# xipengwang/AprilSAM

Hardware: AMD Instinct MI355X
Metric: Gauss-Newton iterations/sec + factorise ms on M3500 (chi2 match <=1e-6) (higher is better)
Workload: dtype f64; 1 GPU; M3500 batch april_graph_cholesky, 1 replica per GPU (3500 poses, 5454 factors, n=10500); parallelism=single GPU, fronts=680, levels=9, nnz_L=422121

## Files before the change

aprilsam_amd/abi.py:

```python
import ctypes as C


class ZArray(C.Structure):
    _fields_ = [("el_sz", C.c_size_t), ("size", C.c_int), ("alloc", C.c_int), ("data", C.c_void_p)]


class Matd3x3(C.Structure):
    _fields_ = [("nrows", C.c_uint), ("ncols", C.c_uint), ("data", C.c_double * 9)]


class Graph(C.Structure):
    _fields_ = [("factors", C.POINTER(ZArray)), ("nodes", C.POINTER(ZArray)),
                ("attr", C.c_void_p), ("stype", C.c_void_p)]


class FactorCommon(C.Structure):
    _fields_ = [("z", C.POINTER(C.c_double)), ("ztruth", C.POINTER(C.c_double)),
                ("W", C.POINTER(Matd3x3)), ("impl", C.c_void_p)]


class Factor(C.Structure):
    _fields_ = [("type", C.c_int), ("nnodes", C.c_int), ("nodes", C.POINTER(C.c_int)),
                ("length", C.c_int), ("attr", C.c_void_p),
                ("copy", C.c_void_p), ("eval", C.c_void_p), ("state_eval", C.c_void_p),
                ("destroy", C.c_void_p), ("u", FactorCommon), ("stype", C.c_void_p)]


class FactorMax(C.Structure):
    _fields_ = [("factors", C.POINTER(C.POINTER(Factor))), ("logw", C.POINTER(C.c_double)), ("nfactors", C.c_int)]


def max_view(factor):
    f = factor.contents if hasattr(factor, "contents") else factor
    return FactorMax.from_address(C.addressof(f) + Factor.u.offset)


FACTOR_MAX_TYPE = 3
_DESTROY = C.CFUNCTYPE(None, C.c_void_p)


def destroy_factor(fptr):
    _DESTROY(fptr.contents.destroy)(C.cast(fptr, C.c_void_p))


class Node(C.Structure):
    _fields_ = [("UID", C.c_int), ("type", C.c_int), ("length", C.c_int),
                ("state", C.POINTER(C.c_double)), ("init", C.POINTER(C.c_double)),
                ("truth", C.POINTER(C.c_double)), ("l_point", C.POINTER(C.c_double)),
                ("delta_X", C.POINTER(C.c_double)), ("attr", C.c_void_p),
                ("copy", C.c_void_p), ("update", C.c_void_p), ("relinearize", C.c_void_p),
                ("destroy", C.c_void_p), ("impl", C.c_void_p), ("stype", C.c_void_p)]


class CholeskyParam(C.Structure):
    _fields_ = [("tikhanov", C.c_double), ("chol", C.c_void_p), ("factor_num", C.c_int),
                ("ordering", C.POINTER(C.c_int)), ("nreordering", C.c_int), ("show_timing", C.c_int),
                ("delta_x", C.POINTER(C.c_double)), ("B", C.POINTER(C.c_double)),
                ("y", C.POINTER(C.c_double)), ("A", C.c_void_p), ("tr", C.c_void_p),
                ("l_thresh", C.c_double), ("delta_thresh", C.c_double), ("nthreshold", C.c_int),
                ("batch_time", C.c_double), ("delta_xy", C.c_double), ("delta_theta", C.c_double)]


class Stats(C.Structure):
    _fields_ = [("n_nodes", C.c_int), ("n_factors", C.c_int), ("n_fronts", C.c_int), ("n_levels", C.c_int),
                ("max_front_rows", C.c_int), ("symbolic_reused", C.c_int), ("not_spd", C.c_int),
                ("reserved0", C.c_int), ("nnz_L", C.c_longlong), ("flops_factor", C.c_double),
                ("bytes_fronts", C.c_double),
                ("ms_pack", C.c_double), ("ms_symbolic", C.c_double), ("ms_h2d", C.c_double),
                ("ms_device", C.c_double), ("ms_d2h", C.c_double), ("ms_unpack", C.c_double),
                ("ms_total", C.c_double), ("ms_dev_linearize", C.c_double), ("ms_dev_factor", C.c_double),
                ("ms_dev_solve", C.c_double), ("chi2_before", C.c_double), ("error_code", C.c_int), ("reserved1", C.c_int),
                ("inc_replanned", C.c_int), ("inc_old_old_cross", C.c_int), ("inc_fronts_updated", C.c_int), ("dn_launch_fronts", C.c_int)]

    def asdict(self):
        return {k: getattr(self, k) for k, _ in self._fields_}



class LmOpts(C.Structure):
    _fields_ = [("max_iters", C.c_int), ("check_every", C.c_int), ("lambda0", C.c_double), ("lambda_max", C.c_double),
                ("eta", C.c_double), ("ftol", C.c_double), ("xtol", C.c_double)]


class LmReport(C.Structure):
    _fields_ = [("status", C.c_int), ("iterations", C.c_int), ("accepted", C.c_int), ("rejected_not_spd", C.c_int),
                ("F_initial", C.c_double), ("F_final", C.c_double), ("chi2_final", C.c_double), ("lambda_final", C.c_double)]

    def asdict(self):
        return {k: getattr(self, k) for k, _ in self._fields_}


LM_CONVERGED_F, LM_CONVERGED_X, LM_STALLED, LM_MAX_ITERS = 1, 2, 3, 4


class GncOpts(C.Structure):
    _fields_ = [("loss", C.c_int), ("c", C.c_double), ("mu_step", C.c_double), ("max_stages", C.c_int), ("lm", LmOpts)]


class GncReport(C.Structure):
    _fields_ = [("status", C.c_int), ("stages", C.c_int), ("iterations", C.c_int), ("accepted", C.c_int), ("stages_stalled", C.c_int),
                ("n_inliers", C.c_int), ("mu_initial", C.c_double), ("mu_final", C.c_double), ("s_max", C.c_double),
                ("F_final", C.c_double), ("chi2_final", C.c_double)]

    def asdict(self):
        return {k: getattr(self, k) for k, _ in self._fields_}


GNC_GM, GNC_TLS = 1, 2
GNC_FINISHED, GNC_MAX_STAGES = 1, 2


class ChordalOpts(C.Structure):
    _fields_ = [("stages", C.c_int)]


class ChordalReport(C.Structure):
    _fields_ = [("status", C.c_int), ("n_degenerate", C.c_int), ("not_spd_stage", C.c_int), ("min_norm", C.c_double),
                ("F_initial", C.c_double), ("F_final", C.c_double)]

    def asdict(self):
        return {k: getattr(self, k) for k, _ in self._fields_}


ROBUST_NONE, ROBUST_HUBER, ROBUST_CAUCHY, ROBUST_DCS = 0, 1, 2, 3

EXPECTED_SIZES = {"ZArray": 24, "Graph": 32, "Factor": 104, "Node": 112, "CholeskyParam": 128}
EXPECTED_OFFSETS = {
    "Node": dict(UID=0, type=4, length=8, state=16, init=24, truth=32, l_point=40, delta_X=48, attr=56,
                 copy=64, update=72, relinearize=80, destroy=88, impl=96, stype=104),
    "Factor": dict(type=0, nnodes=4, nodes=8, length=16, attr=24, copy=32, eval=40, state_eval=48,
                   destroy=56, u=64, stype=96),
    "CholeskyParam": dict(tikhanov=0, chol=8, factor_num=16, ordering=24, nreordering=32, show_timing=36,
                          delta_x=40, B=48, y=56, A=64, tr=72, l_thresh=80, delta_thresh=88,
                          nthreshold=96, batch_time=104, delta_xy=112, delta_theta=120),
}
```

aprilsam_amd/csrc/capi.cpp:

```cpp
#include <algorithm>
#include <cstdio>
#include <cstdlib>
#include <cstring>
#include <string>
#include <vector>

#include "../../include/aprilsam_amd.h"
#include "plan.h"
#include "errors.h"
#include "refmodel.h"
#include "solver.h"

extern "C" {

void APRILSAM_VERSION(void) {
    printf("================\n");
    printf("| APRILSAM 0.0 |   solver: aprilsam_amd (MI355X / gfx950)\n");
    printf("================\n");
    printf("\n");
}

void april_graph_cholesky_param_init(april_graph_cholesky_param_t *param) {
    asam::drop_context(param);
    asam::unbind_param(param);
// ... 77 lines not shown
    for (int i = 0; i < M->N; i++) visited[i] = 0;
    M->solve_visit(x, dxy, dth, [&](int n, bool upd) { visited[n] = upd ? 2 : 1; });
    return M->start_over;
}
void aprilsam_amd_refmodel_get(void *m, int *parent, int *changed, int *relin) {
    asam::RefModel *M = (asam::RefModel *)m;
    for (int i = 0; i < M->N; i++) { if (parent) parent[i] = M->parent[i]; if (changed) changed[i] = M->changed[i]; if (relin) relin[i] = M->relin[i]; }
}
int aprilsam_amd_refmodel_check(void *m) { return ((asam::RefModel *)m)->check_tree(); }
int aprilsam_amd_last_error(char *msg, int cap) { return asam::get_last_error(msg, cap); }
void aprilsam_amd_clear_error(void) { asam::clear_last_error(); }
int aprilsam_amd_selftest(void) { return asam::selftest(); }
const char *aprilsam_amd_version(void) { return "aprilsam_amd 0.1 (gfx950, multifrontal FP64)"; }
void aprilsam_amd_free(void *p) { free(p); }

struct aprilsam_amd_plan { asam::Plan P; };

aprilsam_amd_plan_t *aprilsam_amd_plan_create(int n_nodes, int n_factors, const int *factor_nodes, const double *xy, int leaf_nodes) {
    aprilsam_amd_plan *pl = new aprilsam_amd_plan();
    try {
        asam::build_plan(pl->P, n_nodes, n_factors, factor_nodes, xy, leaf_nodes > 0 ? leaf_nodes : asam::g_opt.leaf_nodes);
    } catch (const asam::SolverError &e) {
        asam::set_last_error(e.code, e.msg);
        fprintf(stderr, "aprilsam_amd: ERROR %d: %s\n", e.code, e.msg.c_str());
        delete pl;
        return nullptr;
    } catch (const std::exception &e) {
        asam::set_last_error(asam::ERR_INTERNAL, e.what());
        fprintf(stderr, "aprilsam_amd: ERROR %d: %s\n", (int)asam::ERR_INTERNAL, e.what());
        delete pl;
        return nullptr;
    }
    return pl;
}
void aprilsam_amd_plan_destroy(aprilsam_amd_plan_t *plan) { delete plan; }

long long aprilsam_amd_shard_plan(const aprilsam_amd_plan_t *plan, int world, int what, long long *out, long long cap) {
    if (!plan || world < 1) return -1;
    std::vector<int> owner; std::vector<char> top; std::vector<long long> xfer, bcast, v;
    asam::shard_map(plan->P, world, owner, top, xfer, bcast);
    if (what == 1) v = xfer; else if (what == 2) v = bcast; else if (what == 3) v.assign(owner.begin(), owner.end());
    else if (what == 4) v = asam::shard_critical_path(plan->P, world, owner, top); else return -1;
    if (out) for (long long i = 0; i < (long long)v.size() && i < cap; i++) out[i] = v[i];
    return (long long)v.size();
}

int aprilsam_amd_xcd_place(int nF, const int *parent, const int *level, const int *nsb, int l0, int cap, int cap_leaf, int which, int *out, int out_cap) {
    if (nF < 0 || !parent || !level || !nsb || which < 0 || which > 3) return -100;
    std::vector<int> up, leaves;
    int top = 0;
    for (int t = 0; t < nF; t++) top = std::max(top, level[t]);
    for (int l = l0; l <= top; l++) for (int t = 0; t < nF; t++) if (level[t] == l) up.push_back(t);
    if (l0 == 1) for (int t = 0; t < nF; t++) if (level[t] == 0) leaves.push_back(t);
    const asam::XcdLists x = asam::xcd_place(up, leaves, parent, nsb, nF, cap, cap_leaf);
    if (which == 3) return asam::xcd_check(x, up, leaves, parent, nF, cap, cap_leaf);
    const std::vector<int> &v = which == 0 ? x.up : which == 1 ? x.dn : x.leaf;
    if (out) for (int i = 0; i < (int)v.size() && i < out_cap; i++) out[i] = v[i];
    return (int)v.size();
}

long long aprilsam_amd_plan_query(const aprilsam_amd_plan_t *plan, const char *what, long long **out) {
    std::string k(what);
    if (k.compare(0, 3, "bd_") == 0 || k.compare(0, 3, "rd_") == 0) asam::build_gather_lists(const_cast<asam::Plan &>(plan->P));
    const asam::Plan &P = plan->P;
    std::vector<long long> v;
    auto from = [&](const auto &a) { v.assign(a.begin(), a.end()); };
    if (k == "perm") from(P.perm);
    else if (k == "pos") from(P.pos);
    else if (k == "front_first") from(P.f_first);
    else if (k == "front_nsb") from(P.f_nsb);
    else if (k == "front_nub") from(P.f_nub);
    else if (k == "front_parent") from(P.f_parent);
    else if (k == "front_level") from(P.f_level);
    else if (k == "front_rows_ptr") from(P.f_rows_ptr);
    else if (k == "front_rows") from(P.f_rows);
    else if (k == "front_rel") from(P.f_rel);
    else if (k == "front_off") from(P.f_off);
    else if (k == "ch_ptr") from(P.ch_ptr);
    else if (k == "ch_idx") from(P.ch_idx);
    else if (k == "factor_front") from(P.fac_front);
    else if (k == "factor_la") from(P.fac_la);
    else if (k == "factor_lb") from(P.fac_lb);
    else if (k == "factor_swap") from(P.fac_swap);
    else if (k == "bd_front_ptr") from(P.bd_front_ptr);
    else if (k == "bd_row") from(P.bd_row);
    else if (k == "bd_col") from(P.bd_col);
    else if (k == "bd_src_ptr") from(P.bd_src_ptr);
    else if (k == "bd_src") from(P.bd_src);
    else if (k == "rd_front_ptr") from(P.rd_front_ptr);
    else if (k == "rd_col") from(P.rd_col);
    else if (k == "rd_src_ptr") from(P.rd_src_ptr);
    else if (k == "rd_src") from(P.rd_src);
    else if (k == "lev_ptr") from(P.lev_ptr);
    else if (k == "lev_fronts") from(P.lev_fronts);
    else if (k == "stats") v = { P.nF, P.nLevels, P.max_rows, (long long)P.nnzL, (long long)P.flops, (long long)P.pool_doubles };
    else { *out = nullptr; return -1; }
    *out = (long long *)malloc(sizeof(long long) * (v.size() + 1));
    if (!v.empty()) memcpy(*out, v.data(), sizeof(long long) * v.size());
    return (long long)v.size();
}

}
```

aprilsam_amd/csrc/kernels.hip.h:

```cpp
#pragma once
#include <hip/hip_runtime.h>
#include <stdint.h>

#include <type_traits>
namespace asam {

constexpr int PROF_SLOTS = 16;
constexpr int PROF_XCD_UP = 12, PROF_XCD_DN = 13;
constexpr int PROF_X_STORED = 14, PROF_X_DRAINED = 11, PROF_X_FLAG = 15;
__device__ __forceinline__ int xcc_id() { return __builtin_amdgcn_s_getreg(20 | (0 << 6) | ((4 - 1) << 11)) & 7; }
constexpr int TPB = 256;
constexpr int NB = 32;
constexpr int TILE = 64;
constexpr int ASM_CB = 4;
constexpr int OBP = 4;

struct FrontDesc {
    long long off;
    int nsb, nub, first;
    int dest_begin, dest_end;
    int ch_begin, ch_end;
    int rows_begin;
    int parent;
    int dinv0;
    int prim1, prim2;
    int pad[2];
};
static_assert(sizeof(FrontDesc) == 64, "FrontDesc must stay one cache line");
struct DestRec { int brow, bcol, src_begin, src_end; };
struct ChildRec {
    long long uoff;
    int cR;
    int cnu;
    int rel_begin;
    int pad;
};
static_assert(sizeof(ChildRec) == 24, "ChildRec layout");

struct DevPlan {
    int nF;
    const FrontDesc *fd;
    const DestRec *dest;
    const ChildRec *child;
    const int *f_rows, *f_rel;
    const int *slot_blk, *slot_rhs;
    const int *src_idx;
    const double *lambda;
    long long *prof;
    int prof_mode;
    int schur_first_nub;
    int *epoch; const int *flevel; int l0; const int *marks;
    int xmode; uint4 *xg; unsigned xg_bytes;
};
enum { X_FLUSH = 0, X_WT = 1, X_TAGGED = 2 };
constexpr int XG_CONST = -1;

__host__ __device__ inline int asm_chunks(int nbc) { return (nbc + ASM_CB - 1) / ASM_CB; }
struct SyrkRange { int k_lo, k_hi, col_lo, col_hi, ntr, ntc; };
__host__ __device__ inline SyrkRange syrk_range(int R, int C, int ns, int s_lo, int s_hi, int tile = TILE, bool ahead = false) {
    SyrkRange g;
    g.k_lo = s_lo * NB;
    g.k_hi = s_hi * NB < ns ? s_hi * NB : ns;
    g.col_lo = g.k_hi;
    g.col_hi = ahead ? (g.k_hi + OBP * NB < ns ? g.k_hi + OBP * NB : ns) : C;
    if (g.k_hi <= g.k_lo || g.col_hi <= g.col_lo) { g.ntr = g.ntc = 0; return g; }
    g.ntr = ((R - 2) - g.col_lo + tile - 1) / tile;
    g.ntc = (g.col_hi - g.col_lo + tile - 1) / tile;
    return g;
}
__host__ __device__ inline int syrk_tiles(int R, int C, int ns, int s_lo, int s_hi, int tile = TILE, bool ahead = false) {
    SyrkRange g = syrk_range(R, C, ns, s_lo, s_hi, tile, ahead);
    return g.ntc * g.ntr - g.ntc * (g.ntc - 1) / 2;
}
__device__ __forceinline__ int find_seg(const int *__restrict__ pre, int n, int bid) {
    int lo = 0, hi = n;
    while (hi - lo > 1) { int m = (lo + hi) >> 1; if (pre[m] <= bid) lo = m; else hi = m; }
    return lo;
}

__device__ __forceinline__ void trapezoid_tile(int l, int ntr, int ntc, int *ti, int *tj_);
constexpr int SYRK_SB = 8;
constexpr int SYRK_MODE_XCD_SHIFT = 8;
__host__ __device__ inline void trapezoid_tile_xcd(int l, int nt, int ntr, int ntc, int *ti, int *tj) {
    const int q = nt >> 3, rem = nt & 7, x = l & 7;
    int lp = x * q + (x < rem ? x : rem) + (l >> 3);
    for (int c0 = 0;; ) {
        const int w = ntc - c0 < SYRK_SB ? ntc - c0 : SYRK_SB;
        const int cnt = w * (ntr - c0) - w * (w - 1) / 2;
        if (lp < cnt || c0 + w >= ntc) {
            const int tri = w * (w + 1) / 2;
            if (lp < tri) { int r = 0; while ((r + 1) * (r + 2) / 2 <= lp) r++; *ti = c0 + r; *tj = c0 + lp - r * (r + 1) / 2; }
            else { const int e = lp - tri; *ti = c0 + w + e / w; *tj = c0 + e % w; }
            return;
        }
        lp -= cnt; c0 += w;
    }
}

__device__ __forceinline__ double mod2pi_dev(double v) {
    const double TWOPI = 6.2831853071795862319959;
    const double PI_ = 3.141592653589793238462643383279502884196;
    double vin = v + PI_;
    return (vin - TWOPI * floor(vin / TWOPI)) - PI_;
}

__device__ __forceinline__ double fast_rsqrt(double d) {
    double y = __builtin_amdgcn_rsq(d);
    const double h = 0.5 * d;
    double e = fma(-h * y, y, 0.5);
// ... 28 lines not shown
            double acc = 0;
#pragma unroll
            for (int k = 0; k < 3; k++) acc += a[i * 3 + k] * b[k * 3 + j];
            c[i * 3 + j] = acc;
        }
}
__device__ __forceinline__ void a_v(const double *a, const double *v, double *c) {
#pragma unroll
    for (int i = 0; i < 3; i++) {
        double acc = 0;
#pragma unroll
        for (int k = 0; k < 3; k++) acc += a[i * 3 + k] * v[k];
        c[i] = acc;
    }
}

__device__ __forceinline__ void factor_residual(bool binary, const double *pa, const double *pb, const double *z,
                                                double *J0, double *J1, double *r) {
    if (binary) {
        double xa = pa[0], ya = pa[1], ta = pa[2];
        double xb = pb[0], yb = pb[1], tb = pb[2];
        double sa, ca;
        sincos(ta, &sa, &ca);
        double dx = xb - xa, dy = yb - ya;
        double zh0 = ca * dx + sa * dy, zh1 = -sa * dx + ca * dy, zh2 = tb - ta;
        J0[0] = -ca; J0[1] = -sa; J0[2] = -sa * dx + ca * dy;
        J0[3] = sa;  J0[4] = -ca; J0[5] = -ca * dx - sa * dy;
        J0[6] = 0;   J0[7] = 0;   J0[8] = -1;
        J1[0] = ca;  J1[1] = sa;  J1[2] = 0;
        J1[3] = -sa; J1[4] = ca;  J1[5] = 0;
        J1[6] = 0;   J1[7] = 0;   J1[8] = 1;
        r[0] = z[0] - zh0; r[1] = z[1] - zh1; r[2] = mod2pi_dev(z[2] - zh2);
    } else {
        J0[0] = 1; J0[1] = 0; J0[2] = 0; J0[3] = 0; J0[4] = 1; J0[5] = 0; J0[6] = 0; J0[7] = 0; J0[8] = 1;
        r[0] = z[0] - pa[0]; r[1] = z[1] - pa[1]; r[2] = mod2pi_dev(z[2] - pa[2]);
    }
}
__device__ __forceinline__ double rtWr(const double *w, const double *r) {
    double X0 = w[0] * r[0] + w[1] * r[1] + w[2] * r[2];
    double X1 = w[3] * r[0] + w[4] * r[1] + w[5] * r[2];
    double X2 = w[6] * r[0] + w[7] * r[1] + w[8] * r[2];
    return r[0] * X0 + r[1] * X1 + r[2] * X2;
}

__global__ void __launch_bounds__(TPB) k_scatter_host(int nh, const int *__restrict__ idx, const double *__restrict__ hostH, const int *__restrict__ fb,
                                                      const unsigned char *__restrict__ swp, const int *__restrict__ slot_blk,
                                                      const int *__restrict__ slot_rhs, double *__restrict__ Hc) {
    const int k = blockIdx.x * blockDim.x + threadIdx.x;
    if (k >= nh) return;
    const int f = idx[k];
    const double *H = hostH + (size_t)33 * k;
    double *o = Hc + (size_t)slot_blk[3 * f] * 9;
#pragma unroll
    for (int i = 0; i < 3; i++)
#pragma unroll
        for (int j = 0; j < 3; j++) o[i * 3 + j] = (i <= j) ? H[i * 3 + j] : H[j * 3 + i];
    double *go = Hc + (size_t)slot_rhs[2 * f] * 9;
    go[0] = H[27]; go[1] = H[28]; go[2] = H[29];
    if (fb[f] >= 0) {
        const bool s = swp[f] & 1;
        double *o1 = Hc + (size_t)slot_blk[3 * f + 1] * 9, *o2 = Hc + (size_t)slot_blk[3 * f + 2] * 9;
        double *g1 = Hc + (size_t)slot_rhs[2 * f + 1] * 9;
#pragma unroll
        for (int i = 0; i < 3; i++)
#pragma unroll
            for (int j = 0; j < 3; j++) {
                o1[i * 3 + j] = s ? H[9 + j * 3 + i] : H[9 + i * 3 + j];
                o2[i * 3 + j] = (i <= j) ? H[18 + i * 3 + j] : H[18 + j * 3 + i];
            }
        g1[0] = H[30]; g1[1] = H[31]; g1[2] = H[32];
    }
}

#ifndef LIN_WAVES
#define LIN_WAVES 4
#endif
constexpr int LIN_STRIDE = 13;
template <bool STAGED>
__device__ __forceinline__ void linearise_factor(int gtid, int f_begin, int f_end, const int *__restrict__ flist, const int *__restrict__ fa, const int *__restrict__ fb,
                                                 const double *__restrict__ Z, const double *__restrict__ Wm,
                                                 const double *__restrict__ lp, const double *__restrict__ st,
                                                 const unsigned char *__restrict__ swp, const int *__restrict__ slot_blk,
                                                 const int *__restrict__ slot_rhs, double *__restrict__ Hc, const double *__restrict__ upt,
                                                 double (*stg)[STAGED ? 64 * LIN_STRIDE : 1], int (*sid)[STAGED ? 128 : 1], double *mirror = nullptr) {
    int f = f_begin + gtid;
    bool active = f < f_end;
    if (!STAGED && !active) return;
    if (!active) f = f_begin;
    if (flist) f = flist[f];
    int a = fa[f], b = fb[f];
    if (a < 0) { if (!STAGED) return; active = false; a = 0; b = -1; }
    double w[9], z[3], J0[9], J1[9], r[3], pa[3], pb[3] = { 0, 0, 0 };
#pragma unroll
    for (int k = 0; k < 9; k++) w[k] = Wm[(size_t)9 * f + k];
#pragma unroll
    for (int k = 0; k < 3; k++) z[k] = Z[(size_t)3 * f + k];
    const bool binary = b >= 0;
    const double *src = binary ? lp + (size_t)3 * a : (upt ? upt + (size_t)3 * f : st + (size_t)3 * a);
#pragma unroll
    for (int k = 0; k < 3; k++) pa[k] = src[k];
    if (binary) {
#pragma unroll
        for (int k = 0; k < 3; k++) pb[k] = lp[(size_t)3 * b + k];
    }
    factor_residual(binary, pa, pb, z, J0, J1, r);
    const int wave = threadIdx.x >> 6, lane = threadIdx.x & 63;
    auto flush = [&](const double *v, auto nv_, int s0, int s1) {
        constexpr int NV = decltype(nv_)::value;
        double *mine = stg[wave] + lane * LIN_STRIDE;
#pragma unroll
        for (int k = 0; k < NV; k++) mine[k] = v[k];
        sid[wave][2 * lane] = s0; sid[wave][2 * lane + 1] = s1;
        asm volatile("s_waitcnt lgkmcnt(0)" ::: "memory");
#pragma unroll
        for (int it = 0; it < NV; it++) {
            const int idx = it * 64 + lane, t = idx / NV, e = idx - t * NV;
            const int sl = sid[wave][2 * t + (e < 9 ? 0 : 1)];
            if (sl >= 0) Hc[(size_t)sl * 9 + (e < 9 ? e : e - 9)] = stg[wave][t * LIN_STRIDE + e];
        }
        asm volatile("" ::: "memory");
    };
    double JtW0[9], H[9], g[3], out[12];
    at_b(J0, w, JtW0);
    a_b(JtW0, J0, H);
    a_v(JtW0, r, g);
    if constexpr (STAGED) {
#pragma unroll
        for (int i = 0; i < 3; i++)
#pragma unroll
            for (int j = 0; j < 3; j++) out[i * 3 + j] = (i <= j) ? H[i * 3 + j] : H[j * 3 + i];
        out[9] = g[0]; out[10] = g[1]; out[11] = g[2];
        flush(out, std::integral_constant<int, 12>{}, active ? slot_blk[3 * f] : -1, active ? slot_rhs[2 * f] : -1);
    } else {
        double *o = Hc + (size_t)slot_blk[3 * f] * 9;
#pragma unroll
        for (int i = 0; i < 3; i++)
#pragma unroll
            for (int j = 0; j < 3; j++) o[i * 3 + j] = (i <= j) ? H[i * 3 + j] : H[j * 3 + i];
        double *go = Hc + (size_t)slot_rhs[2 * f] * 9;
        go[0] = g[0]; go[1] = g[1]; go[2] = g[2];
        if (mirror) {
#pragma unroll
            for (int k = 0; k < 9; k++) mirror[33 * gtid + k] = o[k];
#pragma unroll
            for (int k = 0; k < 3; k++) mirror[33 * gtid + 9 + k] = g[k];
        }
    }
    if (STAGED ? __ballot(binary && active) != 0ull : binary) {
        const bool on = binary && active;
        a_b(JtW0, J1, H);
        const unsigned sw = swp[f];
        const bool s = sw & 1;
        double JtW1[9], H2[9];
        at_b(J1, w, JtW1);
        a_b(JtW1, J1, H2);
        a_v(JtW1, r, g);
        if (sw & 2) {
            double Hba[9];
            a_b(JtW1, J0, Hba);
#pragma unroll
            for (int i = 0; i < 3; i++)
#pragma unroll
                for (int j = 0; j < 3; j++) H[i * 3 + j] = Hba[j * 3 + i];
        }
        if constexpr (STAGED) {
#pragma unroll
            for (int i = 0; i < 3; i++)
#pragma unroll
                for (int j = 0; j < 3; j++) out[i * 3 + j] = s ? H[j * 3 + i] : H[i * 3 + j];
            flush(out, std::integral_constant<int, 9>{}, on ? slot_blk[3 * f + 1] : -1, -1);
#pragma unroll
            for (int i = 0; i < 3; i++)
#pragma unroll
                for (int j = 0; j < 3; j++) out[i * 3 + j] = (i <= j) ? H2[i * 3 + j] : H2[j * 3 + i];
            out[9] = g[0]; out[10] = g[1]; out[11] = g[2];
            flush(out, std::integral_constant<int, 12>{}, on ? slot_blk[3 * f + 2] : -1, on ? slot_rhs[2 * f + 1] : -1);
        } else {
            double *o1 = Hc + (size_t)slot_blk[3 * f + 1] * 9, *o2 = Hc + (size_t)slot_blk[3 * f + 2] * 9;
            double *g1 = Hc + (size_t)slot_rhs[2 * f + 1] * 9;
#pragma unroll
            for (int i = 0; i < 3; i++)
#pragma unroll
                for (int j = 0; j < 3; j++) o1[i * 3 + j] = s ? H[j * 3 + i] : H[i * 3 + j];
#pragma unroll
            for (int i = 0; i < 3; i++)
#pragma unroll
// ... 1423 lines not shown
    syrk_big_body<4, false, 1>(P, list, pre, n, s_lo, s_hi, mode, pool);
}

__device__ __forceinline__ void trapezoid_tile(int l, int ntr, int ntc, int *ti, int *tj_) {
    const float b = 2.0f * ntr + 1.0f;
    int tj = (int)((b - sqrtf(fmaxf(b * b - 8.0f * l, 0.0f))) * 0.5f);
    if (tj < 0) tj = 0;
    if (tj > ntc - 1) tj = ntc - 1;
    while (tj > 0 && tj * ntr - tj * (tj - 1) / 2 > l) tj--;
    while (tj + 1 < ntc && (tj + 1) * ntr - (tj + 1) * tj / 2 <= l) tj++;
    *tj_ = tj;
    *ti = tj + (l - (tj * ntr - tj * (tj - 1) / 2));
}

template <int CTRL, int ROW_MASK>
__device__ __forceinline__ double dpp_take(double v) {
    const int lo = __builtin_amdgcn_update_dpp(0, __double2loint(v), CTRL, ROW_MASK, 0xf, true);
    const int hi = __builtin_amdgcn_update_dpp(0, __double2hiint(v), CTRL, ROW_MASK, 0xf, true);
    return __hiloint2double(hi, lo);
}
__device__ __forceinline__ double wave_sum63(double v) {
    v += dpp_take<0x111, 0xf>(v);
    v += dpp_take<0x112, 0xf>(v);
    v += dpp_take<0x114, 0xf>(v);
    v += dpp_take<0x118, 0xf>(v);
    v += dpp_take<0x142, 0xa>(v);
    v += dpp_take<0x143, 0xc>(v);
    return v;
}

constexpr long long BS_SPLIT_MIN = 1 << 17;
constexpr int BS_CHUNK = 4096;
__host__ __device__ inline bool bs_split_front(int nsb, int nub) { return nub > 0 && (9ll * nsb * nub >= BS_SPLIT_MIN || 3 * nsb > NB * 4); }
__global__ void __launch_bounds__(TPB) k_backsolve_gemv(DevPlan P, const int *__restrict__ list, const int *__restrict__ pre, int n,
                                                        const double *__restrict__ pool, double *__restrict__ x) {
    __shared__ double xu[BS_CHUNK];
    const int seg = find_seg(pre, n, blockIdx.x);
    const int t = list[seg], cb = blockIdx.x - pre[seg];
    const FrontDesc D_ = P.fd[t];
    const int nsb = D_.nsb, nub = D_.nub, nbc = nsb + nub;
    const int R = 3 * (nbc + 1), ns = 3 * nsb, nu = 3 * nub;
    const int k0 = cb * NB, wdt = min(NB, ns - k0);
    const double *Fg = pool + D_.off;
    const int tid = threadIdx.x, wave = tid >> 6, lane = tid & 63;
    const int *rows = P.f_rows + D_.rows_begin;
    const int c0 = wave * 8;
    double acc[8];
    const double *colp[8];
#pragma unroll
    for (int q = 0; q < 8; q++) { acc[q] = 0; colp[q] = Fg + (size_t)(k0 + min(c0 + q, wdt - 1)) * R + ns; }
    for (int r0 = 0; r0 < nu; r0 += BS_CHUNK) {
        const int nr = min(BS_CHUNK, nu - r0);
        __syncthreads();
        for (int e = tid; e < nr; e += TPB) xu[e] = x[(size_t)3 * rows[(r0 + e) / 3] + (r0 + e) % 3];
        __syncthreads();
        int i = lane;
        for (; i + 192 < nr; i += 256) {
            double v[4][8];
#pragma unroll
            for (int u = 0; u < 4; u++)
#pragma unroll
                for (int q = 0; q < 8; q++) v[u][q] = colp[q][r0 + i + 64 * u];
#pragma unroll
            for (int u = 0; u < 4; u++) {
                const double xv = xu[i + 64 * u];
#pragma unroll
                for (int q = 0; q < 8; q++) acc[q] = fma(v[u][q], xv, acc[q]);
            }
        }
        for (; i < nr; i += 64) {
            const double xv = xu[i];
#pragma unroll
            for (int q = 0; q < 8; q++) acc[q] = fma(colp[q][r0 + i], xv, acc[q]);
        }
    }
#pragma unroll
    for (int q = 0; q < 8; q++) {
        const double sum = wave_sum63(acc[q]);
        if (lane == 63 && c0 + q < wdt) x[(size_t)3 * D_.first + k0 + c0 + q] = sum;
    }
}

__host__ __device__ inline size_t backsolve_lds(int m, int ns, bool pre) { return (size_t)(m + NB + 8 + NB * (NB + 1) + (pre ? (size_t)ns * ((m + 3) | 1) : 0)) * 8; }
struct UpdArgs { const int *perm; const double *lp; double *st, *dX, *st_out, *dx_out; int *bad_out; double *lp_next; };
__device__ __forceinline__ void backsolve_finish(const FrontDesc &D_, int t, const double *xw, double *__restrict__ x, int *xflags, int *bad, const UpdArgs &upd, int ev = 0,
                                                 int xmode = X_FLUSH, const DevPlan *P = nullptr, long long *pf = nullptr) {
    const int tid = threadIdx.x, nsb = D_.nsb, ns = 3 * nsb;
    if (xmode == X_TAGGED) {
        const __amdgpu_buffer_rsrc_t r = xg_rsrc(*P);
        for (int e = tid; e < ns; e += TPB) st_granule(r, (size_t)3 * D_.first + e, xw[e], ev);
        if (pf && tid == 0) pf[PROF_X_STORED] = pf[PROF_X_FLAG] = wall_clock64();
        for (int e = tid; e < ns; e += TPB) x[(size_t)3 * D_.first + e] = xw[e];
    } else if (xmode == X_WT) {
        for (int e = tid; e < ns; e += TPB) st_agent(x + (size_t)3 * D_.first + e, xw[e]);
        if (pf && tid == 0) pf[PROF_X_STORED] = wall_clock64();
        publish_flag_wt(xflags + t, ev, pf);
    } else {
        for (int e = tid; e < ns; e += TPB) x[(size_t)3 * D_.first + e] = xw[e];
        if (pf && tid == 0) pf[PROF_X_STORED] = wall_clock64();
        if (xflags) publish_flag(xflags + t, ev, pf);
    }
    if (upd.perm) {
        for (int k = tid; k < nsb; k += TPB) {
            const int i = upd.perm[D_.first + k];
            const double d0 = xw[3 * k], d1 = xw[3 * k + 1], d2 = xw[3 * k + 2];
            if (isnan(d0) || isnan(d1) || isnan(d2)) {
                const double qnan = __longlong_as_double(0x7ff8000000000000ll);
                upd.dX[3 * i + 0] = qnan; upd.dX[3 * i + 1] = qnan; upd.dX[3 * i + 2] = qnan;
                if (upd.dx_out) { upd.dx_out[3 * i + 0] = qnan; upd.dx_out[3 * i + 1] = qnan; upd.dx_out[3 * i + 2] = qnan; }
                continue;
            }
            const double s0 = upd.lp[3 * i + 0] + d0, s1 = upd.lp[3 * i + 1] + d1, s2 = mod2pi_dev(upd.lp[3 * i + 2] + d2);
            if (upd.st) { upd.st[3 * i + 0] = s0; upd.st[3 * i + 1] = s1; upd.st[3 * i + 2] = s2; }
            if (upd.lp_next) { upd.lp_next[3 * i + 0] = s0; upd.lp_next[3 * i + 1] = s1; upd.lp_next[3 * i + 2] = s2; }
            upd.dX[3 * i + 0] = d0; upd.dX[3 * i + 1] = d1; upd.dX[3 * i + 2] = d2;
            if (upd.st_out) {
                upd.st_out[3 * i + 0] = s0; upd.st_out[3 * i + 1] = s1; upd.st_out[3 * i + 2] = s2;
                upd.dx_out[3 * i + 0] = d0; upd.dx_out[3 * i + 1] = d1; upd.dx_out[3 * i + 2] = d2;
            }
        }
    }
    if (upd.bad_out && tid == 0 && __hip_atomic_load(bad, __ATOMIC_RELAXED, __HIP_MEMORY_SCOPE_AGENT) != 0) {
#pragma unroll
        for (int k = 0; k < 4; k++) upd.bad_out[k] = __hip_atomic_load(bad + k, __ATOMIC_RELAXED, __HIP_MEMORY_SCOPE_AGENT);
    }
}
constexpr int BS_TALL_ROWS = 768;
template <bool PRE, bool TALL = false>
__global__ void __launch_bounds__(TPB) k_backsolve_t(DevPlan P, const int *__restrict__ fronts, const double *__restrict__ pool,
                                                     double *__restrict__ x, int split, int *xflags, int wait, int *bad, UpdArgs upd) {
    extern __shared__ __attribute__((aligned(16))) double smem[];
    const int t = fronts[blockIdx.x];
    if (t < 0) return;
    const int ev = xflags ? flag_value(P) : 0;
    const FrontDesc D_ = P.fd[t];
    const int nsb = D_.nsb, nub = D_.nub, nbc = nsb + nub;
    const int R = 3 * (nbc + 1), ns = 3 * nsb, m = 3 * nbc;
    double *xw = smem;
    double *part = smem + m;
    double *Ldg = smem + m + NB + 8;
    const double *Fg = pool + D_.off;
    const int tid = threadIdx.x, wave = tid >> 6, lane = tid & 63;
    const int *rows = P.f_rows + D_.rows_begin;
    long long *pf = (P.prof && P.prof_mode == 2) ? P.prof + (size_t)t * PROF_SLOTS : nullptr;
    double *Lp = smem + m + NB + 8 + NB * (NB + 1);
    const int ldp = R | 1;
    auto Lat = [&](int c, int r) -> double { if constexpr (PRE) return Lp[c * ldp + r]; else return Fg[(size_t)c * R + r]; };
    if constexpr (PRE) {
        const int ne = ns * R;
        for (int e0 = tid; e0 < ne; e0 += 8 * TPB) {
            double v[8];
#pragma unroll
            for (int u = 0; u < 8; u++) v[u] = Fg[min(e0 + u * TPB, ne - 1)];
#pragma unroll
            for (int u = 0; u < 8; u++) { const int e = e0 + u * TPB; if (e < ne) { const int c = e / R; Lp[c * ldp + (e - c * R)] = v[u]; } }
        }
    }
    const int xmode = x_handover_mode(P, xflags, ev, PRE && wait);
    const bool xtag = xmode == X_TAGGED && D_.parent >= 0;
    if (wait && D_.parent >= 0 && !xtag) {
        if (tid == 0) wait_flag(xflags + D_.parent, bad, ev);
        if constexpr (PRE) { __syncthreads(); asm volatile("" ::: "memory"); }
        else acquire_all();
    }
    if (pf && tid == 0 && !xtag) pf[4] = wall_clock64();
    const bool pre_t = split && bs_split_front(nsb, nub);
    const int mprod = pre_t ? ns : m;
    if (pre_t) { for (int e = tid; e < ns; e += TPB) xw[e] = Fg[(size_t)e * R + m] - x[(size_t)3 * D_.first + e]; }
    else {
        for (int e = tid; e < ns; e += TPB) xw[e] = Fg[(size_t)e * R + m];
        if (xtag) gather_x(P, D_, rows, xw + ns, 3 * nub, ev, bad, pf);
        else for (int e = tid; e < 3 * nub; e += TPB) { const double *xp = x + (size_t)3 * rows[e / 3] + e % 3; if constexpr (PRE) xw[ns + e] = ld_agent(xp); else xw[ns + e] = *xp; }
    }
    __syncthreads();
    if (pf && tid == 0) pf[5] = wall_clock64();
    long long t_prod = 0, t_sum = 0, t_solve = 0, ts = 0;
    constexpr int PFU = 8;
    double pv[TALL ? PFU : 1][8], pdg[4];
    auto prefetch = [&](int k1p) {
        if constexpr (TALL && !PRE) {
            const int k0p = max(0, k1p - NB), wdtp = k1p - k0p;
#pragma unroll
            for (int q = 0; q < 4; q++) {
                const int e = tid + q * TPB, r = e & 31, cc = e >> 5;
                pdg[q] = Fg[(size_t)(k0p + min(cc, wdtp - 1)) * R + k0p + min(r, wdtp - 1)];
            }
#pragma unroll
            for (int u = 0; u < PFU; u++) {
                const int row = min(k1p + lane + 64 * u, mprod - 1);
                if (k1p + 64 * u < mprod) {
#pragma unroll
                    for (int q = 0; q < 8; q++) pv[u][q] = Fg[(size_t)(k0p + min(wave * 8 + q, wdtp - 1)) * R + row];
                } else {
#pragma unroll
                    for (int q = 0; q < 8; q++) pv[u][q] = 0.0;
                }
            }
        }
    };
    prefetch(ns);
    for (int k1 = ns; k1 > 0; k1 -= NB) {
        const int k0 = max(0, k1 - NB), wdt = k1 - k0;
        if (pf) ts = wall_clock64();
        double dg[4];
#pragma unroll
        for (int q = 0; q < 4; q++) {
            const int e = tid + q * TPB, r = e & 31, cc = e >> 5;
            if constexpr (TALL && !PRE) dg[q] = pdg[q]; else dg[q] = Lat(k0 + min(cc, wdt - 1), k0 + min(r, wdt - 1));
// ... 153 lines not shown
    double *Iv = Ls + 6 * NB * (NB + 1);
    const bool pre_t = split && bs_split_front(nsb, nub);
    for (int e = tid; e < ns; e += TPB) xw[e] = pre_t ? x[(size_t)3 * D_.first + e] : 0.0;
    __syncthreads();
    for (int B = nB - 1; B >= 0; B--) {
        const int k0 = B * OBW, Wb = min(OBW, ns - k0), nsub = (Wb + NB - 1) / NB;
        double lv[24], iv[16];
#pragma unroll
        for (int k = 0; k < 24; k++) {
            const int e = tid + TPB * k, bq = e >> 10, i = e & 31, j = (e >> 5) & 31;
            const int sr = bq == 0 ? 1 : (bq < 3 ? 2 : 3), sc = bq == 0 ? 0 : (bq < 3 ? bq - 1 : bq - 3);
            lv[k] = Fg[(size_t)(k0 + min(NB * sc + j, Wb - 1)) * R + k0 + min(NB * sr + i, Wb - 1)];
        }
        const double *dv = dinv_keep + ((size_t)D_.dinv0 + B * OBP) * (NB * NB);
#pragma unroll
        for (int k = 0; k < 16; k++) iv[k] = dv[tid + TPB * k];
        Gemv128 g;
        const int wnext = B < nB - 1 ? min(OBW, ns - (k0 + OBW)) : 1;
        if (B < nB - 1) gemv128_load(g, Fg, R, k0 + OBW, wnext, k0);
        if (B < nB - 2 && tid == 0) wait_flag(tflag + B, bad);
#pragma unroll
        for (int k = 0; k < 24; k++) {
            const int e = tid + TPB * k, bq = e >> 10, i = e & 31, j = (e >> 5) & 31;
            const int sr = bq == 0 ? 1 : (bq < 3 ? 2 : 3);
            Ls[bq * (NB * (NB + 1)) + i * (NB + 1) + j] = (NB * sr + i < Wb) ? lv[k] : 0.0;
        }
#pragma unroll
        for (int k = 0; k < 16; k++) { const int e = tid + TPB * k; Iv[(e >> 10) * (NB * (NB + 1)) + ((e >> 5) & 31) * (NB + 1) + (e & 31)] = iv[k]; }
        if (B < nB - 1) gemv128_sums(g, w, [&](int q, double sum) { xs[32 * wave + q] = sum; });
        __syncthreads();
        {
            double v = 0.0;
            const int e = tid;
            if (e < Wb) {
                v = Fg[(size_t)(k0 + e) * R + m] - xw[k0 + e];
                if (B < nB - 1) v -= xs[e];
                if (B < nB - 2) v -= ld_agent(farf + (size_t)B * OBW + e);
            }
            __syncthreads();
            if (e < OBW) w[e] = v;
        }
        __syncthreads();
        for (int sb = nsub - 1; sb >= 0; sb--) {
            {
                const int i = tid & 31, part = tid >> 5;
                double acc = 0;
#pragma unroll
                for (int jj = 0; jj < 4; jj++) { const int j = 4 * part + jj; acc = fma(Iv[sb * (NB * (NB + 1)) + j * (NB + 1) + i], w[NB * sb + j], acc); }
                xs[part * NB + i] = acc;
            }
            __syncthreads();
            if (tid < NB) {
                double v = 0;
#pragma unroll
                for (int part = 0; part < 8; part++) v += xs[part * NB + tid];
                w[NB * sb + tid] = v;
                if (NB * sb + tid < Wb) xw[k0 + NB * sb + tid] = v;
            }
            __syncthreads();
            if (sb > 0) {
                const int q = tid >> 6, l = tid & 63, j = l & 31, half = l >> 5;
                if (q < sb) {
                    const int bq = (sb == 1 ? 0 : (sb == 2 ? 1 : 3)) + q;
                    double acc = 0;
#pragma unroll
                    for (int ii = 0; ii < 16; ii++) { const int i = 16 * half + ii; acc = fma(Ls[bq * (NB * (NB + 1)) + i * (NB + 1) + j], w[NB * sb + i], acc); }
                    xs[256 + (q * 2 + half) * NB + j] = acc;
                }
                __syncthreads();
                if (tid < NB * sb) { const int q = tid >> 5, j = tid & 31; w[NB * q + j] -= xs[256 + (q * 2) * NB + j] + xs[256 + (q * 2 + 1) * NB + j]; }
                __syncthreads();
            }
        }
        for (int e = tid; e < Wb; e += TPB) x[(size_t)3 * D_.first + k0 + e] = xw[k0 + e];
        if (B >= 2 && H > 0) publish_flag(xflag + B);
    }
    __syncthreads();
    for (int e = tid; e < 2 * BSB_MAXB; e += TPB) reset_flag(xflag + e, 0);
    backsolve_finish(D_, t, xw, x, nullptr, bad, upd);
}

constexpr int BSW = 64;
constexpr int BSW_MAX_NS = NB + 8 + NB * (NB + 1) - 256;
template <int BSWT = BSW>
__device__ __forceinline__ void backsolve_w_body(const DevPlan &P, const int t, const double *__restrict__ pool, double *__restrict__ x, int *xflags, int *bad,
                                                 const UpdArgs &upd, double *smem) {
    const int ev = xflags ? flag_value(P) : 0;
    const FrontDesc D_ = P.fd[t];
    const int nsb = D_.nsb, nub = D_.nub, nbc = nsb + nub;
    const int R = 3 * (nbc + 1), ns = 3 * nsb, m = 3 * nbc;
    double *xw = smem;
    double *partial = smem + m;
    double *dgs = smem + m + 256;
    double *Lp = smem + m + NB + 8 + NB * (NB + 1);
    const int ldp = R | 1;
    const double *Fg = pool + D_.off;
    const int tid = threadIdx.x, wave = tid >> 6, lane = tid & 63;
    const int *rows = P.f_rows + D_.rows_begin;
    long long *pf = (P.prof && P.prof_mode == 2) ? P.prof + (size_t)t * PROF_SLOTS : nullptr;
    if (pf && tid == 0) pf[PROF_XCD_DN] = 1 + xcc_id();
    {
        const int ne = ns * R;
        for (int e0 = tid; e0 < ne; e0 += 8 * TPB) {
            double v[8];
#pragma unroll
            for (int u = 0; u < 8; u++) v[u] = Fg[min(e0 + u * TPB, ne - 1)];
#pragma unroll
            for (int u = 0; u < 8; u++) {
                const int e = e0 + u * TPB;
                if (e < ne) {
                    const int c = e / R, r = e - c * R;
                    Lp[c * ldp + r] = r > c ? v[u] : 0.0;
                    if (r == c) dgs[c] = v[u];
                }
            }
        }
    }
    const int xmode = x_handover_mode(P, xflags, ev, true);
    const bool xtag = xmode == X_TAGGED && D_.parent >= 0;
    if (xflags && D_.parent >= 0 && !xtag) {
        if (tid == 0) wait_flag(xflags + D_.parent, bad, ev);
        __syncthreads();
        asm volatile("" ::: "memory");
    }
    if (pf && tid == 0 && !xtag) pf[4] = wall_clock64();
    for (int e = tid; e < ns; e += TPB) xw[e] = Fg[(size_t)e * R + m];
    if (xtag) gather_x(P, D_, rows, xw + ns, 3 * nub, ev, bad, pf);
    else for (int e = tid; e < 3 * nub; e += TPB) xw[ns + e] = ld_agent(x + (size_t)3 * rows[e / 3] + e % 3);
    __syncthreads();
    if (pf && tid == 0) pf[5] = wall_clock64();
    for (int k1 = ns; k1 > 0; k1 -= BSWT) {
        const int k0 = max(0, k1 - BSWT), wdt = k1 - k0;
        const bool on = lane < wdt;
        const int c = k0 + (on ? lane : 0);
        const double *Lc = Lp + (size_t)c * ldp;
        auto chain = [&](auto w_) {
            constexpr int W = decltype(w_)::value;
            double l[W];
#pragma unroll
            for (int i = 1; i < W; i++) l[i] = Lc[k0 + min(i, wdt - 1)];
            const double rinv = on ? 1.0 / dgs[c] : 1.0;
#pragma unroll
            for (int i = 1; i < W; i++) l[i] *= rinv;
            __syncthreads();
            if (pf && tid == 0 && k1 == ns) pf[6] = wall_clock64();
            double w = on ? (xw[c] - ((partial[64 + lane] + partial[128 + lane]) + partial[192 + lane])) * rinv : 0.0;
#pragma unroll
            for (int i = W - 1; i > 0; i--) {
                const double xi = readlane_d(w, i);
                w = fma(-l[i], xi, w);
            }
            if (on) xw[c] = w;
        };
        if (wave == 0) {
            if (wdt <= 16) chain(std::integral_constant<int, 16>{});
            else if (BSWT <= 32 || wdt <= 32) chain(std::integral_constant<int, 32>{});
            else if constexpr (BSWT > 32) chain(std::integral_constant<int, 64>{});
        } else {
            double acc0 = 0, acc1 = 0;
            int i = k1 + wave - 1;
            for (; i + 3 < m; i += 6) { acc0 = fma(Lc[i], xw[i], acc0); acc1 = fma(Lc[i + 3], xw[i + 3], acc1); }
            if (i < m) acc0 = fma(Lc[i], xw[i], acc0);
            partial[wave * 64 + lane] = acc0 + acc1;
            __syncthreads();
        }
        __syncthreads();
    }
    if (pf && tid == 0) pf[7] = wall_clock64();
    backsolve_finish(D_, t, xw, x, xflags, bad, upd, ev, xmode, &P, pf);
}
__global__ void __launch_bounds__(TPB) k_backsolve_w(DevPlan P, const int *__restrict__ fronts, const double *__restrict__ pool,
                                                     double *__restrict__ x, int *xflags, int *bad, UpdArgs upd) {
    extern __shared__ __attribute__((aligned(16))) double smem[];
    const int t = fronts[blockIdx.x];
    if (t < 0) return;
    backsolve_w_body(P, t, pool, x, xflags, bad, upd, smem);
}

__host__ __device__ inline long long upd_packed_offset(int R, int ns, int j) {
    const long long Rv = R - 2, nb0 = ns / 3, b = j / 3, e = j - 3 * b;
    return 3 * ((b - nb0) * Rv - 3 * (nb0 + b - 1) * (b - nb0) / 2) + e * (Rv - 3 * b);
}
__global__ void __launch_bounds__(TPB) k_guard(int mode, const long long *__restrict__ offs, int n, int len, double *__restrict__ pool, int *count) {
    const int b = blockIdx.x;
    if (b >= n) return;
    unsigned long long *g = (unsigned long long *)(pool + offs[b]);
    int bad = 0;
    for (int i = threadIdx.x; i < len; i += TPB) {
        if (mode == 0) g[i] = ~0ull;
        else if (g[i] != ~0ull) bad++;
    }
    if (bad) { atomicAdd(count, bad); count[1] = b; }
}
__global__ void __launch_bounds__(TPB) k_poison(DevPlan P, const int *__restrict__ list, int n, const int *__restrict__ skip_mode, int skip_stride, int what,
                                                double *__restrict__ pool, double *__restrict__ x) {
    if ((int)blockIdx.x >= n) return;
    if (skip_mode && skip_mode[(size_t)blockIdx.x * skip_stride]) return;
    const int t = list ? list[blockIdx.x] : (int)blockIdx.x;
    const FrontDesc D = P.fd[t];
    const int nbc = D.nsb + D.nub, R = 3 * (nbc + 1), ns = 3 * D.nsb, C = 3 * nbc;
    const double qnan = __longlong_as_double(0x7ff8000000000000ll);
    double *Fg = pool + D.off;
    if (what & 1)
        for (int c = ns + (threadIdx.x >> 6); c < C; c += TPB / 64)
            for (int r = 3 * (c / 3) + (threadIdx.x & 63); r < R - 2; r += 64) Fg[(size_t)c * R + r] = qnan;
    if (what & 2) for (int e = threadIdx.x; e < ns; e += TPB) x[(size_t)3 * D.first + e] = qnan;
}
__global__ void __launch_bounds__(TPB) k_pack_update(double *__restrict__ front, int R, int ns, double *__restrict__ buf, int dir) {
    const int j = ns + blockIdx.x, Rv = R - 2, r0 = j / 3 * 3;
    double *__restrict__ col = front + (size_t)j * R;
    double *__restrict__ pk = buf + upd_packed_offset(R, ns, j) - r0;
    if (dir == 0) { for (int r = r0 + threadIdx.x; r < Rv; r += TPB) pk[r] = col[r]; }
    else { for (int r = r0 + threadIdx.x; r < Rv; r += TPB) col[r] = pk[r]; }
}

struct Patch { void *dst; long long src_off; long long bytes; };
__global__ void __launch_bounds__(TPB) k_apply_patches(const Patch *__restrict__ patches, const char *__restrict__ payload) {
    const Patch p = patches[blockIdx.x];
    const char *src = payload + p.src_off;
    char *dst = (char *)p.dst;
    if (((((size_t)dst) | ((size_t)src) | (size_t)p.bytes) & 3) == 0) {
        for (long long i = threadIdx.x; i < p.bytes / 4; i += TPB) ((int *)dst)[i] = ((const int *)src)[i];
    } else {
        for (long long i = threadIdx.x; i < p.bytes; i += TPB) dst[i] = src[i];
    }
}
struct IncFlags { int *epoch; int *marks; const int *up_list; int n_up; };
constexpr int INL_PATCHES = 24, INL_BYTES = 2048;
struct alignas(16) InlinePatches { Patch hdr[INL_PATCHES]; char pay[INL_BYTES]; };
struct IncPrologue {
    const Patch *patches; const char *payload; int n_patch, f_begin, f_end;
    int inl;

    const int *fa, *fb; const double *Z, *Wm, *lp, *st; const unsigned char *swp; const int *slot_blk, *slot_rhs; double *Hc; int *bad;
    long long *stamps;
    int *done; int seq;
};
struct IncArgsHead { IncPrologue a; IncFlags fl; InlinePatches inl; };
constexpr int TAIL_MAXF = 8;
__device__ __forceinline__ void inc_prologue_body(const IncPrologue &a, const IncFlags &fl, double *mirror = nullptr) {
    const Patch *patches = a.patches; const char *payload = a.payload; const int n_patch = a.n_patch, f_begin = a.f_begin, f_end = a.f_end;
    const int *__restrict__ fa = a.fa, *__restrict__ fb = a.fb; const double *__restrict__ Z = a.Z, *__restrict__ Wm = a.Wm, *__restrict__ lp = a.lp, *__restrict__ st = a.st;
    const unsigned char *__restrict__ swp = a.swp; const int *__restrict__ slot_blk = a.slot_blk, *__restrict__ slot_rhs = a.slot_rhs; double *__restrict__ Hc = a.Hc; int *__restrict__ bad = a.bad;
    const int wave = threadIdx.x >> 6, lane = threadIdx.x & 63, nthr = (int)blockDim.x;
    if (threadIdx.x < 4) bad[threadIdx.x] = 0;
    const char *kargs = (const char *)__builtin_amdgcn_kernarg_segment_ptr() + offsetof(IncArgsHead, inl);
    if (a.inl) { patches = (const Patch *)(kargs + offsetof(InlinePatches, hdr)); payload = kargs + offsetof(InlinePatches, pay); }
    for (int q = wave; q < n_patch; q += nthr >> 6) {
        const Patch p = patches[q];
        const char *src = payload + p.src_off;
        char *dst = (char *)p.dst;
        if (((((size_t)dst) | ((size_t)src) | (size_t)p.bytes) & 3) == 0) {
            const int nw = (int)(p.bytes / 4);
            for (int i0 = lane; i0 < nw; i0 += 512) {
                int v[8];
#pragma unroll
                for (int u = 0; u < 8; u++) v[u] = ((const int *)src)[min(i0 + 64 * u, nw - 1)];
#pragma unroll
                for (int u = 0; u < 8; u++) if (i0 + 64 * u < nw) ((int *)dst)[i0 + 64 * u] = v[u];
// ... 243 lines not shown
```

aprilsam_amd/csrc/plan.h:

```cpp
#pragma once
#include <cstdint>
#include <functional>
#include <vector>

namespace asam {

struct Plan {
    int N = 0;
    int F = 0;
    int leaf_nodes = 16;

    std::vector<int> perm;
    std::vector<int> pos;

    int nF = 0;
    std::vector<int> f_first;
    std::vector<int> f_nsb;
    std::vector<int> f_nub;
    std::vector<int> f_parent;
    std::vector<int> f_level;
    std::vector<int64_t> f_rows_ptr;
    std::vector<int> f_rows;
    std::vector<int> f_rel;
    std::vector<int> ch_ptr, ch_idx;
    std::vector<int64_t> f_off;
    int64_t pool_doubles = 0;

    inline int rows(int t) const { return 3 * (f_nsb[t] + f_nub[t] + 1); }
    inline int cols(int t) const { return 3 * (f_nsb[t] + f_nub[t]); }

    std::vector<int> fac_front;
    std::vector<int> fac_la, fac_lb;
    std::vector<int> bd_front_ptr;
    std::vector<int> bd_row, bd_col;
    std::vector<int> bd_src_ptr;
    std::vector<int> bd_src;
    std::vector<int> rd_front_ptr;
    std::vector<int> rd_col;
    std::vector<int> rd_src_ptr;
    std::vector<int> rd_src;
    std::vector<uint8_t> fac_swap;
    struct DestRec { int brow, bcol, src_begin, src_end; };
    std::vector<int> dest_front_ptr;
    std::vector<DestRec> dest;
    std::vector<int> slot_blk;
    std::vector<int> slot_rhs;
    int n_slots = 0;

    int nLevels = 0;
    std::vector<int> lev_ptr, lev_fronts;

    int max_rows = 0;
    int64_t nnzL = 0;
    double flops = 0;
};

void build_plan(Plan &P, int N, int F, const int *factor_nodes, const double *xy, int leaf_nodes);
void build_gather_lists(Plan &P);

struct XcdLists { std::vector<int> up, dn, leaf; };
XcdLists xcd_place(const std::vector<int> &up, const std::vector<int> &leaves, const int *parent, const int *nsb, int nF, int cap, int cap_leaf);
int xcd_check(const XcdLists &x, const std::vector<int> &up, const std::vector<int> &leaves, const int *parent, int nF, int cap, int cap_leaf);

struct NDTree {
    struct Node { std::vector<int> verts; std::vector<int> children; };
    std::vector<Node> nodes;
    std::vector<int> roots;
};
void nested_dissection(int N, const std::vector<int> &adj_ptr, const std::vector<int> &adj,
                       const double *xy, int leaf_nodes, NDTree &tree);

struct PlanSession { explicit PlanSession(int n_nodes, int min_nodes = 1024); ~PlanSession(); PlanSession(const PlanSession &) = delete; bool on = false; };
void plan_parallel_for(int n, int grain, const std::function<void(int, int)> &body);

}
```

aprilsam_amd/csrc/solver.h:

```cpp
#pragma once
#include <vector>
#include "../../include/aprilsam_amd.h"

namespace asam {

struct Options {
    int leaf_nodes = 16;
    int deterministic = 0;
    int use_graph = 1;
    int device_timing = 0;
    int trust_factor_cache = 0;
    int small_lds_kb = 156;
    int inc_fast = 1;
    int inc_multi = 1;
    int inc_one = 1;
    int inc_one_up = 3, inc_one_dn = 4, inc_one_threads = 512, inc_one_spin = 1;
    int inc_tail = 1;
    int inc_inline = 1;
    int inc_tail_solve = 1;
    int inc_lazy_states = 1;
    int inc_replan_tall = 1;
    int inc_update = 1;
    int speculate_factors = 1;
    int warm_up = 1;
    int syrk_xcd_order = 512;
    int syrk_small_tiles = 320;
    int syrk_pair_tiles = 2048;
    int syrk_group = 3;
    int schur_first = 40;
    int small_threads = 1024;
    int tp_threads = 512;
    int tp_fronts = 1000;
    int tp_lds_kb = 80;
    int amalg = 0;
    int amalg_max = 64;
    int pin_last = 0;
    int batch_extend = 1;
    int extend_tail_fronts = 3;
    int persist = 1;
    int persist_max_fronts = 240;
    int xcd_place = 1;
    int tail_poses = 28;
    int blk_backsolve = 1;
    int wave_backsolve = 1;
    int tagged_x = 1;
    int linearize_staged_min = 32768;
    int mem_cap_mb = 0;
    int pool_guard = 0;
    int pool_poison = 0;
    int skip_flag_waits = 0;
    int panel_mode = 1;
};
extern Options g_opt;

void batch_step(april_graph_t *g, april_graph_cholesky_param_t *param);
void inc_step(april_graph_t *g, april_graph_cholesky_param_t *param);
void inc_solve_only(april_graph_t *g, april_graph_cholesky_param_t *param);
double graph_chi2(april_graph_t *g);
int batch_resident(april_graph_t *g, april_graph_cholesky_param_t *param, int iters, double *chi2_out, double *ms_out);
int resident_begin(april_graph_t *g, april_graph_cholesky_param_t *param);
int resident_steps(april_graph_t *g, april_graph_cholesky_param_t *param, int n, int mode);
int resident_sync(april_graph_t *g, april_graph_cholesky_param_t *param);
double resident_chi2(april_graph_t *g);
int resident_end(april_graph_t *g, april_graph_cholesky_param_t *param);
int level_profile(const april_graph_cholesky_param_t *param, double *out, int cap_levels);
int kernel_profile(const april_graph_cholesky_param_t *param, double *ms, long long *calls, double *flops, double *bytes, const char **names);
void drop_context(const april_graph_cholesky_param_t *p);
void drop_graph_pack(const april_graph_t *g);
bool get_stats(const april_graph_cholesky_param_t *p, aprilsam_amd_stats_t *out);
int shard_begin(april_graph_t *g, april_graph_cholesky_param_t *param, int rank, int world);
long long shard_info(const april_graph_cholesky_param_t *param, int what, long long *out, long long cap);
int shard_comm_unique_id(char *out128);
int shard_comm_init_rccl(const april_graph_cholesky_param_t *param, const char *id128);
int shard_comm_init_host(const april_graph_cholesky_param_t *param, const aprilsam_amd_host_comm_t *cb);
int shard_comm_info(const april_graph_cholesky_param_t *param, long long *out, char *path, int cap);
int shard_iterate(april_graph_t *g, april_graph_cholesky_param_t *param, int n);
int shard_gather_states(april_graph_t *g, april_graph_cholesky_param_t *param);
double shard_chi2(april_graph_t *g, april_graph_cholesky_param_t *param);
void shard_end(const april_graph_cholesky_param_t *param);
int debug_guard_selftest(const april_graph_cholesky_param_t *param);
int debug_stage(april_graph_t *g, april_graph_cholesky_param_t *param, int what, double *out);
int debug_front_times(const april_graph_cholesky_param_t *param, long long *out, int n_fronts);
int api_device_count();
int selftest();
struct Plan;
void shard_map(const Plan &P, int world, std::vector<int> &owner, std::vector<char> &top, std::vector<long long> &xfer, std::vector<long long> &bcast);
std::vector<long long> shard_critical_path(const Plan &P, int world, const std::vector<int> &owner, const std::vector<char> &top);
int api_set_device(int d);
int api_param_set_device(const april_graph_cholesky_param_t *param, int slot);
int api_param_get_device(const april_graph_cholesky_param_t *param);
void unbind_param(const april_graph_cholesky_param_t *param);
void warm_up() noexcept;
int api_set_option(const char *name, double v);
int api_get_option(const char *name, double *v);
int marginals(april_graph_t *g, april_graph_cholesky_param_t *param, int n, const int *qa, const int *qb, double *cov, bool joint);
long long selinv_runs(const april_graph_cholesky_param_t *param);
int marginals_joint_any(april_graph_t *g, april_graph_cholesky_param_t *param, int n, const int *a, const int *b, double *cov);
int gate_xyt(april_graph_t *g, april_graph_cholesky_param_t *param, int n, const int *a, const int *b, const double *z, const double *W, double *d2, double *S);
long long path_solve_bytes(const april_graph_cholesky_param_t *param);
int max_selected(april_graph_t *g, april_graph_cholesky_param_t *param, int n, const int *factors, int *out);
void lm_opts_init(aprilsam_amd_lm_opts_t *opts);
int optimize_lm(april_graph_t *g, april_graph_cholesky_param_t *param, const aprilsam_amd_lm_opts_t *opts, aprilsam_amd_lm_report_t *report, double *trace);
void gnc_opts_init(aprilsam_amd_gnc_opts_t *opts);
int optimize_gnc(april_graph_t *g, april_graph_cholesky_param_t *param, const aprilsam_amd_gnc_opts_t *opts, int n, const int *candidates,
                 aprilsam_amd_gnc_report_t *report, double *weights, double *stage_trace);
long long graph_captures(const april_graph_cholesky_param_t *param);
void chordal_opts_init(aprilsam_amd_chordal_opts_t *opts);
int initialize_chordal(april_graph_t *g, april_graph_cholesky_param_t *param, const aprilsam_amd_chordal_opts_t *opts, aprilsam_amd_chordal_report_t *report,
                       double *rot_out, double *raw_out);
constexpr int MAX_MIX_K = 8;
bool is_native_max(const april_graph_factor_t *f);
bool max_check(const april_graph_factor_t *f, char *why, int cap);
double max_const(const april_graph_factor_t *f, int i);
int max_select(const april_graph_factor_t *f, const double *pa, const double *pb);
bool robust_of(const april_graph_factor_t *f, int *kind, double *c);
bool plain_common_factor(const april_graph_factor_t *f);
double robust_host_s(const double *z, const double *w, const double *pa, const double *pb);
int robust_weights(april_graph_t *g, april_graph_cholesky_param_t *param, int n, const int *factors, double *w);

}
```

aprilsam_amd/csrc/solver.hip.cpp:

```cpp
#include <hip/hip_runtime.h>
#include <rccl/rccl.h>
#include <dlfcn.h>

#include <algorithm>
#include <array>
#include <chrono>
#include <thread>
#include <cmath>
#include <cstdio>
#include <cstdlib>
#include <cstring>
#include <functional>
#include <map>
#include <memory>
#include <atomic>
#include <mutex>
#include <string>
#include <unordered_map>
#include <vector>

#include "../../include/aprilsam_amd.h"
#include "errors.h"
#include "kernels.hip.h"
#include "maxmix.hip.h"
#include "robust.hip.h"
#include "gnc.hip.h"
#include "lm.hip.h"
#include "chordal.hip.h"
#include "selinv.hip.h"
#include "pathsolve.hip.h"
#include "plan.h"
#include "refmodel.h"
#include "solver.h"

namespace asam {

#define HIPCHECK(expr)                                                                                 \
    do {                                                                                               \
        hipError_t e_ = (expr);                                                                        \
        if (e_ != hipSuccess) {                                                                        \
            (void)hipGetLastError();                                                                   \
            fail(e_ == hipErrorOutOfMemory ? ERR_OOM : ERR_HIP, "%s failed: %s (%s:%d)", #expr, hipGetErrorString(e_), __FILE__, __LINE__); \
        }                                                                                              \
    } while (0)

static double now_ms() {
    return std::chrono::duration<double, std::milli>(std::chrono::steady_clock::now().time_since_epoch()).count();
}

Options g_opt;
struct OptionDef { const char *name; int Options::*member; int min_value; bool policy; int max_value = 0x7fffffff; };
static const OptionDef OPTION_TABLE[] = {
    { "leaf_nodes", &Options::leaf_nodes, 1, false }, { "deterministic", &Options::deterministic, 0, true }, { "use_graph", &Options::use_graph, 0, true },
    { "device_timing", &Options::device_timing, 0, true }, { "trust_factor_cache", &Options::trust_factor_cache, 0, true },
    { "small_lds_kb", &Options::small_lds_kb, 0, false }, { "syrk_xcd_order", &Options::syrk_xcd_order, 0, false },
    { "schur_first", &Options::schur_first, 0, false }, { "syrk_small_tiles", &Options::syrk_small_tiles, 0, false }, { "syrk_pair_tiles", &Options::syrk_pair_tiles, 0, false }, { "syrk_group", &Options::syrk_group, 2, false, 8 }, { "panel_mode", &Options::panel_mode, 0, false },
    { "small_threads", &Options::small_threads, 64, false }, { "tp_fronts", &Options::tp_fronts, 0, false }, { "tp_lds_kb", &Options::tp_lds_kb, 0, false },
    { "tp_threads", &Options::tp_threads, 64, false }, { "inc_fast", &Options::inc_fast, 0, true }, { "inc_multi", &Options::inc_multi, 0, true },
    { "inc_one", &Options::inc_one, 0, true }, { "inc_one_up", &Options::inc_one_up, 1, true }, { "inc_one_dn", &Options::inc_one_dn, 1, true },
    { "inc_one_threads", &Options::inc_one_threads, 64, true }, { "inc_one_spin", &Options::inc_one_spin, 0, true }, { "inc_tail", &Options::inc_tail, 0, false },
    { "inc_inline", &Options::inc_inline, 0, true }, { "inc_update", &Options::inc_update, 0, true }, { "inc_tail_solve", &Options::inc_tail_solve, 0, true },
    { "inc_lazy_states", &Options::inc_lazy_states, 0, true }, { "inc_replan_tall", &Options::inc_replan_tall, 0, true },
    { "speculate_factors", &Options::speculate_factors, 0, true }, { "warm_up", &Options::warm_up, 0, true }, { "pin_last", &Options::pin_last, 0, false }, { "persist", &Options::persist, 0, false },
    { "persist_max_fronts", &Options::persist_max_fronts, 0, false }, { "xcd_place", &Options::xcd_place, 0, false }, { "linearize_staged_min", &Options::linearize_staged_min, 0, false },
    { "wave_backsolve", &Options::wave_backsolve, 0, false }, { "tagged_x", &Options::tagged_x, 0, false, 2 }, { "blk_backsolve", &Options::blk_backsolve, 0, false }, { "tail_poses", &Options::tail_poses, 8, false },
    { "batch_extend", &Options::batch_extend, 0, true }, { "extend_tail_fronts", &Options::extend_tail_fronts, 0, true }, { "mem_cap_mb", &Options::mem_cap_mb, 0, true },
    { "pool_guard", &Options::pool_guard, 0, false }, { "amalg", &Options::amalg, 0, false }, { "amalg_max", &Options::amalg_max, 1, false }, { "pool_poison", &Options::pool_poison, 0, false }, { "skip_flag_waits", &Options::skip_flag_waits, 0, false },
};
static const OptionDef *find_option(const char *name) {
    for (const OptionDef &d : OPTION_TABLE) if (!strcmp(d.name, name)) return &d;
    return nullptr;
}
static std::once_flag g_opt_once;
static void load_env_options() {
    std::call_once(g_opt_once, [] {
        for (const OptionDef &d : OPTION_TABLE) {
            std::string env = "APRILSAM_AMD_";
            for (const char *q = d.name; *q; q++) env += (char)toupper((unsigned char)*q);
            const char *sv = getenv(env.c_str());
            if (sv && *sv) g_opt.*(d.member) = std::min(d.max_value, std::max(d.min_value, (int)atof(sv)));
        }
    });
}

constexpr int MAX_SLOTS = 64;
static std::atomic<int> g_device{ -1 };
static std::mutex g_slot_mu[MAX_SLOTS];
static thread_local int t_slot = 0;
static int device_count() {
    static std::atomic<int> cached{ 0 };
    int n = cached.load(std::memory_order_relaxed);
    if (n > 0) return n;
    if (hipGetDeviceCount(&n) != hipSuccess) { (void)hipGetLastError(); return 0; }
    if (n > 0) cached.store(n, std::memory_order_relaxed);
    return n;
}
static int physical_device(int slot) { const int n = device_count(); return n > 0 ? slot % n : 0; }
static thread_local int t_device = -1;
template <class V> struct Registry {
    using Map = std::map<const void *, std::unique_ptr<V>>;
    Map m; mutable std::mutex mu;
    typename Map::iterator find(const void *k) { std::lock_guard<std::mutex> lk(mu); return m.find(k); }
    typename Map::iterator end() { return m.end(); }
    std::pair<typename Map::iterator, bool> emplace(const void *k, std::unique_ptr<V> v) { std::lock_guard<std::mutex> lk(mu); return m.emplace(k, std::move(v)); }
    void erase(typename Map::iterator it) { std::lock_guard<std::mutex> lk(mu); m.erase(it); }
    void put(const void *k, std::unique_ptr<V> v) { std::lock_guard<std::mutex> lk(mu); m[k] = std::move(v); }
    template <class F> void for_each(F &&f) { std::lock_guard<std::mutex> lk(mu); for (auto &kv : m) f(*kv.second); }
    template <class F> bool with(const void *k, F &&f) { std::lock_guard<std::mutex> lk(mu); auto it = m.find(k); if (it == m.end()) return false; f(*it->second); return true; }
};
static std::map<const void *, int> g_param_slot; static std::mutex g_param_slot_mu;
static std::atomic<int> g_param_slot_n{ 0 };
static int default_slot() { const int d = g_device.load(std::memory_order_relaxed); return d < 0 ? 0 : d % MAX_SLOTS; }
static int slot_of_graph(const void *g);
static int slot_for(const void *param, const void *g) {
    if (param && g_param_slot_n.load(std::memory_order_acquire) > 0) { std::lock_guard<std::mutex> lk(g_param_slot_mu); auto it = g_param_slot.find(param); if (it != g_param_slot.end()) return it->second; }
    if (!param && g) { const int s = slot_of_graph(g); if (s >= 0) return s; }
    return default_slot();
}
struct SlotLock {
    int slot; std::unique_lock<std::mutex> lk;
    SlotLock(const void *param, const void *g) : slot(slot_for(param, g)), lk(g_slot_mu[slot]) {
        for (int now; (now = slot_for(param, g)) != slot; ) { lk.unlock(); slot = now; lk = std::unique_lock<std::mutex>(g_slot_mu[slot]); }
        t_slot = slot;
        if (device_count() > 0) {
            const int dev = physical_device(slot);
            int cur = -1;
            if (t_device != dev || hipGetDevice(&cur) != hipSuccess || cur != dev) { (void)hipSetDevice(dev); t_device = dev; }
        }
    }
};
static std::once_flag g_dev_once;
static void ensure_device() {
    std::call_once(g_dev_once, [] {
        load_env_options();
        int n = device_count();
        if (n <= 0) fail(ERR_NO_DEVICE, "no HIP device visible: the april_graph_cholesky* / april_graph_chi2 entry points of "
                         "libaprilsam_amd.so run on an AMD GPU only (there is NO CPU fallback: nothing was computed)");
        if (g_device < 0) {
            const char *lr = getenv("LOCAL_RANK");
            g_device = lr ? atoi(lr) % n : 0;
        }
    });
}

template <class T> struct DBuf {
    T *p = nullptr; size_t cap = 0;
    bool need(size_t n) {
// ... 312 lines not shown
```

aprilsam_amd/csrc/solver_context.inc.h:

```cpp
enum { K_LINEARIZE = 0, K_FRONT_SMALL, K_ASSEMBLE_BIG, K_PANEL_BIG, K_SYRK_BIG, K_BACKSOLVE, K_UPDATE, NKERN };
static const char *const KNAMES[NKERN] = { "k_linearize", "k_front_small", "k_assemble_big", "k_panel_big", "k_syrk_big", "k_backsolve", "k_update_states" };
struct Launch { int list_off, pre_off, n, grid; bool single = false; int tile = TILE; };

struct LevelPlan {
    int small_off = 0, n_small = 0; size_t small_lds = 0;
    long long full_limit = 0;
    int small_nt = 512;
    int n_big = 0; size_t asm_lds = 0;
    Launch asm_big{};
    std::vector<Launch> syrka, syrk1;
    bool paired = false;
    std::vector<Launch> bchain, btile, syrkw;
    int all_off = 0, n_all = 0; size_t solve_lds = 0;
    size_t solve_w_lds = 0; int maxns = 0;
    Launch bs_gemv{};
    Launch bs_blk{}; size_t bs_blk_lds = 0;
    int rest_off = 0, n_rest = 0; size_t rest_lds = 0;
};

struct IncState {
    bool ready = false;
    bool pristine = false;
    int Nb = 0, Fb = 0, nF0 = 0, nLev0 = 0;
    int cap_nodes = 0, cap_fact = 0;
// ... 16 lines not shown
    std::vector<int> t_first, t_cnt;
    std::vector<int> tf_of;
    std::vector<std::vector<int>> kids;
    std::vector<LevelPlan> base_levels;
    std::vector<int> st_i32, st_tab, st_sb, st_sr, st_ids; std::vector<DestRec> st_dest; std::vector<ChildRec> st_child;
    std::vector<unsigned char> st_sw; std::vector<double> st_zeros; std::vector<char> need;
    std::vector<char> stale;
    bool upd_ok = true;
    bool base_has_big = false;
    std::vector<char> st_mid, st_mode; std::vector<int> st_owner, st_mask, st_wout, st_slot; std::vector<UpdRec> st_upd, st_rec;
};

struct SelLevel { int gat_off = 0, n_gat = 0, diag_off = 0, n_diag = 0, tri_off = 0, n_tri = 0, x_off = 0, n_x = 0, sus_off = 0, n_sus = 0, sss_off = 0, n_sss = 0; };

struct PathState {
    long long serial = -1;
    int N = 0;
    std::vector<SelFront> fr; std::vector<int> depth, i32, rec, node_j;
    DBuf<PsFront> d_fr; DBuf<int4> d_ent; DBuf<int> d_cmap; DBuf<long long> d_at; DBuf<PsPath> d_path; DBuf<PsPair> d_pair;
    DBuf<double> d_buf, d_cov, d_in; HBuf<double> h_out;
    long long peak_doubles = 0;
    void release() {
        d_fr.release(); d_ent.release(); d_cmap.release(); d_at.release(); d_path.release(); d_pair.release(); d_buf.release(); d_cov.release(); d_in.release(); h_out.release();
        fr.clear(); depth.clear(); i32.clear(); rec.clear(); node_j.clear(); serial = -1;
    }
};

struct Context {
    Plan plan;
    bool have_plan = false;
    std::vector<int> pat;
    int patN = 0;
    DBuf<int> d_i32; DBuf<FrontDesc> d_fd; DBuf<DestRec> d_dest; DBuf<ChildRec> d_child; DBuf<double> d_lambda;
    DevPlan dp{};
    DBuf<int> d_tab;
    std::vector<LevelPlan> levels;
    DBuf<unsigned char> d_swap;
    DBuf<int> d_pos;
    DBuf<long long> d_prof;
    DBuf<double> d_pool, d_H, d_x, d_diag;
    DBuf<int> d_bad;
    HBuf<int> h_bad;
    IncPrologue pro{}; InlinePatches inl{};
    bool no_speculation = false;
    HBuf<long long> h_kstamp; HBuf<int> h_done; int done_seq = 0, one_wait = 0;
    std::vector<double> h_lambda;
    aprilsam_amd_stats_t st{};
    hipEvent_t ev[8] = {};
    bool have_events = false;
    double k_ms[NKERN] = {}; long long k_calls[NKERN] = {};
    std::vector<hipEvent_t> k_ev; std::vector<int> k_ids, k_lev;
    std::vector<double> lev_up_ms, lev_dn_ms;
    bool have_fact = false;
    int plan_pin = 0;
    long long plan_persist = 0;
    int same_topo_batches = 0;
    bool used_inc = false;
    bool want_inc = false;
    int batch_nodes = 0;
    IncState inc;
    int inc_F = 0, inc_N = 0;
    std::vector<RefModel::Visit> visits; std::vector<int> involved;
    std::vector<int> base_tab;
    std::vector<int> inc_slot_blk, inc_slot_rhs;
    long long pat_serial = -1, pat_topo = -1;
    RefModel model;
    PatchList patches;
    int batch_factors = 0;
    std::vector<unsigned char> wt; bool wt_any = false, wt_dirty = false;
    long long wt_serial = -1, wt_topo = -1, wt_content = -1;
    DBuf<long long> d_guard; DBuf<int> d_guard_cnt; int n_guard = 0, guard_len = 0;
    std::vector<unsigned char> swap_host;
    int persist_l0 = -1;
    int p_up_off = 0, p_up_n = 0, p_dn_off = 0, p_dn_n = 0, p_nt = 1024; size_t p_up_lds = 0, p_dn_lds = 0; long long p_up_full = 0; int p_dn_maxns = 0, p_dn_maxnu = 0;
    int x_up_off = 0, x_up_n = 0, x_dn_off = 0, x_dn_n = 0;
    int x_leaf_off = 0, x_leaf_n = 0;
    DBuf<int> d_flags, d_flevel, d_perm, d_epoch, d_marks;
    DBuf<uint4> d_xg;
    int flag_stride = 0;
    long long epoch_steps = 0;
    DBuf<double> d_dinv, d_bsb_far; DBuf<int> d_bsb_flags;
    DBuf<int> d_solve_tab; std::vector<int> solve_tab;
    DBuf<UpdRec> d_upd; DBuf<double> d_wbuf;
    hipGraphExec_t gexec = nullptr;
    const void *gexec_key = nullptr;
    long long gexec_serial = 0;
    long long gexec_mx = -1;
    long long gexec_rb = -1;
    hipGraphExec_t gexec_api = nullptr;
    const void *api_key[9] = {};
    hipGraphExec_t gexec_lm = nullptr;
    const void *lm_key[10] = {};
    DBuf<double> d_lm_trial, d_lm_hacc, d_lm_terms, d_lm_trace; DBuf<LmScalars> d_lm; HBuf<LmScalars> h_lm;
    DBuf<double> d_ch; HBuf<double> h_ch; DBuf<int> d_ch_sel;
    long long n_captures = 0;
    int api_key_runs = 0;
    struct Retired { hipGraphExec_t g; hipEvent_t done; };
    std::vector<Retired> retired;
    hipStream_t graph_stream = nullptr;
    void reap_retired(bool wait = false) {
        size_t keep = 0;
        for (Retired &r : retired) {
            if (r.done) {
                if (wait) (void)hipEventSynchronize(r.done);
                else if (hipEventQuery(r.done) != hipSuccess) { retired[keep++] = r; continue; }
                (void)hipEventDestroy(r.done);
            }
            (void)hipGraphExecDestroy(r.g);
        }
        retired.resize(keep);
    }
    void retire(hipGraphExec_t &g) {
        if (!g) return;
        if (retired.size() >= 8) reap_retired();
        if (retired.size() >= 32) reap_retired(true);
        Retired r{ g, nullptr };
        if (graph_stream && hipEventCreateWithFlags(&r.done, hipEventDisableTiming) == hipSuccess) {
            if (hipEventRecord(r.done, graph_stream) != hipSuccess) { (void)hipEventDestroy(r.done); r.done = nullptr; }
        } else r.done = nullptr;
        retired.push_back(r); g = nullptr;
    }
    double lambda_val = -1; int lambda_N = -1;
    int fact_kind = 0; long long fact_epoch = -1; bool fact_asym = false;
    DBuf<double> d_sigma, d_sel_scr; DBuf<SelFront> d_sel_fd; DBuf<int> d_sel_i32, d_sel_q; DBuf<int4> d_sel_ent; HBuf<double> h_cov;
    long long fact_serial = 0;
    std::vector<SelLevel> sel_levels; int sel_tab_kind = 0, sel_N = 0;
    long long sel_serial = -1, sel_tab_serial = -1, sel_runs = 0, sel_pool = 1; double sel_flops = 0;
    PathState ps;
    void release_sel() {
        d_sigma.release(); d_sel_scr.release(); d_sel_fd.release(); d_sel_i32.release(); d_sel_q.release(); d_sel_ent.release(); h_cov.release();
        sel_levels.clear(); sel_serial = -1; sel_tab_serial = -1;
        ps.release();
    }
    void release() {
        release_sel();
        d_i32.release(); d_fd.release(); d_dest.release(); d_child.release(); d_lambda.release(); d_tab.release(); d_swap.release(); d_pos.release();
        d_pool.release(); d_H.release(); d_x.release(); d_diag.release(); d_bad.release(); h_bad.release(); patches.release();
        h_done.release(); h_kstamp.release(); d_prof.release(); d_upd.release(); d_wbuf.release(); d_flags.release(); d_flevel.release(); d_epoch.release(); d_marks.release(); d_perm.release(); d_solve_tab.release(); d_dinv.release(); d_bsb_far.release(); d_bsb_flags.release(); d_guard.release(); d_guard_cnt.release(); n_guard = 0;
        d_lm_trial.release(); d_lm_hacc.release(); d_lm_terms.release(); d_lm_trace.release(); d_lm.release(); h_lm.release();
        d_ch.release(); h_ch.release(); d_ch_sel.release();
        retire(gexec); retire(gexec_api); retire(gexec_lm); reap_retired(true);
        if (have_events) for (auto &e : ev) (void)hipEventDestroy(e);
        have_events = false;
        for (auto &e : k_ev) (void)hipEventDestroy(e);
        k_ev.clear();
    }
};
static Registry<Context> g_ctx;

static void forget_stream(hipStream_t s) {
    g_ctx.for_each([&](Context &c) { if (c.graph_stream == s) c.graph_stream = nullptr; });
}

static Context &ctx_for(const april_graph_cholesky_param_t *p) {
    auto it = g_ctx.find(p);
    if (it == g_ctx.end()) it = g_ctx.emplace(p, std::make_unique<Context>()).first;
    return *it->second;
}
void drop_context(const april_graph_cholesky_param_t *p) {
    SlotLock lk(p, nullptr);
    auto it = g_ctx.find(p);
    if (it != g_ctx.end()) { it->second->release(); g_ctx.erase(it); }
}
bool get_stats(const april_graph_cholesky_param_t *p, aprilsam_amd_stats_t *out) {
    SlotLock lk(p, nullptr);
    auto it = g_ctx.find(p);
    if (it == g_ctx.end()) return false;
    *out = it->second->st;
    return true;
}

struct ShardState;
static void drop_shard_state(const void *param);
static void on_failure(const april_graph_cholesky_param_t *param, const april_graph_t *g, int code, const std::string &msg) {
    set_last_error(code, msg);
    fprintf(stderr, "aprilsam_amd: ERROR %d: %s -- node states left untouched\n", code, msg.c_str());
    fflush(stderr);
    SlotLock lk(param, g);
    (void)hipGetLastError();
    if (g) {
        auto it = g_packs.find(g);
        if (it != g_packs.end()) {
            hipStream_t s = it->second->stream;
            if (s) {
                hipStreamCaptureStatus cs = hipStreamCaptureStatusNone;
                if (hipStreamIsCapturing(s, &cs) == hipSuccess && cs != hipStreamCaptureStatusNone) {
                    hipGraph_t gr = nullptr;
                    (void)hipStreamEndCapture(s, &gr);
                    if (gr) (void)hipGraphDestroy(gr);
                }
                (void)hipStreamSynchronize(s);
                (void)hipGetLastError();
            }
            it->second->release(); g_packs.erase(it);
        }
    }
    if (param) {
        drop_shard_state(param);
        auto it = g_ctx.find(param);
        aprilsam_amd_stats_t st{};
        if (it != g_ctx.end()) { st = it->second->st; it->second->release(); }
        auto fresh = std::make_unique<Context>();
        fresh->st = st; fresh->st.error_code = code; fresh->st.not_spd = 0;
        g_ctx.put(param, std::move(fresh));
    }
}
template <class Fn> static void guarded(const april_graph_cholesky_param_t *param, const april_graph_t *g, Fn &&fn) {
    try { fn(); }
    catch (const SolverError &e) { on_failure(param, g, e.code, e.msg); }
    catch (const std::bad_alloc &) { on_failure(param, g, ERR_OOM, "host memory exhausted (std::bad_alloc)"); }
    catch (const std::exception &e) { on_failure(param, g, ERR_INTERNAL, e.what()); }
}
template <class Fn> static int guarded_rc(const april_graph_cholesky_param_t *param, const april_graph_t *g, Fn &&fn) {
    try { return fn(); }
    catch (const SolverError &e) { on_failure(param, g, e.code, e.msg); return e.code; }
    catch (const std::bad_alloc &) { on_failure(param, g, ERR_OOM, "host memory exhausted (std::bad_alloc)"); return ERR_OOM; }
    catch (const std::exception &e) { on_failure(param, g, ERR_INTERNAL, e.what()); return ERR_INTERNAL; }
}

static const int FIRST_EPOCH = 1 << 20;
struct Context;
static void rewind_epoch(Context &c, hipStream_t s, long long phases);
static void set_const_granules(Context &c, hipStream_t s);
enum { FACT_NONE = 0, FACT_PLAN = 1, FACT_EXTENDED = 2 };
// ... 79 lines not shown
        if (!wide.empty() && wgs <= BSB_MAX_WGS && g_opt.blk_backsolve) {
            const int lo = (int)tab.size();
            tab.insert(tab.end(), wide.begin(), wide.end());
            L.bs_blk = Launch{ lo, (int)tab.size(), (int)wide.size(), 0, false };
            int acc = 0; tab.push_back(0);
            for (int t : wide) { acc += 1 + bsb_helpers(3 * nsb_of(t)); tab.push_back(acc); L.bs_blk_lds = std::max(L.bs_blk_lds, bsb_lds(3 * nsb_of(t))); }
            L.bs_blk.grid = acc;
            L.rest_off = (int)tab.size(); L.n_rest = (int)rest.size();
            tab.insert(tab.end(), rest.begin(), rest.end());
            size_t mm = 0; for (int t : rest) mm = std::max<size_t>(mm, cols(t));
            L.rest_lds = (mm + NB + 8 + NB * (NB + 1)) * 8;
        }
    }
    const int steps = (3 * nsb_of(big[0]) + NB - 1) / NB;
    auto active = [&](int sidx) { int nact = 0; while (nact < (int)big.size() && 3 * nsb_of(big[nact]) > sidx * NB) nact++; return nact; };
    const int nobs = (steps + OBP - 1) / OBP;
    auto make_sub = [&](int i0, int i1, auto count) {
        Launch La; La.list_off = list_off + i0; La.n = i1 - i0; La.pre_off = (int)tab.size();
        int acc = 0; tab.push_back(0);
        for (int i = i0; i < i1; i++) { acc += count(big[i]); tab.push_back(acc); }
        La.grid = acc; La.single = acc == La.n;
        return La;
    };
    auto tile_for = [&](int i0, int i1, int s_lo, int s_hi, bool ahead) {
        int tile = TILE;
        if (g_opt.syrk_small_tiles > 0) {
            long long nt64 = 0;
            for (int i = i0; i < i1; i++) nt64 += syrk_tiles(rows(big[i]), cols(big[i]), 3 * nsb_of(big[i]), s_lo, s_hi, TILE, ahead);
            if (nt64 < g_opt.syrk_small_tiles) tile = TILE / 2;
        }
        return tile;
    };
    {
        long long nt0 = 0;
        for (int i = 0; i < active(0); i++) nt0 += syrk_tiles(rows(big[i]), cols(big[i]), 3 * nsb_of(big[i]), 0, OBP, TILE);
        L.paired = g_opt.syrk_pair_tiles > 0 && nobs >= 2 && nt0 >= g_opt.syrk_pair_tiles;
    }
    for (int o = 0; o < nobs; o++) {
        const int s_lo = o * OBP, s_hi = std::min(s_lo + OBP, steps), nact = active(s_lo);
        if (!L.paired) {
            const int tile = tile_for(0, nact, s_lo, s_hi, false);
            L.syrkw.push_back(make(nact, [&](int t) { return syrk_tiles(rows(t), cols(t), 3 * nsb_of(t), s_lo, s_hi, tile); }));
            L.syrkw.back().tile = tile;
            continue;
        }
        const int G = std::max(2, g_opt.syrk_group), p_lo = (o - o % G) * OBP;
        if (o % G != G - 1) {
            const int n2 = o + 1 < nobs ? active((o + 1) * OBP) : 0;
            int tile = tile_for(0, n2, p_lo, s_hi, true);
            L.syrka.push_back(make_sub(0, n2, [&](int t) { return syrk_tiles(rows(t), cols(t), 3 * nsb_of(t), p_lo, s_hi, tile, true); })); L.syrka.back().tile = tile;
            tile = tile_for(n2, nact, p_lo, s_hi, false);
            L.syrk1.push_back(make_sub(n2, nact, [&](int t) { return syrk_tiles(rows(t), cols(t), 3 * nsb_of(t), p_lo, s_hi, tile); })); L.syrk1.back().tile = tile;
            L.syrkw.push_back(Launch{ 0, 0, 0, 0, false });
        } else {
            const int tile = tile_for(0, nact, p_lo, s_hi, false);
            L.syrka.push_back(Launch{ 0, 0, 0, 0, false }); L.syrk1.push_back(Launch{ 0, 0, 0, 0, false });
            L.syrkw.push_back(make(nact, [&](int t) { return syrk_tiles(rows(t), cols(t), 3 * nsb_of(t), p_lo, s_hi, tile); }));
            L.syrkw.back().tile = tile;
        }
    }
    for (int o = 0; o * OBP < steps; o++) {
        const int nact = active(o * OBP);
        Launch bc{ list_off, 0, nact, nact, true };
        L.bchain.push_back(bc);
        long long tiles1 = 0;
        for (int i = 0; i < nact; i++) tiles1 += block_tiles(rows(big[i]), 3 * nsb_of(big[i]), o, 1);
        const int rb = tiles1 > 1024 ? 2 : 1;
        L.btile.push_back(make(nact, [&](int t) { return block_tiles(rows(t), 3 * nsb_of(t), o, rb); }));
        L.btile.back().tile = rb;
    }
}

struct ShardLayout { std::vector<long long> off; std::vector<char> ghost; long long pool_doubles = 0; };

static void fill_swap_host(Context &c) {
    const Plan &P = c.plan;
    c.swap_host.assign(P.fac_swap.begin(), P.fac_swap.end());
    if (c.wt_any) for (size_t f = 0; f < c.swap_host.size() && f < c.wt.size(); f++) c.swap_host[f] |= (unsigned char)(c.wt[f] << 1);
}
static void upload_plan(Context &c, hipStream_t s, const ShardLayout *lay = nullptr) {
    const Plan &P = c.plan;
    const bool uprof = getenv("APRILSAM_AMD_PLAN_PROFILE") != nullptr;
    const double u0 = uprof ? now_ms() : 0;
    c.retire(c.gexec); c.retire(c.gexec_api); c.retire(c.gexec_lm); c.api_key_runs = 0;
    c.lambda_N = -1;
    c.release_sel();
    std::vector<FrontDesc> &fd = c.inc.fd; fd.assign(P.nF, FrontDesc());
    std::vector<ChildRec> ch(std::max<size_t>(1, P.ch_idx.size()));
    for (int t = 0; t < P.nF; t++) {
        FrontDesc &d = fd[t];
        memset(&d, 0, sizeof(d));
        d.off = lay ? std::max<long long>(lay->off[t], 0) : P.f_off[t]; d.nsb = P.f_nsb[t]; d.nub = P.f_nub[t]; d.first = P.f_first[t];
        d.dest_begin = P.dest_front_ptr[t]; d.dest_end = P.dest_front_ptr[t + 1];
        d.ch_begin = P.ch_ptr[t]; d.ch_end = P.ch_ptr[t + 1];
        d.rows_begin = 0; d.parent = P.f_parent[t];
    }
    for (int t = 0; t < P.nF; t++) {
        int best = -1, second = -1;
        for (int k = P.ch_ptr[t]; k < P.ch_ptr[t + 1]; k++) if (P.f_nub[P.ch_idx[k]] > 0 && (best < 0 || P.f_nub[P.ch_idx[k]] > P.f_nub[P.ch_idx[best]])) best = k;
        for (int k = P.ch_ptr[t]; k < P.ch_ptr[t + 1]; k++) if (k != best && P.f_nub[P.ch_idx[k]] > 0 && (second < 0 || P.f_nub[P.ch_idx[k]] > P.f_nub[P.ch_idx[second]])) second = k;
        fd[t].prim1 = best < 0 ? 0 : best - P.ch_ptr[t] + 1; fd[t].prim2 = second < 0 ? 0 : second - P.ch_ptr[t] + 1;
    }
    for (size_t k = 0; k < P.ch_idx.size(); k++) {
        const int cfr = P.ch_idx[k];
        ChildRec &r = ch[k];
        r.cR = P.rows(cfr); r.cnu = P.f_nub[cfr];
        r.uoff = P.f_off[cfr] + (long long)(3 * P.f_nsb[cfr]) * r.cR + 3 * P.f_nsb[cfr];
        if (lay) {
            if (lay->ghost[cfr]) { r.cR = 3 * r.cnu + 3; r.uoff = lay->off[cfr]; }
            else r.uoff = std::max<long long>(lay->off[cfr], 0) + (long long)(3 * P.f_nsb[cfr]) * r.cR + 3 * P.f_nsb[cfr];
        }
        r.rel_begin = 0; r.pad = cfr;
    }
    const double u1 = uprof ? now_ms() : 0;
    const bool inc = c.want_inc;
    const int INC_NODES_ = inc ? INC_NODES : 0, INC_FACT_ = inc ? INC_FACT : 0;
    const size_t INC_I32_ = inc ? INC_I32 : 0, INC_DEST_ = inc ? INC_DEST : 0, INC_CHILD_ = inc ? INC_CHILD : 0, INC_TAB_ = inc ? INC_TAB : 0;
    c.inc.cap_nodes = INC_NODES_; c.inc.cap_fact = INC_FACT_;
    std::vector<int> i32;
    auto put32 = [&](const std::vector<int> &v) { size_t o = i32.size(); i32.insert(i32.end(), v.begin(), v.end()); if (v.empty()) i32.push_back(0); return o; };
    size_t o_rows = put32(P.f_rows), o_rel = put32(P.f_rel);
    size_t o_sb = put32(P.slot_blk); i32.resize(i32.size() + (size_t)3 * INC_FACT_, -1);
    size_t o_sr = put32(P.slot_rhs); i32.resize(i32.size() + (size_t)2 * INC_FACT_, -1);
    c.inc.i32_used = (long long)i32.size(); c.inc.dest_used = (long long)P.dest.size(); c.inc.child_used = (long long)P.ch_idx.size();
    for (int t = 0; t < P.nF; t++) fd[t].rows_begin = (int)(o_rows + P.f_rows_ptr[t]);
    for (size_t k = 0; k < P.ch_idx.size(); k++) ch[k].rel_begin = (int)(o_rel + P.f_rows_ptr[ch[k].pad]);
    c.d_i32.need(i32.size() + INC_I32_); c.d_fd.need(fd.size() + 1 + (inc ? MAX_TAIL_FRONTS : 0)); c.d_child.need(ch.size() + INC_CHILD_);
    c.d_dest.need(std::max<size_t>(1, P.dest.size()) + INC_DEST_);
    HIPCHECK(hipMemcpyAsync(c.d_i32.p, i32.data(), i32.size() * 4, hipMemcpyHostToDevice, s));
    HIPCHECK(hipMemcpyAsync(c.d_fd.p, fd.data(), fd.size() * sizeof(FrontDesc), hipMemcpyHostToDevice, s));
    HIPCHECK(hipMemcpyAsync(c.d_child.p, ch.data(), ch.size() * sizeof(ChildRec), hipMemcpyHostToDevice, s));
    static_assert(sizeof(DestRec) == sizeof(Plan::DestRec), "DestRec layout");
    if (!P.dest.empty()) HIPCHECK(hipMemcpyAsync(c.d_dest.p, P.dest.data(), P.dest.size() * sizeof(DestRec), hipMemcpyHostToDevice, s));
    c.d_lambda.need((size_t)P.N + INC_NODES_);
    DevPlan &d = c.dp;
    d.nF = P.nF;
    d.fd = c.d_fd.p; d.dest = c.d_dest.p; d.child = c.d_child.p;
    d.f_rows = c.d_i32.p; d.f_rel = c.d_i32.p; d.slot_blk = c.d_i32.p + o_sb; d.slot_rhs = c.d_i32.p + o_sr; d.src_idx = c.d_i32.p;
    c.inc.o_rows = (long long)o_rows; c.inc.o_rel = (long long)o_rel;
    d.lambda = c.d_lambda.p;
    d.prof = nullptr; d.prof_mode = 0;
    d.schur_first_nub = std::max(0, g_opt.schur_first);
    d.epoch = nullptr; d.flevel = nullptr; d.l0 = 0; d.marks = nullptr;
    if (getenv("APRILSAM_AMD_KPROF")) { c.d_prof.need((size_t)PROF_SLOTS * P.nF); HIPCHECK(hipMemsetAsync(c.d_prof.p, 0, (size_t)8 * PROF_SLOTS * P.nF, s)); d.prof = c.d_prof.p; d.prof_mode = atoi(getenv("APRILSAM_AMD_KPROF")) >= 2 ? atoi(getenv("APRILSAM_AMD_KPROF")) : 1; }
    c.d_swap.need((size_t)P.F + INC_FACT_); c.d_pos.need((size_t)P.N + INC_NODES_);
    fill_swap_host(c);
    HIPCHECK(hipMemcpyAsync(c.d_swap.p, c.swap_host.data(), P.F, hipMemcpyHostToDevice, s));
    c.wt_dirty = false;
    HIPCHECK(hipMemcpyAsync(c.d_pos.p, P.pos.data(), (size_t)P.N * 4, hipMemcpyHostToDevice, s));
    c.d_perm.need((size_t)P.N + INC_NODES_);
    HIPCHECK(hipMemcpyAsync(c.d_perm.p, P.perm.data(), (size_t)P.N * 4, hipMemcpyHostToDevice, s));

    const double u2 = uprof ? now_ms() : 0;
    std::vector<int> tab;
    c.levels.assign(P.nLevels, LevelPlan());
    for (int l = 0; l < P.nLevels; l++) {
        std::vector<int> fr(P.lev_fronts.begin() + P.lev_ptr[l], P.lev_fronts.begin() + P.lev_ptr[l + 1]);
        build_level(c.levels[l], fr, tab, [&](int t, int *nsb, int *nub) { *nsb = P.f_nsb[t]; *nub = P.f_nub[t]; }, [](int) { return true; });
    }
    {
        long long slots = 0;
        for (int t = 0; t < P.nF; t++) fd[t].dinv0 = -1;
        for (int l = 0; l < P.nLevels; l++) {
            const LevelPlan &L = c.levels[l];
            for (int k = 0; k < L.asm_big.n; k++) { const int t = tab[L.asm_big.list_off + k]; fd[t].dinv0 = (int)slots; slots += (long long)OBP * bsb_blocks(3 * P.f_nsb[t]); }
        }
        c.d_dinv.need((size_t)std::max<long long>(slots, 1) * NB * NB);
        HIPCHECK(hipMemcpyAsync(c.d_fd.p, fd.data(), fd.size() * sizeof(FrontDesc), hipMemcpyHostToDevice, s));
        if (!c.d_bsb_flags.p) { c.d_bsb_flags.need((size_t)BSB_MAX_WGS * 2 * BSB_MAXB); HIPCHECK(hipMemsetAsync(c.d_bsb_flags.p, 0, c.d_bsb_flags.cap * 4, s)); c.d_bsb_far.need((size_t)BSB_MAX_WGS * BSB_FAR); }
    }
    for (int l = 0; l < P.nLevels; l++)
        if (c.levels[l].solve_lds > 160 * 1024)
            fail(ERR_UNSUPPORTED, "a frontal matrix has more rows than the back-substitution kernel can hold in LDS (an unsplittable dense region "
                 "of more than ~6000 poses); this build does not tile the solve of such a front");
    c.persist_l0 = -1;
    if (g_opt.persist && !lay && P.nLevels >= 3) {
        int l0 = P.nLevels, cnt = 0;
        const int nt_top = c.levels[P.nLevels - 1].small_nt;
        for (int l = P.nLevels - 1; l >= 0; l--) {
            const LevelPlan &L = c.levels[l];
            if (L.n_big > 0 || L.bs_gemv.grid > 0 || L.small_nt != nt_top || L.n_small != L.n_all || cnt + L.n_small > g_opt.persist_max_fronts) break;
            cnt += L.n_small; l0 = l;
        }
        if (P.nLevels - l0 >= 2) {
            c.persist_l0 = l0; c.p_nt = nt_top; c.p_up_lds = 0; c.p_dn_lds = 0; c.p_up_full = 0; c.p_dn_maxns = 0; c.p_dn_maxnu = 0;
            c.p_up_off = (int)tab.size(); c.p_up_n = cnt;
            for (int l = l0; l < P.nLevels; l++) {
                const LevelPlan &L = c.levels[l];
                for (int k = 0; k < L.n_small; k++) tab.push_back(tab[L.small_off + k]);
                c.p_up_lds = std::max(c.p_up_lds, L.small_lds); c.p_up_full = std::max(c.p_up_full, L.full_limit);
                for (int k = 0; k < L.n_all; k++) { const int t = tab[L.all_off + k]; c.p_dn_lds = std::max(c.p_dn_lds, backsolve_lds(P.cols(t), 3 * P.f_nsb[t], true)); c.p_dn_maxns = std::max(c.p_dn_maxns, 3 * P.f_nsb[t]); c.p_dn_maxnu = std::max(c.p_dn_maxnu, P.cols(t) - 3 * P.f_nsb[t]); }
            }
            c.p_dn_off = (int)tab.size(); c.p_dn_n = cnt;
            for (int l = P.nLevels - 1; l >= l0; l--) { const LevelPlan &L = c.levels[l]; for (int k = 0; k < L.n_all; k++) tab.push_back(tab[L.all_off + k]); }
        }
    }
    c.x_up_n = c.x_dn_n = c.x_leaf_n = 0;
    if (c.persist_l0 >= 0 && g_opt.xcd_place) {
        int cus = 0;
        HIPCHECK(hipDeviceGetAttribute(&cus, hipDeviceAttributeMultiprocessorCount, physical_device(t_slot)));
        const int per_xcd = std::max(1, cus / 8);
        auto per_cu = [](size_t lds, int nt) { return std::max(1, std::min(2048 / std::max(nt, 64), (int)((160 * 1024) / std::max<size_t>(lds, 1)))); };
        const std::vector<int> up(tab.begin() + c.p_up_off, tab.begin() + c.p_up_off + c.p_up_n);
        const LevelPlan &L0 = c.levels[0];
        const bool leaf = c.persist_l0 == 1 && L0.n_big == 0 && L0.bs_gemv.grid == 0 && L0.bs_blk.grid == 0 && L0.n_small == L0.n_all;
        const std::vector<int> leaves = leaf ? std::vector<int>(tab.begin() + L0.small_off, tab.begin() + L0.small_off + L0.n_small) : std::vector<int>();
        const int cap = per_xcd * per_cu(c.p_up_lds, c.p_nt), cap_leaf = per_xcd * (((int)leaves.size() + 8 * per_xcd - 1) / (8 * per_xcd));
        const XcdLists x = xcd_place(up, leaves, P.f_parent.data(), P.f_nsb.data(), P.nF, cap, cap_leaf);
        c.x_up_off = (int)tab.size(); c.x_up_n = (int)x.up.size(); tab.insert(tab.end(), x.up.begin(), x.up.end());
        c.x_dn_off = (int)tab.size(); c.x_dn_n = (int)x.dn.size(); tab.insert(tab.end(), x.dn.begin(), x.dn.end());
        c.x_leaf_off = (int)tab.size(); c.x_leaf_n = (int)x.leaf.size(); tab.insert(tab.end(), x.leaf.begin(), x.leaf.end());
    }
    {
        const size_t stride = (size_t)P.nF + MAX_TAIL_FRONTS;
        const bool fresh = c.d_flags.need(3 * stride);
        c.d_flevel.need(stride);
        if (fresh || (size_t)c.flag_stride != stride) HIPCHECK(hipMemsetAsync(c.d_flags.p, 0, c.d_flags.cap * 4, s));
        c.flag_stride = (int)stride;
        if (c.d_marks.need(stride)) HIPCHECK(hipMemsetAsync(c.d_marks.p, 0, c.d_marks.cap * 4, s));
        if (c.d_epoch.need(1)) { HIPCHECK(hipMemcpyAsync(c.d_epoch.p, &FIRST_EPOCH, 4, hipMemcpyHostToDevice, s)); c.epoch_steps = 0; }
        d.epoch = c.d_epoch.p;
    }
    if (inc) { c.d_upd.need((size_t)g_opt.persist_max_fronts + 64); c.d_wbuf.need((size_t)1 << 19); }
    HIPCHECK(hipMemcpyAsync(c.d_flevel.p, P.f_level.data(), (size_t)P.nF * 4, hipMemcpyHostToDevice, s));
    if (tab.empty()) tab.push_back(0);
    c.d_tab.need(tab.size() + INC_TAB_);
    c.inc.tab_used = (long long)tab.size();
    c.base_tab = tab;
    const double u3 = uprof ? now_ms() : 0;
    HIPCHECK(hipMemcpyAsync(c.d_tab.p, tab.data(), tab.size() * 4, hipMemcpyHostToDevice, s));
    HIPCHECK(hipStreamSynchronize(s));
    const double u4 = uprof ? now_ms() : 0;

    const long long pool_slack = inc ? std::max<long long>(INC_POOL_MIN, P.pool_doubles / 4) : 0;
// ... 136 lines not shown
```

aprilsam_amd/csrc/solver_launch.inc.h:

```cpp

template <class K> static void allow_full_lds(K kern) { HIPCHECK(hipFuncSetAttribute((const void *)kern, hipFuncAttributeMaxDynamicSharedMemorySize, 160 * 1024)); }
static void set_small_attr() {
    static std::once_flag once[MAX_SLOTS];
    std::call_once(once[physical_device(t_slot) % MAX_SLOTS], [] {
        allow_full_lds(k_front_small<256>); allow_full_lds(k_front_small<512>); allow_full_lds(k_front_small<1024>);
        allow_full_lds(k_backsolve_t<false>); allow_full_lds(k_backsolve_t<true>); allow_full_lds(k_backsolve_w); allow_full_lds(k_backsolve_t<false, true>);
        allow_full_lds(k_block_chain); allow_full_lds(k_backsolve_blk); allow_full_lds(k_block_solve<1>); allow_full_lds(k_block_solve<2>);
        allow_full_lds(k_inc_one<256>); allow_full_lds(k_inc_one<512>); allow_full_lds(k_inc_one<1024>);
    });
}
template <class... Args> static void launch_front_small_nt(int nt, int grid, size_t lds, hipStream_t s, const Args &...a) {
    if (nt >= 1024) hipLaunchKernelGGL(k_front_small<1024>, dim3(grid), dim3(1024), lds, s, a...);
    else if (nt >= 512) hipLaunchKernelGGL(k_front_small<512>, dim3(grid), dim3(512), lds, s, a...);
    else hipLaunchKernelGGL(k_front_small<256>, dim3(grid), dim3(256), lds, s, a...);
}
template <class... Args> static void launch_inc_one_nt(int nt, size_t lds, hipStream_t s, const Args &...a) {
    if (nt >= 1024) hipLaunchKernelGGL(k_inc_one<1024>, dim3(1), dim3(1024), lds, s, a...);
    else if (nt >= 512) hipLaunchKernelGGL(k_inc_one<512>, dim3(1), dim3(512), lds, s, a...);
    else hipLaunchKernelGGL(k_inc_one<256>, dim3(1), dim3(256), lds, s, a...);
}

struct KTimer {
    Context *c = nullptr; hipStream_t s = nullptr; size_t nev = 0;
    int level = -1;
    void tic(int id) {
        if (!c) return;
        if (c->k_ev.size() < nev + 2) { c->k_ev.resize(nev + 2); HIPCHECK(hipEventCreate(&c->k_ev[nev])); HIPCHECK(hipEventCreate(&c->k_ev[nev + 1])); }
        HIPCHECK(hipEventRecord(c->k_ev[nev], s));
        c->k_ids.push_back(id); c->k_lev.push_back(level);
    }
    void toc() { if (c) { HIPCHECK(hipEventRecord(c->k_ev[nev + 1], s)); nev += 2; } }
};
static KTimer no_timer;

enum BsForm { BS_WAVE, BS_THREAD, BS_THREAD_TALL };
static void launch_backsolve_list(Context &c, hipStream_t s, BsForm form, const int *list, int n, size_t lds, int split, int *bad, const UpdArgs &upd) {
    if (form == BS_WAVE) hipLaunchKernelGGL(k_backsolve_w, dim3(n), dim3(TPB), lds, s, c.dp, list, c.d_pool.p, c.d_x.p, (int *)nullptr, bad, upd);
    else if (form == BS_THREAD_TALL) hipLaunchKernelGGL((k_backsolve_t<false, true>), dim3(n), dim3(TPB), lds, s, c.dp, list, c.d_pool.p, c.d_x.p, split, (int *)nullptr, 0, bad, upd);
    else hipLaunchKernelGGL((k_backsolve_t<false>), dim3(n), dim3(TPB), lds, s, c.dp, list, c.d_pool.p, c.d_x.p, split, (int *)nullptr, 0, bad, upd);
}

static void launch_backsolve(Context &c, const LevelPlan &L, hipStream_t s, KTimer &kt, const int *tab = nullptr, UpdArgs upd = UpdArgs{}, int list_off = -1, int list_n = 0) {
    if (!tab) tab = c.d_tab.p;
    if (!L.n_all) return;
    kt.tic(K_BACKSOLVE);
    if (L.bs_gemv.grid > 0)
        hipLaunchKernelGGL(k_backsolve_gemv, dim3(L.bs_gemv.grid), dim3(TPB), 0, s, c.dp, tab + L.bs_gemv.list_off, tab + L.bs_gemv.pre_off,
                           L.bs_gemv.n, c.d_pool.p, c.d_x.p);
    int n_all = list_off >= 0 ? list_n : L.n_all, all_off = list_off >= 0 ? list_off : L.all_off; size_t solve_lds = L.solve_lds;
    if (L.bs_blk.grid > 0) {
        hipLaunchKernelGGL(k_backsolve_blk, dim3(L.bs_blk.grid), dim3(TPB), L.bs_blk_lds, s, c.dp, tab + L.bs_blk.list_off, tab + L.bs_blk.pre_off, L.bs_blk.n,
                           c.d_pool.p, c.d_x.p, c.d_dinv.p, c.d_bsb_flags.p, c.d_bsb_far.p, L.bs_gemv.grid > 0 ? 1 : 0, c.d_bad.p, upd);
        n_all = L.n_rest; all_off = L.rest_off; solve_lds = L.rest_lds;
        if (!n_all) { kt.toc(); return; }
    }
    const bool wave = g_opt.wave_backsolve && L.bs_gemv.grid == 0 && L.n_all < g_opt.tp_fronts && L.maxns <= BSW_MAX_NS && L.solve_w_lds <= 80 * 1024;
    const BsForm form = wave ? BS_WAVE : solve_lds >= (size_t)(BS_TALL_ROWS + NB + 8 + NB * (NB + 1)) * 8 ? BS_THREAD_TALL : BS_THREAD;
    launch_backsolve_list(c, s, form, tab + all_off, n_all, wave ? L.solve_w_lds : solve_lds, L.bs_gemv.grid > 0 ? 1 : 0, c.d_bad.p, upd);
    kt.toc();
}

static int launch_xmode(const Context &c, int max_upd_rows) { return c.dp.xmode == X_TAGGED && max_upd_rows > TPB ? (int)X_FLUSH : c.dp.xmode; }
static int device_cus() {
    int cus = 0;
    HIPCHECK(hipDeviceGetAttribute(&cus, hipDeviceAttributeMultiprocessorCount, physical_device(t_slot)));
    return cus;
}
static size_t handover_lds(int xmode, size_t lds, int grid) {
    if (xmode == X_WT || (xmode == X_TAGGED && grid <= device_cus())) return std::max(lds, HANDOVER_LDS_MIN);
    return lds;
}
static DevPlan launch_plan(const Context &c, DevPlan d, int max_upd_rows) { d.xmode = launch_xmode(c, max_upd_rows); return d; }
static DevPlan persist_plan(const Context &c) { DevPlan d = c.dp; d.flevel = c.d_flevel.p; d.l0 = c.persist_l0; d.xmode = launch_xmode(c, c.p_dn_maxnu); return d; }
static void launch_backsolve_multi(Context &c, hipStream_t s, const DevPlan &dp, const int *list, int n, size_t lds, int maxns, int *xflags, const UpdArgs &upd) {
    lds = handover_lds(dp.xmode, lds, n);
    if (g_opt.wave_backsolve && maxns <= BSW_MAX_NS) hipLaunchKernelGGL(k_backsolve_w, dim3(n), dim3(TPB), lds, s, dp, list, c.d_pool.p, c.d_x.p, xflags, c.d_bad.p, upd);
    else hipLaunchKernelGGL((k_backsolve_t<true>), dim3(n), dim3(TPB), lds, s, dp, list, c.d_pool.p, c.d_x.p, 0, xflags, 1, c.d_bad.p, upd);
}

static void enqueue_poison(Context &c, hipStream_t s, const int *list, int n, int what = 3, const UpdRec *recs = nullptr) {
    if (g_opt.pool_poison <= 0 || n <= 0) return;
    static_assert(offsetof(UpdRec, mode) % 4 == 0 && sizeof(UpdRec) % 4 == 0, "UpdRec::mode as a strided int");
    hipLaunchKernelGGL(k_poison, dim3(n), dim3(TPB), 0, s, c.dp, list, n, recs ? (const int *)((const char *)recs + offsetof(UpdRec, mode)) : (const int *)nullptr,
                       (int)(sizeof(UpdRec) / 4), what, c.d_pool.p, c.d_x.p);
}
static void launch_front_persist(Context &c, hipStream_t s) {
    const bool xp = c.x_up_n > 0;
    const int *list = c.d_tab.p + (xp ? c.x_up_off : c.p_up_off), n = xp ? c.x_up_n : c.p_up_n;
    DevPlan dpe = persist_plan(c);
    if (g_opt.skip_flag_waits > 0) dpe.l0 = 1 << 30;
    launch_front_small_nt(c.p_nt, n, c.p_up_lds, s, dpe, list, c.d_pool.p, c.d_H.p, c.d_bad.p, c.p_up_full, c.d_flags.p, 1);
}

static void launch_front_small(Context &c, const LevelPlan &L, hipStream_t s, const int *tab = nullptr, int list_off = -1, int list_n = 0) {
    if (!tab) tab = c.d_tab.p;
    const int off = list_off >= 0 ? list_off : L.small_off, n = list_off >= 0 ? list_n : L.n_small;
    launch_front_small_nt(L.small_nt, n, L.small_lds, s, c.dp, tab + off, c.d_pool.p, c.d_H.p, c.d_bad.p, L.full_limit, (int *)nullptr, 0);
}

static void enqueue_big_steps(Context &c, const LevelPlan &L, hipStream_t s, KTimer &kt, const int *tab = nullptr) {
    if (!tab) tab = c.d_tab.p;
    const int xcd = std::max(0, g_opt.syrk_xcd_order) << SYRK_MODE_XCD_SHIFT;
    for (size_t o = 0; o < L.bchain.size(); o++) {
        const Launch &bc = L.bchain[o], &bt = L.btile[o], &sw = L.syrkw[o];
        kt.tic(K_PANEL_BIG);
        hipLaunchKernelGGL(k_block_chain, dim3(bc.n), dim3(BCH_THREADS), block_chain_lds(), s, c.dp, tab + bc.list_off, (int)o, c.d_pool.p, c.d_diag.p, c.d_dinv.p, c.d_bad.p);
        if (bt.grid > 0) {
            if (bt.tile == 2) hipLaunchKernelGGL(k_block_solve<2>, dim3(bt.grid), dim3(TPB), block_solve_lds(), s, c.dp, tab + bt.list_off, tab + bt.pre_off, bt.n, (int)o, c.d_pool.p, c.d_diag.p, c.d_dinv.p);
            else hipLaunchKernelGGL(k_block_solve<1>, dim3(bt.grid), dim3(TPB), block_solve_lds(), s, c.dp, tab + bt.list_off, tab + bt.pre_off, bt.n, (int)o, c.d_pool.p, c.d_diag.p, c.d_dinv.p);
        }
        kt.toc();
        auto wide = [&](const Launch &w, int s_lo, int s_hi, int mode) {
            if (w.grid <= 0) return;
            kt.tic(K_SYRK_BIG);
            if (w.tile == TILE / 2) hipLaunchKernelGGL(k_syrk_big32, dim3(w.grid), dim3(TPB), 0, s, c.dp, tab + w.list_off, tab + w.pre_off, w.n, s_lo, s_hi, mode | xcd, c.d_pool.p);
            else hipLaunchKernelGGL(k_syrk_big, dim3(w.grid), dim3(TPB), 0, s, c.dp, tab + w.list_off, tab + w.pre_off, w.n, s_lo, s_hi, mode | xcd, c.d_pool.p);
            kt.toc();
        };
        const int G = std::max(2, g_opt.syrk_group), g0 = (int)(o - o % G) * OBP;
        if (!L.paired) wide(sw, (int)o * OBP, (int)(o + 1) * OBP, 1);
        else if ((int)(o % G) != G - 1) { wide(L.syrka[o], g0, (int)(o + 1) * OBP, 2); wide(L.syrk1[o], g0, (int)(o + 1) * OBP, 1); }
        else wide(sw, g0, (int)(o + 1) * OBP, 1);
    }
}

static void enqueue_factor_level(Context &c, const LevelPlan &L, hipStream_t s, KTimer &kt, const int *tab = nullptr) {
    if (!tab) tab = c.d_tab.p;
    if (L.n_small) {
        kt.tic(K_FRONT_SMALL);
        launch_front_small(c, L, s, tab);
        kt.toc();
    }
    if (L.n_big) {
        kt.tic(K_ASSEMBLE_BIG);
        hipLaunchKernelGGL(k_assemble_big, dim3(L.asm_big.grid), dim3(TPB), L.asm_lds, s, c.dp, tab + L.asm_big.list_off,
                           tab + L.asm_big.pre_off, L.asm_big.n, c.d_pool.p, c.d_H.p);
        kt.toc();
        enqueue_big_steps(c, L, s, kt, tab);
    }
}

template <class K, class... Args> static void launch_gnc(hipStream_t s, GraphPack &gp, K kern, const Args &...a) {
    hipLaunchKernelGGL(kern, dim3((gp.gc_n + TPB - 1) / TPB), dim3(TPB), 0, s, gp.gc_n, (const int *)gp.d_gc_f.p, (const double *)gp.d_gc_W0.p, (const GncPar *)gp.d_gc_par.p, a...);
}
static void enqueue_gnc_weight(GraphPack &gp, hipStream_t s, const double *upt) {
    if (gp.gc_n == 0) return;
    launch_gnc(s, gp, k_gnc_weight, (const int *)gp.d_fa.p, (const int *)gp.d_fb.p, (const double *)gp.d_z.p, (const double *)gp.d_lp.p, (const double *)gp.d_state.p, upt, gp.d_W.p, gp.d_gc_w.p);
}

static void enqueue_linearise(Context &c, GraphPack &gp, hipStream_t s, bool unary_at_lp) {
    const int F = c.plan.F;
    enqueue_select(gp, s);
    enqueue_robust(gp, s, unary_at_lp ? gp.d_upt.p : (const double *)nullptr);
    enqueue_gnc_weight(gp, s, unary_at_lp ? gp.d_upt.p : (const double *)nullptr);
    auto launch = [&](auto kern) {
        hipLaunchKernelGGL(kern, dim3((F + TPB - 1) / TPB), dim3(TPB), 0, s, 0, F, (const int *)nullptr, gp.d_fa.p, gp.d_fb.p, gp.d_z.p, gp.d_W.p,
                           gp.d_lp.p, gp.d_state.p, c.d_swap.p, c.dp.slot_blk, c.dp.slot_rhs, c.d_H.p, c.d_bad.p, unary_at_lp ? gp.d_upt.p : (const double *)nullptr, c.d_epoch.p);
    };
    if (F >= g_opt.linearize_staged_min) launch(k_linearize_t<true>); else launch(k_linearize_t<false>);
    if (!gp.host_idx.empty()) {
        const int nh = (int)gp.host_idx.size();
        HIPCHECK(hipMemcpyAsync(gp.d_hostH.p, gp.h_hostH.p, (size_t)33 * 8 * nh, hipMemcpyHostToDevice, s));
        hipLaunchKernelGGL(k_scatter_host, dim3((nh + TPB - 1) / TPB), dim3(TPB), 0, s, nh, gp.d_host_idx.p, gp.d_hostH.p, gp.d_fb.p, c.d_swap.p,
                           c.dp.slot_blk, c.dp.slot_rhs, c.d_H.p);
    }
}

struct NumericArgs {
    hipEvent_t *ev = nullptr;
    bool unary_at_lp = false;
    bool ktime = false;
    bool io_host = false;
    bool relin = false;
    double *st_dest = nullptr;
    const std::function<void()> *fill = nullptr;
};
static void enqueue_numeric(Context &c, GraphPack &gp, hipStream_t s, const NumericArgs &a = NumericArgs{}) {
    const Plan &P = c.plan;
    const int N = P.N;
    const bool io_host = a.io_host;
    KTimer kt;
    if (a.ktime) { c.k_ids.clear(); c.k_lev.clear(); kt.c = &c; kt.s = s; }
    if (a.ev) HIPCHECK(hipEventRecord(a.ev[0], s));
    if (c.dp.prof) HIPCHECK(hipMemsetAsync(c.d_prof.p, 0, (size_t)8 * PROF_SLOTS * P.nF, s));
    if (io_host) hipLaunchKernelGGL(k_load_states, dim3((3 * N + TPB - 1) / TPB), dim3(TPB), 0, s, 3 * N, gp.h_state.p, gp.d_state.p, gp.d_lp.p);
    enqueue_poison(c, s, nullptr, P.nF);
    kt.tic(K_LINEARIZE);
    if (a.fill) (*a.fill)(); else enqueue_linearise(c, gp, s, a.unary_at_lp);
    kt.toc();
    if (a.ev) HIPCHECK(hipEventRecord(a.ev[1], s));
    const int l0 = c.persist_l0 >= 0 ? c.persist_l0 : P.nLevels;
    for (int l = 0; l < l0; l++) {
        kt.level = l;
        if (l == 0 && c.x_leaf_n > 0) { kt.tic(K_FRONT_SMALL); launch_front_small(c, c.levels[0], s, nullptr, c.x_leaf_off, c.x_leaf_n); kt.toc(); }
        else enqueue_factor_level(c, c.levels[l], s, kt);
    }
    kt.level = l0;
    if (l0 < P.nLevels) { kt.tic(K_FRONT_SMALL); launch_front_persist(c, s); kt.toc(); }
    if (a.ev) HIPCHECK(hipEventRecord(a.ev[2], s));
    UpdArgs upd{ c.d_perm.p, gp.d_lp.p, a.st_dest ? a.st_dest : gp.d_state.p, gp.d_dx.p, io_host ? gp.h_lp.p : nullptr, io_host ? gp.h_dx.p : nullptr, nullptr, a.relin ? gp.d_lp.p : nullptr };
    if (l0 < P.nLevels) {
        UpdArgs u = upd; if (l0 == 0) u.bad_out = io_host ? c.h_bad.p : nullptr;
        kt.tic(K_BACKSOLVE);
        const bool xp = c.x_dn_n > 0;
        launch_backsolve_multi(c, s, persist_plan(c), c.d_tab.p + (xp ? c.x_dn_off : c.p_dn_off), xp ? c.x_dn_n : c.p_dn_n, c.p_dn_lds, c.p_dn_maxns, c.d_flags.p + c.flag_stride, u);
        kt.toc();
    }
    for (int l = l0 - 1; l >= 0; l--) {
        UpdArgs u = upd; if (l == 0) u.bad_out = io_host ? c.h_bad.p : nullptr;
        kt.level = l;
        if (l == 0 && c.x_leaf_n > 0) launch_backsolve(c, c.levels[0], s, kt, nullptr, u, c.x_leaf_off, c.x_leaf_n);
        else launch_backsolve(c, c.levels[l], s, kt, nullptr, u);
    }
    if (a.ev) HIPCHECK(hipEventRecord(a.ev[3], s));
    HIPCHECK(hipGetLastError());
}
static void collect_kernel_times(Context &c) {
    for (size_t i = 0; i < c.k_ids.size(); i++) {
        float ms = 0;
        HIPCHECK(hipEventElapsedTime(&ms, c.k_ev[2 * i], c.k_ev[2 * i + 1]));
        c.k_ms[c.k_ids[i]] += ms; c.k_calls[c.k_ids[i]]++;
        const int l = i < c.k_lev.size() ? c.k_lev[i] : -1;
        if (l >= 0) {
            if (c.lev_up_ms.size() <= (size_t)l) { c.lev_up_ms.resize(l + 1, 0.0); c.lev_dn_ms.resize(l + 1, 0.0); }
            (c.k_ids[i] == K_BACKSOLVE ? c.lev_dn_ms : c.lev_up_ms)[l] += ms;
        }
    }
    c.k_ids.clear();
}

template <class Enqueue> static void replay_captured(Context &c, hipGraphExec_t &exec, hipStream_t s, Enqueue enqueue) {
    if (!exec) {
        hipGraph_t graph = nullptr;
        HIPCHECK(hipStreamBeginCapture(s, hipStreamCaptureModeThreadLocal));
        enqueue();
        HIPCHECK(hipStreamEndCapture(s, &graph));
        HIPCHECK(hipGraphInstantiate(&exec, graph, nullptr, nullptr, 0));
        HIPCHECK(hipGraphDestroy(graph));
        c.n_captures++;
    }
    c.graph_stream = s;
    HIPCHECK(hipGraphLaunch(exec, s));
}

long long graph_captures(const april_graph_cholesky_param_t *param) {
    SlotLock lk(param, nullptr);
    auto it = g_ctx.find(param);
    return it == g_ctx.end() ? -1 : it->second->n_captures;
}

struct RunArgs { bool timing = false, unary_at_lp = false, io_host = false, relin = false; };
static void run_numeric(Context &c, GraphPack &gp, const RunArgs &r = RunArgs{}) {
    hipStream_t s = gp.stream;
    set_small_attr();
    rewind_epoch(c, s, 1);
    if (r.timing && !c.have_events) { for (auto &e : c.ev) HIPCHECK(hipEventCreate(&e)); c.have_events = true; }
    NumericArgs a;
    a.io_host = r.io_host;
    if (!r.io_host) a.relin = r.relin;
    const bool graph = g_opt.use_graph && !r.timing && gp.host_idx.empty();
    if (r.io_host && graph) {
        const void *key[9] = { gp.d_state.p, gp.h_state.p, gp.h_lp.p, gp.h_dx.p, c.h_bad.p, (const void *)(size_t)gp.N, (const void *)(size_t)gp.serial, (const void *)(size_t)gp.mx_gen,
                               (const void *)(size_t)gp.rb_gen };
        if (memcmp(key, c.api_key, sizeof(key)) != 0) { c.retire(c.gexec_api); memcpy(c.api_key, key, sizeof(key)); c.api_key_runs = 0; }
        if (c.api_key_runs++ == 0) enqueue_numeric(c, gp, s, a);
        else replay_captured(c, c.gexec_api, s, [&] { enqueue_numeric(c, gp, s, a); });
    } else if (!r.io_host && graph && !r.unary_at_lp) {
        if (c.gexec_key != (const void *)gp.d_state.p || c.gexec_serial != gp.serial || c.gexec_mx != gp.mx_gen || c.gexec_rb != gp.rb_gen) {
            c.retire(c.gexec);
            c.gexec_key = (const void *)gp.d_state.p; c.gexec_serial = gp.serial; c.gexec_mx = gp.mx_gen; c.gexec_rb = gp.rb_gen;
        }
        replay_captured(c, c.gexec, s, [&] { enqueue_numeric(c, gp, s, a); });
    } else {
        a.ev = r.timing ? c.ev : nullptr;
        if (!r.io_host) a.unary_at_lp = r.unary_at_lp;
        enqueue_numeric(c, gp, s, a);
    }
}
```

aprilsam_amd/csrc/solver_pack.inc.h:

```cpp
static std::atomic<long long> g_pack_serial{ 0 };
static void forget_stream(hipStream_t s);
constexpr int STREAM_POOL_MAX = 4;
static std::mutex g_stream_pool_mu;
static std::vector<hipStream_t> g_stream_pool[MAX_SLOTS];
static hipStream_t take_stream(int slot) {
    {
        std::lock_guard<std::mutex> lk(g_stream_pool_mu);
        auto &v = g_stream_pool[slot];
        if (!v.empty()) { hipStream_t s = v.back(); v.pop_back(); return s; }
    }
    hipStream_t s = nullptr;
    HIPCHECK(hipStreamCreateWithFlags(&s, hipStreamNonBlocking));
    return s;
}
static void park_stream(int slot, hipStream_t s) {
    if (hipStreamSynchronize(s) == hipSuccess) {
        std::lock_guard<std::mutex> lk(g_stream_pool_mu);
        auto &v = g_stream_pool[slot];
        if ((int)v.size() < STREAM_POOL_MAX) { v.push_back(s); return; }
    } else (void)hipGetLastError();
    (void)hipStreamDestroy(s);
}
struct GraphPack {
    int slot = 0;
    const long long serial = ++g_pack_serial;
    int N = 0, F = 0;
    int Fg = 0;
    std::vector<int> g2p, p2g;
    std::vector<unsigned> vslot;
    std::vector<const void *> fptr;
    std::vector<int> pending;
    HBuf<int> h_fa, h_fb;
    HBuf<double> h_z, h_W, h_state, h_lp, h_dx;
    DBuf<int> d_fa, d_fb;
    DBuf<double> d_z, d_W, d_state, d_lp, d_dx, d_chi2f, d_scalar;
    DBuf<double> d_lp_last; bool lp_last_valid = false;
    int F_on_device = 0;
    int dirty_lo = 0, dirty_hi = 0;
    long long content_version = 0;
    long long topo_version = 0;
    std::vector<unsigned char> asym; int n_asym = 0;
    void note_asym(int p, const double *w, bool device_factor) {
        const unsigned char a = device_factor && (w[1] != w[3] || w[2] != w[6] || w[5] != w[7]);
        if ((size_t)p >= asym.size()) asym.resize((size_t)p + 1, 0);
        n_asym += (int)a - (int)asym[p]; asym[p] = a;
    }
    std::vector<char> is_host;
    std::vector<double> h_upt; DBuf<double> d_upt;
    int F_cap = 0;
    std::vector<int> host_idx; HBuf<double> h_hostH; DBuf<double> d_hostH; DBuf<int> d_host_idx; int host_evaluated = 0;
    std::vector<int> mx_f, mx_k{ 0 }, mx_sel, mx_of; std::vector<double> mx_z, mx_W, mx_c, mx_logw;
    DBuf<int> d_mx_f, d_mx_k, d_sel; DBuf<double> d_mx_z, d_mx_W, d_mx_c; HBuf<double> mx_stage;
    int mx_on_device = 0; bool mx_dirty = false; long long mx_gen = 0;
    int n_max() const { return (int)mx_f.size(); }
    void mx_clear() {
        if (!mx_f.empty() || mx_on_device) mx_gen++;
        mx_f.clear(); mx_k.assign(1, 0); mx_sel.clear(); mx_of.clear(); mx_z.clear(); mx_W.clear(); mx_c.clear(); mx_logw.clear(); mx_on_device = 0; mx_dirty = false; }
    std::vector<int> rb_f, rb_kind, rb_of; std::vector<double> rb_c, rb_W0, rb_w;
    DBuf<int> d_rb_f, d_rb_kind; DBuf<double> d_rb_c, d_rb_W0, d_rb_w; HBuf<double> rb_stage;
    int rb_on_device = 0; bool rb_dirty = false; long long rb_gen = 0;
    int n_robust() const { return (int)rb_f.size(); }
    void rb_clear() {
        if (!rb_f.empty() || rb_on_device) rb_gen++;
        rb_f.clear(); rb_kind.clear(); rb_of.clear(); rb_c.clear(); rb_W0.clear(); rb_w.clear(); rb_on_device = 0; rb_dirty = false; }
    DBuf<int> d_gc_f; DBuf<double> d_gc_W0, d_gc_w, d_gc_out; DBuf<GncPar> d_gc_par; HBuf<double> gc_stage;
    int gc_n = 0; long long gc_gen = 0;
    hipStream_t stream = nullptr;
    HBuf<double> h_scalar;
    HBuf<double> h_out; bool mirror_sync = false; std::vector<int> changed; const double *new_states = nullptr;
    void release() {
        h_out.release(); mirror_sync = false;
        h_fa.release(); h_fb.release(); h_z.release(); h_W.release(); h_state.release(); h_lp.release(); h_dx.release();
        d_fa.release(); d_fb.release(); d_z.release(); d_W.release(); d_state.release(); d_lp.release(); d_lp_last.release(); d_dx.release();
        d_chi2f.release(); d_scalar.release(); h_scalar.release(); h_hostH.release(); d_hostH.release(); d_host_idx.release(); d_upt.release();
        d_mx_f.release(); d_mx_k.release(); d_sel.release(); d_mx_z.release(); d_mx_W.release(); d_mx_c.release(); mx_stage.release(); mx_clear();
        d_rb_f.release(); d_rb_kind.release(); d_rb_c.release(); d_rb_W0.release(); d_rb_w.release(); rb_stage.release(); rb_clear();
        d_gc_f.release(); d_gc_W0.release(); d_gc_w.release(); d_gc_out.release(); d_gc_par.release(); gc_stage.release(); gc_n = 0;
        if (stream) { forget_stream(stream); park_stream(slot, stream); }
        stream = nullptr;
    }
};

static Registry<GraphPack> g_packs;

static int slot_of_graph(const void *g) {
    int slot = -1;
    g_packs.with(g, [&](GraphPack &gp) { slot = gp.slot; });
    return slot;
}
static GraphPack &pack_for(const april_graph_t *g) {
    auto it = g_packs.find(g);
    if (it != g_packs.end() && it->second->slot != t_slot) {
        const int os = it->second->slot;
        std::unique_lock<std::mutex> old_slot(g_slot_mu[os], std::try_to_lock);
        for (const auto t0 = std::chrono::steady_clock::now(); !old_slot.owns_lock(); (void)old_slot.try_lock()) {
            if (std::chrono::steady_clock::now() - t0 > std::chrono::seconds(10))
                fail(ERR_UNSUPPORTED, "graph %p was last solved on device slot %d, which other threads kept busy for 10 s: one graph is driven from one slot at a "
                     "time (the call on slot %d did nothing)", (const void *)g, os, t_slot);
            std::this_thread::sleep_for(std::chrono::microseconds(20));
        }
        it = g_packs.find(g);
        if (it != g_packs.end() && it->second->slot != t_slot) { it->second->release(); g_packs.erase(it); it = g_packs.end(); }
    }
    if (it == g_packs.end()) {
        auto p = std::make_unique<GraphPack>();
        p->slot = t_slot;
        p->stream = take_stream(t_slot);
        it = g_packs.emplace(g, std::move(p)).first;
    }
    return *it->second;
}
void drop_graph_pack(const april_graph_t *g) {
    SlotLock lk(nullptr, g);
    auto it = g_packs.find(g);
    if (it != g_packs.end()) { it->second->release(); g_packs.erase(it); }
}

static inline int zsize(const zarray_t *z) { return z ? z->size : 0; }

static void pack_factors(GraphPack &gp, const april_graph_t *g, bool validate_old = true) {
    const bool trust = g_opt.trust_factor_cache || !validate_old;
    const int Fg = zsize(g->factors);
    april_graph_factor_t **fs = (april_graph_factor_t **)g->factors->data;
    const int N = zsize(g->nodes);
    int from = gp.Fg;
    bool valid = from <= Fg && (int)gp.fptr.size() == from && (int)gp.g2p.size() == from + 1;
    if (valid && trust) valid = from == 0 || (validate_old ? memcmp(gp.fptr.data(), fs, sizeof(void *) * from) == 0 : (gp.fptr[0] == fs[0] && gp.fptr[from - 1] == fs[from - 1]));
    auto restart = [&]() { gp.topo_version++; from = 0; gp.F = 0; gp.F_on_device = 0; gp.host_idx.clear(); gp.host_evaluated = 0; gp.is_host.clear(); gp.p2g.clear(); gp.vslot.clear(); gp.g2p.assign(1, 0); gp.asym.clear(); gp.n_asym = 0; gp.mx_clear(); gp.rb_clear(); };
    if (!valid) restart();
    struct Ent { int a, b; bool host; unsigned short slots; unsigned char carry; };
    Ent ents[64]; int ne = 0; bool is_max = false, is_rb = false; int rb_kind = 0; double rb_c = 0;
    auto classify = [&](const april_graph_factor_t *f, int i) {
        ne = 0; is_max = false; is_rb = false;
        if (is_native_max(f)) {
            char why[192];
            if (f->nnodes != 2 || !max_check(f, why, sizeof why)) fail(ERR_UNSUPPORTED, "factor %d: max factor: %s", i, f->nnodes != 2 ? "not binary" : why);
            ents[ne++] = Ent{ f->nodes[0], f->nodes[1], false, 0, 3 }; is_max = true;
        } else if (f->type == APRIL_GRAPH_FACTOR_XYT_TYPE && f->nnodes == 2) { ents[ne++] = Ent{ f->nodes[0], f->nodes[1], false, 0, 3 }; is_rb = robust_of(f, &rb_kind, &rb_c); }
        else if (f->type == APRIL_GRAPH_FACTOR_XYTPOS_TYPE && f->nnodes == 1) { ents[ne++] = Ent{ f->nodes[0], -1, false, 0, 3 }; is_rb = robust_of(f, &rb_kind, &rb_c); }
        else if ((f->nnodes == 1 || f->nnodes == 2) && f->eval)
            ents[ne++] = Ent{ f->nodes[0], f->nnodes == 2 ? f->nodes[1] : -1, true, (unsigned short)(f->nnodes == 2 ? 1 : 0xff), 3 };
        else if (f->nnodes >= 3 && f->nnodes <= 11 && f->eval) {
            for (int x = 0; x < f->nnodes; x++)
                for (int y = x + 1; y < f->nnodes; y++) {
                    const unsigned char carry = (unsigned char)(((x == 0 && y == 1) ? 1 : 0) | ((x == 0) ? 2 : 0));
                    ents[ne++] = Ent{ f->nodes[x], f->nodes[y], true, (unsigned short)((x << 8) | y), carry };
                }
        } else {
            fail(ERR_UNSUPPORTED, "factor %d has type %d / %d nodes; factors of foreign types are supported with 1 to 11 nodes and an "
                                  "eval() function pointer (aprilsam.h:110-122)", i, f->type, f->nnodes);
        }
        if (is_rb && !robust_spd(f->u.common.W->data))
            fail(ERR_UNSUPPORTED, "factor %d: a robust factor's W must be symmetric positive definite (DESIGN.md section 15)", i);
        for (int e = 0; e < ne; e++) {
            if (ents[e].a < 0 || ents[e].a >= N || ents[e].b >= N || (f->nnodes >= 2 && ents[e].b < 0))
                fail(ERR_BAD_GRAPH, "factor %d references node %d / %d of %d", i, ents[e].a, ents[e].b, N);
// ... 400 lines not shown
```

aprilsam_amd/csrc/solver_resident.inc.h:

```cpp
static int resident_begin_impl(april_graph_t *g, april_graph_cholesky_param_t *param);
int resident_begin(april_graph_t *g, april_graph_cholesky_param_t *param) { return guarded_rc(param, g, [&] { return resident_begin_impl(g, param); }); }
static int resident_begin_impl(april_graph_t *g, april_graph_cholesky_param_t *param) {
    if (zsize(g->nodes) == 0 || zsize(g->factors) == 0) return -1;
    ensure_device();
    SlotLock lk(param, g);
    Context &c = ctx_for(param);
    GraphPack &gp = pack_for(g);
    pack_factors(gp, g);
    if (!gp.host_idx.empty()) return -4;
    pack_states(gp, g, false);
    gp.lp_last_valid = false;
    orient_asymmetric(c, gp);
    const bool reused = prepare_plan(c, gp, g);
    flush_orientation(c, gp.stream);
    upload_factors(gp);
    set_lambda(c, gp, param->tikhanov);
    if (!c.have_events) { for (auto &e : c.ev) HIPCHECK(hipEventCreate(&e)); c.have_events = true; }
    for (int k = 0; k < NKERN; k++) { c.k_ms[k] = 0; c.k_calls[k] = 0; }
    c.lev_up_ms.clear(); c.lev_dn_ms.clear();
    c.st.n_nodes = gp.N; c.st.n_factors = gp.F; c.st.symbolic_reused = reused; c.st.not_spd = 0;
    HIPCHECK(hipStreamSynchronize(gp.stream));
    return 0;
}
static int resident_steps_impl(april_graph_t *g, april_graph_cholesky_param_t *param, int n, int mode);
int resident_steps(april_graph_t *g, april_graph_cholesky_param_t *param, int n, int mode) { return guarded_rc(param, g, [&] { return resident_steps_impl(g, param, n, mode); }); }
static int resident_steps_impl(april_graph_t *g, april_graph_cholesky_param_t *param, int n, int mode) {
    SlotLock lk(param, g);
    auto it = g_ctx.find(param);
    if (it == g_ctx.end() || !it->second->have_plan) return -1;
    Context &c = *it->second;
    GraphPack &gp = pack_for(g);
    hipStream_t s = gp.stream;
    const int N = gp.N;
    set_small_attr();
    gp.mirror_sync = false;
    HIPCHECK(hipMemcpyAsync(gp.d_lp.p, gp.d_state.p, (size_t)24 * N, hipMemcpyDeviceToDevice, s));
    for (int i = 0; i < n; i++) {
        if (i == n - 1) {
            gp.d_lp_last.need((size_t)3 * N);
            HIPCHECK(hipMemcpyAsync(gp.d_lp_last.p, gp.d_lp.p, (size_t)24 * N, hipMemcpyDeviceToDevice, s));
            gp.lp_last_valid = true;
        }
        if (mode == 1) {
            NumericArgs a; a.ktime = true; a.relin = true;
            enqueue_numeric(c, gp, s, a);
            HIPCHECK(hipStreamSynchronize(s));
            collect_kernel_times(c);
        } else {
            RunArgs r; r.relin = true;
            run_numeric(c, gp, r);
        }
    }
    return 0;
}
static int resident_sync_impl(april_graph_t *g, april_graph_cholesky_param_t *param);
int resident_sync(april_graph_t *g, april_graph_cholesky_param_t *param) { return guarded_rc(param, g, [&] { return resident_sync_impl(g, param); }); }
static int resident_sync_impl(april_graph_t *g, april_graph_cholesky_param_t *param) {
    SlotLock lk(param, g);
    auto it = g_ctx.find(param);
    if (it == g_ctx.end()) return -1;
    Context &c = *it->second;
    GraphPack &gp = pack_for(g);
    HIPCHECK(hipMemcpyAsync(c.h_bad.p, c.d_bad.p, 16, hipMemcpyDeviceToHost, gp.stream));
    HIPCHECK(hipStreamSynchronize(gp.stream));
    check_bad(c);
    check_guard(c, gp.stream);
    if (c.h_bad.p[0] && getenv("APRILSAM_AMD_DEBUG")) {
        const int t = c.h_bad.p[1];
        fprintf(stderr, "aprilsam_amd: bad pivot: front %d kernel %d step %d", t, c.h_bad.p[2], c.h_bad.p[3]);
        if (t >= 0 && t < c.plan.nF) fprintf(stderr, " (nsb %d nub %d level %d off %lld)", c.plan.f_nsb[t], c.plan.f_nub[t], c.plan.f_level[t], (long long)c.plan.f_off[t]);
        fprintf(stderr, "\n");
    }
    return c.h_bad.p[0] ? -2 : 0;
}
static double resident_chi2_impl(april_graph_t *g);
double resident_chi2(april_graph_t *g) {
    double out = std::nan("");
    guarded(nullptr, g, [&] { out = resident_chi2_impl(g); });
    return out;
}
static double resident_chi2_impl(april_graph_t *g) {
    SlotLock lk(nullptr, g);
    return device_chi2(pack_for(g));
}
static int resident_end_impl(april_graph_t *g, april_graph_cholesky_param_t *param);
int resident_end(april_graph_t *g, april_graph_cholesky_param_t *param) { return guarded_rc(param, g, [&] { return resident_end_impl(g, param); }); }
static int resident_end_impl(april_graph_t *g, april_graph_cholesky_param_t *param) {
    SlotLock lk(param, g);
    auto it = g_ctx.find(param);
    if (it == g_ctx.end()) return -1;
    Context &c = *it->second;
    GraphPack &gp = pack_for(g);
    hipStream_t s = gp.stream;
    const int N = gp.N, F = gp.F;
    HIPCHECK(hipMemcpyAsync(gp.h_state.p, gp.d_state.p, (size_t)24 * N, hipMemcpyDeviceToHost, s));
    if (gp.lp_last_valid && gp.d_lp_last.cap >= (size_t)3 * N) HIPCHECK(hipMemcpyAsync(gp.d_lp.p, gp.d_lp_last.p, (size_t)24 * N, hipMemcpyDeviceToDevice, s));
    gp.lp_last_valid = false;
    HIPCHECK(hipMemcpyAsync(gp.h_lp.p, gp.d_lp.p, (size_t)24 * N, hipMemcpyDeviceToHost, s));
    HIPCHECK(hipMemcpyAsync(gp.h_dx.p, gp.d_dx.p, (size_t)24 * N, hipMemcpyDeviceToHost, s));
    HIPCHECK(hipStreamSynchronize(s));
    april_graph_node_t **ns = (april_graph_node_t **)g->nodes->data;
    for (int i = 0; i < N; i++) {
        april_graph_node_t *n = ns[i];
        n->UID = i;
        memcpy(n->state, gp.h_state.p + (size_t)3 * i, 24);
        memcpy(n->l_point, gp.h_lp.p + (size_t)3 * i, 24);
        const double *dx = gp.h_dx.p + (size_t)3 * i;
        if (!(std::isnan(dx[0]) || std::isnan(dx[1]) || std::isnan(dx[2]))) memcpy(n->delta_X, dx, 24);
    }
    if (param->ordering) free(param->ordering);
    param->ordering = (int *)malloc(sizeof(int) * (size_t)N);
    memcpy(param->ordering, c.plan.perm.data(), sizeof(int) * (size_t)N);
    param->nreordering = N; param->factor_num = gp.Fg;
    c.have_fact = true; c.batch_nodes = N; c.batch_factors = F; c.model.valid = false;
    record_factor(c, c.inc.t_first.empty() ? FACT_PLAN : FACT_EXTENDED, gp);
    inc_prepare(c); c.inc_F = F; c.inc_N = N;
    record_unary_points(gp, 0, F, gp.h_lp.p);
    return 0;
}
int batch_resident(april_graph_t *g, april_graph_cholesky_param_t *param, int iters, double *chi2_out, double *ms_out) {
    int rc = resident_begin(g, param);
    if (rc) return rc;
    if (chi2_out) chi2_out[0] = resident_chi2(g);
    for (int it = 0; it < iters && rc == 0; it++) {
        const double t0 = now_ms();
        resident_steps(g, param, 1, 0);
        rc = resident_sync(g, param);
        if (ms_out) ms_out[it] = now_ms() - t0;
        if (rc == 0 && chi2_out) chi2_out[it + 1] = resident_chi2(g);
    }
    if (rc == 0) rc = resident_end(g, param);
    return rc;
}
int level_profile(const april_graph_cholesky_param_t *param, double *out, int cap_levels) {
    SlotLock lk(param, nullptr);
    auto it = g_ctx.find(param);
    if (it == g_ctx.end() || !it->second->have_plan) return -1;
    Context &c = *it->second;
    const Plan &P = c.plan;
    for (int l = 0; l < P.nLevels && l < cap_levels; l++) {
        double *o = out + 6 * l;
        o[0] = l < (int)c.lev_up_ms.size() ? c.lev_up_ms[l] : 0.0; o[1] = l < (int)c.lev_dn_ms.size() ? c.lev_dn_ms[l] : 0.0;
        o[2] = P.lev_ptr[l + 1] - P.lev_ptr[l]; o[3] = l < (int)c.levels.size() ? c.levels[l].n_big : 0; o[4] = 0; o[5] = 0;
        for (int k = P.lev_ptr[l]; k < P.lev_ptr[l + 1]; k++) {
            const int t = P.lev_fronts[k];
            const double ns = 3.0 * P.f_nsb[t], nu = 3.0 * P.f_nub[t];
            o[4] = std::max(o[4], ns);
            o[5] += ns * (nu + 1) * (nu + 1) + ns * ns * (nu + 1) + ns * ns * ns / 3.0;
        }
    }
    return P.nLevels;
}
int debug_guard_selftest(const april_graph_cholesky_param_t *param) {
    return guarded_rc(param, nullptr, [&]() -> int {
        SlotLock lk(param, nullptr);
        auto it = g_ctx.find(param);
        if (it == g_ctx.end() || !it->second->have_plan || it->second->n_guard <= 0) return -1;
        Context &c = *it->second;
        const long long inside = c.plan.f_off[0];
        HIPCHECK(hipMemcpy(c.d_guard.p, &inside, 8, hipMemcpyHostToDevice));
        check_guard(c, nullptr);
        return 0;
    });
}
int kernel_profile(const april_graph_cholesky_param_t *param, double *ms, long long *calls, double *flops, double *bytes, const char **names) {
    SlotLock lk(param, nullptr);
    auto it = g_ctx.find(param);
    if (it == g_ctx.end() || !it->second->have_plan) return -1;
    Context &c = *it->second;
    const Plan &P = c.plan;
    for (int k = 0; k < NKERN; k++) { ms[k] = c.k_ms[k]; calls[k] = c.k_calls[k]; flops[k] = 0; bytes[k] = 0; if (names) names[k] = KNAMES[k]; }
    const size_t small_max = (size_t)g_opt.small_lds_kb * 1024;
    for (int t = 0; t < P.nF; t++) {
        const double ns = 3.0 * P.f_nsb[t], nu = 3.0 * P.f_nub[t], R = P.rows(t), C = P.cols(t);
        double fl = 0;
        for (int q = 0; q < (int)ns; q++) { double cj = (ns - q) + nu + 1; fl += cj * cj; }
        const int nwp = waves_of(small_threads_for((size_t)(P.lev_ptr[P.f_level[t] + 1] - P.lev_ptr[P.f_level[t]])));
        const bool small = small_front_lds((int)R, (int)C, nwp) <= small_max || (g_opt.panel_mode && panel_front_lds((int)R, (int)ns, nwp) <= small_max);
        const double by = 8.0 * (ns * (ns + 1) / 2 + (nu + 1) * ns + (nu + 1) * (nu + 2) / 2);
        if (small) { flops[K_FRONT_SMALL] += fl; bytes[K_FRONT_SMALL] += by; }
        else {
            const double Rv = R - 2;
            double fsy = 0;
            auto trapezoid = [&](double c_lo, double c_hi) { const double n = c_hi - c_lo; return n <= 0 ? 0.0 : n * Rv - (c_lo + c_hi - 1) * n / 2; };
            const int steps = ((int)ns + NB - 1) / NB;
            for (int o = 0; o * OBP < steps; o++) {
                const double k_lo = (double)o * OBP * NB, k_hi = std::min<double>(ns, (double)(o + 1) * OBP * NB);
                fsy += 2.0 * (k_hi - k_lo) * trapezoid(k_hi, C);
            }
            fsy = std::min(fsy, fl);
            flops[K_SYRK_BIG] += fsy; flops[K_PANEL_BIG] += fl - fsy;
            bytes[K_SYRK_BIG] += by; bytes[K_ASSEMBLE_BIG] += by;
        }
        bytes[K_BACKSOLVE] += 8.0 * (ns * (ns + 1) / 2 + nu * ns) + 16.0 * (ns + nu);
        flops[K_BACKSOLVE] += 2.0 * (ns * (ns + 1) / 2 + nu * ns);
    }
    int F2 = 0, F1 = 0;
    for (int f = 0; f < P.F; f++) (c.pat[2 * f + 1] >= 0 ? F2 : F1)++;
    bytes[K_LINEARIZE] = F2 * 152.0 + F1 * 124.0 + 8.0 * (27.0 * F2 + 9.0 * F1 + 6.0 * F2 + 3.0 * F1);
    flops[K_LINEARIZE] = 150.0 * F2 + 40.0 * F1;
    bytes[K_UPDATE] = 8.0 * 3 * P.N * 4;
    return NKERN;
}

static int debug_stage_impl(april_graph_t *g, april_graph_cholesky_param_t *param, int what, double *out);
int debug_stage(april_graph_t *g, april_graph_cholesky_param_t *param, int what, double *out) { return guarded_rc(param, g, [&] { return debug_stage_impl(g, param, what, out); }); }
static int debug_stage_impl(april_graph_t *g, april_graph_cholesky_param_t *param, int what, double *out) {
    if (zsize(g->nodes) == 0 || zsize(g->factors) == 0) return -1;
    ensure_device();
    SlotLock lk(param, g);
    Context &c = ctx_for(param);
    GraphPack &gp = pack_for(g);
    pack_factors(gp, g);
    if (!gp.host_idx.empty()) return -4;
    pack_states(gp, g, false);
    orient_asymmetric(c, gp);
    prepare_plan(c, gp, g);
    flush_orientation(c, gp.stream);
    upload_factors(gp);
    const Plan &P = c.plan;
    const int N = gp.N, F = gp.F;
    hipStream_t s = gp.stream;
    gp.mirror_sync = false;
    HIPCHECK(hipMemcpyAsync(gp.d_lp.p, gp.d_state.p, (size_t)24 * N, hipMemcpyDeviceToDevice, s));
    enqueue_select(gp, s);
    enqueue_robust(gp, s, nullptr);
    hipLaunchKernelGGL((k_linearize_t<false>), dim3((F + TPB - 1) / TPB), dim3(TPB), 0, s, 0, F, (const int *)nullptr, gp.d_fa.p, gp.d_fb.p, gp.d_z.p, gp.d_W.p,
                       gp.d_lp.p, gp.d_state.p, c.d_swap.p, c.dp.slot_blk, c.dp.slot_rhs, c.d_H.p, c.d_bad.p, (const double *)nullptr);
    if (what == 0) {
        std::vector<double> H((size_t)9 * std::max(1, P.n_slots));
        HIPCHECK(hipMemcpyAsync(H.data(), c.d_H.p, H.size() * 8, hipMemcpyDeviceToHost, s));
        HIPCHECK(hipStreamSynchronize(s));
        for (int f = 0; f < F; f++) {
            double *o = out + (size_t)33 * f;
            memset(o, 0, 33 * 8);
            memcpy(o, &H[(size_t)9 * P.slot_blk[3 * f]], 72);
            memcpy(o + 27, &H[(size_t)9 * P.slot_rhs[2 * f]], 24);
            if (gp.h_fb.p[f] < 0) continue;
            const double *b1 = &H[(size_t)9 * P.slot_blk[3 * f + 1]];
            for (int i = 0; i < 3; i++) for (int j = 0; j < 3; j++) o[9 + i * 3 + j] = P.fac_swap[f] ? b1[j * 3 + i] : b1[i * 3 + j];
            memcpy(o + 18, &H[(size_t)9 * P.slot_blk[3 * f + 2]], 72);
            memcpy(o + 30, &H[(size_t)9 * P.slot_rhs[2 * f + 1]], 24);
        }
        return 0;
    }
    if (what != 1 || N > 2000) return -2;
    const int nd = (int)P.dest.size();
    DBuf<double> d_out; d_out.need((size_t)9 * std::max(1, nd));
    hipLaunchKernelGGL(k_debug_dest, dim3((9 * nd + TPB - 1) / TPB), dim3(TPB), 0, s, nd, c.dp.dest, c.dp.src_idx, c.d_H.p, d_out.p);
    std::vector<double> D((size_t)9 * std::max(1, nd));
    HIPCHECK(hipMemcpyAsync(D.data(), d_out.p, D.size() * 8, hipMemcpyDeviceToHost, s));
    HIPCHECK(hipStreamSynchronize(s));
    d_out.release();
    const size_t n = (size_t)3 * N;
    double *A = out, *B = out + n * n;
    memset(out, 0, (n * n + n) * 8);
    for (int t = 0; t < P.nF; t++) {
        auto node_of = [&](int lb) { const int pos = lb < P.f_nsb[t] ? P.f_first[t] + lb : P.f_rows[P.f_rows_ptr[t] + lb - P.f_nsb[t]]; return P.perm[pos]; };
        for (int d = P.dest_front_ptr[t]; d < P.dest_front_ptr[t + 1]; d++) {
            const Plan::DestRec &r = P.dest[d];
            const double *v = &D[(size_t)9 * d];
            const int nc = node_of(r.bcol);
            if (r.brow < 0) { for (int j = 0; j < 3; j++) B[(size_t)3 * nc + j] += v[j]; continue; }
            const int nr = node_of(r.brow);
            for (int i = 0; i < 3; i++)
                for (int j = 0; j < 3; j++) {
                    if (r.brow == r.bcol && i < j) continue;
                    const size_t rr = (size_t)3 * nr + i, cc = (size_t)3 * nc + j;
                    A[rr * n + cc] += v[i * 3 + j];
                    if (rr != cc) A[cc * n + rr] += v[i * 3 + j];
                }
        }
    }
    for (size_t i = 0; i < n; i++) A[i * n + i] += param->tikhanov > 0 ? param->tikhanov : 0.0;
    return 0;
}

int debug_front_times(const april_graph_cholesky_param_t *param, long long *out, int n_fronts) {
    return guarded_rc(param, nullptr, [&]() -> int {
        SlotLock lk(param, nullptr);
        auto it = g_ctx.find(param);
        if (it == g_ctx.end() || !it->second->d_prof.p) return -1;
        HIPCHECK(hipDeviceSynchronize());
        int n = std::min(n_fronts, it->second->plan.nF);
        HIPCHECK(hipMemcpy(out, it->second->d_prof.p, (size_t)8 * PROF_SLOTS * n, hipMemcpyDeviceToHost));
        return n;
    });
}
```

aprilsam_amd/csrc/symbolic.cpp:

```cpp
#include "plan.h"
#include "solver.h"
#include "errors.h"

#include <algorithm>
#include <atomic>
#include <cassert>
#include <cstdio>
#include <cstdlib>
#include <tuple>
#include <chrono>
#include <mutex>

namespace asam {

static void amalgamate(NDTree &tree, int N, const std::vector<int> &ap, const std::vector<int> &ai, int max_own, size_t lds_budget) {
    const double HAND = 12.0 + 2.7, PERCOL = 0.19 + 0.8 / 64.0;
    constexpr int REGION_MAX = 4096;
    const int nT = (int)tree.nodes.size();
    std::vector<int> order; order.reserve(nT);
    {
        std::vector<std::pair<int, size_t>> st;
        for (int r : tree.roots) {
            st.push_back({ r, 0 });
            while (!st.empty()) {
// ... 126 lines not shown
                NDTree::Node &nd = tree.nodes[top.first];
                if (top.second < nd.children.size()) { int c = nd.children[top.second++]; st.push_back({ c, 0 }); continue; }
                int t = nextfront++;
                tfront[top.first] = t;
                P.f_first[t] = nextpos; P.f_nsb[t] = (int)nd.verts.size();
                for (int v : nd.verts) { P.perm[nextpos] = v; P.pos[v] = nextpos; nextpos++; }
                st.pop_back();
            }
        }
        assert(nextpos == N && nextfront == nT);
    }
    std::vector<int> pos_front(N);
    for (int t = 0; t < nT; t++) for (int k = 0; k < P.f_nsb[t]; k++) pos_front[P.f_first[t] + k] = t;

    stamp();
    P.f_nub.assign(nT, 0); P.f_parent.assign(nT, -1); P.f_rows_ptr.assign(nT + 1, 0);
    std::vector<std::vector<int>> kids(nT);
    std::vector<int> mark(N, -1), tmp;
    std::vector<std::vector<int>> strct(nT);
    for (int t = 0; t < nT; t++) {
        const int last = P.f_first[t] + P.f_nsb[t] - 1;
        tmp.clear();
        for (int p = P.f_first[t]; p <= last; p++) {
            int v = P.perm[p];
            for (int e = ap[v]; e < ap[v + 1]; e++) { int q = P.pos[ai[e]]; if (q > last && mark[q] != t) { mark[q] = t; tmp.push_back(q); } }
        }
        for (int c : kids[t]) for (int q : strct[c]) if (q > last && mark[q] != t) { mark[q] = t; tmp.push_back(q); }
        std::sort(tmp.begin(), tmp.end());
        strct[t] = tmp;
        P.f_nub[t] = (int)tmp.size();
        if (!tmp.empty()) { int par = pos_front[tmp[0]]; assert(par > t); P.f_parent[t] = par; kids[par].push_back(t); }
    }
    for (int t = 0; t < nT; t++) P.f_rows_ptr[t + 1] = P.f_rows_ptr[t] + P.f_nub[t];
    P.f_rows.resize(P.f_rows_ptr[nT]); P.f_rel.assign(P.f_rows_ptr[nT], -1);
    for (int t = 0; t < nT; t++) std::copy(strct[t].begin(), strct[t].end(), P.f_rows.begin() + P.f_rows_ptr[t]);

    auto local_index = [&](int t, int p) -> int {
        if (p >= P.f_first[t] && p < P.f_first[t] + P.f_nsb[t]) return p - P.f_first[t];
        const int *b = P.f_rows.data() + P.f_rows_ptr[t], *e = b + P.f_nub[t];
        const int *it = std::lower_bound(b, e, p);
        if (it == e || *it != p) return -1;
        return P.f_nsb[t] + (int)(it - b);
    };
    for (int t = 0; t < nT; t++) {
        int par = P.f_parent[t];
        for (int64_t k = P.f_rows_ptr[t]; k < P.f_rows_ptr[t + 1]; k++) {
            int li = local_index(par, P.f_rows[k]);
            if (li < 0) fail(ERR_INTERNAL, "symbolic inconsistency (front %d row %d)", t, P.f_rows[k]);
            P.f_rel[k] = li;
        }
    }
    P.ch_ptr.assign(nT + 1, 0);
    for (int t = 0; t < nT; t++) P.ch_ptr[t + 1] = P.ch_ptr[t] + (int)kids[t].size();
    P.ch_idx.resize(P.ch_ptr[nT]);
    for (int t = 0; t < nT; t++) std::copy(kids[t].begin(), kids[t].end(), P.ch_idx.begin() + P.ch_ptr[t]);

    stamp();
    P.f_level.assign(nT, 0);
    for (int t = 0; t < nT; t++) { int par = P.f_parent[t]; if (par >= 0) P.f_level[par] = std::max(P.f_level[par], P.f_level[t] + 1); }
    P.nLevels = 0;
    for (int t = 0; t < nT; t++) P.nLevels = std::max(P.nLevels, P.f_level[t] + 1);
    P.lev_ptr.assign(P.nLevels + 1, 0);
    for (int t = 0; t < nT; t++) P.lev_ptr[P.f_level[t] + 1]++;
    for (int l = 0; l < P.nLevels; l++) P.lev_ptr[l + 1] += P.lev_ptr[l];
    P.lev_fronts.resize(nT);
    { std::vector<int> fill(P.lev_ptr.begin(), P.lev_ptr.end() - 1); for (int t = 0; t < nT; t++) P.lev_fronts[fill[P.f_level[t]]++] = t; }

    stamp();
    P.fac_front.assign(F, -1); P.fac_la.assign(F, -1); P.fac_lb.assign(F, -1); P.fac_swap.assign(F, 0);
    std::atomic<int> lost{ -1 };
    plan_parallel_for(F, 4096, [&](int f0, int f1) {
        for (int f = f0; f < f1; f++) {
            int a = fn[2 * f], b = fn[2 * f + 1];
            if (a < 0 || a >= N || b >= N || a == b) continue;
            int pa = P.pos[a], pb = b >= 0 ? P.pos[b] : -1;
            int t = pos_front[(pb >= 0 && pb < pa) ? pb : pa];
            int la = local_index(t, pa), lb = pb >= 0 ? local_index(t, pb) : -1;
            if (la < 0 || (pb >= 0 && lb < 0)) { lost.store(f); continue; }
            P.fac_front[f] = t; P.fac_la[f] = la; P.fac_lb[f] = lb;
        }
    });
    if (lost.load() >= 0) fail(ERR_INTERNAL, "factor %d not inside its front", lost.load());
    for (int f = 0; f < F; f++) if (P.fac_front[f] >= 0 && P.fac_lb[f] >= 0) P.fac_swap[f] = P.fac_la[f] < P.fac_lb[f];
    constexpr int KEY_SRC_BITS = 30, KEY_ROW_BITS = 17, KEY_COL_BITS = 16;
    static_assert(1 + KEY_SRC_BITS + KEY_ROW_BITS + KEY_COL_BITS == 64 && sizeof(unsigned long long) == 8, "packed sort keys");
    if ((size_t)3 * F >= (1u << KEY_SRC_BITS) || (size_t)5 * F >= 0x7fffffffu)
        fail(ERR_UNSUPPORTED, "%d factors: this build handles up to %u (packed sort keys of the symbolic analysis)", F, (1u << KEY_SRC_BITS) / 3 - 1);
    for (int t = 0; t < nT; t++)
        if (P.f_nsb[t] + P.f_nub[t] + 1 >= (1 << KEY_COL_BITS))
            fail(ERR_UNSUPPORTED, "front %d has %d block rows: this build handles up to %d (packed sort keys of the symbolic analysis)", t, P.f_nsb[t] + P.f_nub[t] + 1, (1 << KEY_COL_BITS) - 1);
    P.bd_front_ptr.clear(); P.rd_front_ptr.clear();

    stamp();
    {
        std::vector<int> ptr(nT + 1, 0);
        for (int f = 0; f < F; f++) if (P.fac_front[f] >= 0) ptr[P.fac_front[f] + 1] += P.fac_lb[f] >= 0 ? 5 : 2;
        for (int t = 0; t < nT; t++) ptr[t + 1] += ptr[t];
        const size_t total = (size_t)ptr[nT];
        std::vector<unsigned long long> key(total);
        auto pack = [](int col, int row, int src, int rhs) {
            return ((unsigned long long)(unsigned)col << (1 + KEY_SRC_BITS + KEY_ROW_BITS)) | ((unsigned long long)(unsigned)(row + 1) << (1 + KEY_SRC_BITS)) | ((unsigned long long)(unsigned)src << 1) | (unsigned)rhs;
        };
        {
            std::vector<int> fill(ptr.begin(), ptr.end() - 1);
            for (int f = 0; f < F; f++) {
                const int t = P.fac_front[f], la = P.fac_la[f], lb = P.fac_lb[f];
                if (t < 0) continue;
                int &w = fill[t];
                key[w++] = pack(la, la, 3 * f + 0, 0); key[w++] = pack(la, -1, 2 * f + 0, 1);
                if (lb >= 0) {
                    key[w++] = pack(std::min(la, lb), std::max(la, lb), 3 * f + 1, 0);
                    key[w++] = pack(lb, lb, 3 * f + 2, 0); key[w++] = pack(lb, -1, 2 * f + 1, 1);
                }
            }
        }
        auto same_dest = [](unsigned long long a, unsigned long long b) { return (a >> (1 + KEY_SRC_BITS)) == (b >> (1 + KEY_SRC_BITS)); };
        P.dest_front_ptr.assign(nT + 1, 0);
        plan_parallel_for(nT, 64, [&](int t0, int t1) {
            for (int t = t0; t < t1; t++) {
                std::sort(key.begin() + ptr[t], key.begin() + ptr[t + 1]);
                int fresh = 0;
                for (int i = ptr[t]; i < ptr[t + 1]; i++) fresh += i == ptr[t] || !same_dest(key[i], key[i - 1]);
                P.dest_front_ptr[t + 1] = fresh;
            }
        });
        for (int t = 0; t < nT; t++) P.dest_front_ptr[t + 1] += P.dest_front_ptr[t];
        P.dest.resize((size_t)P.dest_front_ptr[nT]);
        P.slot_blk.assign((size_t)3 * F, -1); P.slot_rhs.assign((size_t)2 * F, -1);
        plan_parallel_for(nT, 64, [&](int t0, int t1) {
            for (int t = t0; t < t1; t++) {
                int d = P.dest_front_ptr[t] - 1;
                for (int i = ptr[t]; i < ptr[t + 1]; i++) {
                    const unsigned long long k = key[i];
                    const int col = (int)(k >> (1 + KEY_SRC_BITS + KEY_ROW_BITS)), row = (int)((k >> (1 + KEY_SRC_BITS)) & ((1u << KEY_ROW_BITS) - 1)) - 1,
                              src = (int)((k >> 1) & ((1u << KEY_SRC_BITS) - 1)), rhs = (int)(k & 1);
                    if (i == ptr[t] || !same_dest(k, key[i - 1])) P.dest[++d] = { row, col, i, i };
                    P.dest[d].src_end = i + 1;
                    (rhs ? P.slot_rhs : P.slot_blk)[src] = i;
                }
            }
        });
        P.n_slots = (int)total;
    }

    stamp();
    P.f_off.assign(nT, 0);
    int64_t off = 0;
    P.max_rows = 0; P.nnzL = 0; P.flops = 0;
    for (int t = 0; t < nT; t++) {
        P.f_off[t] = off;
        int64_t sz = (int64_t)P.rows(t) * P.cols(t);
        off += (sz + 31) & ~int64_t(31);
        int ns = 3 * P.f_nsb[t], nu = 3 * P.f_nub[t];
        P.max_rows = std::max(P.max_rows, ns + nu);
        P.nnzL += (int64_t)ns * (ns + 1) / 2 + (int64_t)nu * ns;
        for (int q = 0; q < ns; q++) { double c = (double)(ns - q) + nu; P.flops += c * c; }
    }
    P.pool_doubles = off;
    stamp();
    if (prof && nph == 8)
        fprintf(stderr, "aprilsam_amd planner N=%d F=%d: adjacency %.3f dissection %.3f front structure %.3f levels %.3f factor lists %.3f records+slots %.3f offsets %.3f | total %.3f ms\n",
                N, F, tph[1] - tph[0], tph[2] - tph[1], tph[3] - tph[2], tph[4] - tph[3], tph[5] - tph[4], tph[6] - tph[5], tph[7] - tph[6], tph[7] - tph[0]);
}

void build_gather_lists(Plan &P) {
    if (!P.bd_front_ptr.empty()) return;
// ... 150 lines not shown
```

include/aprilsam_amd.h:

```cpp
#ifndef APRILSAM_AMD_H
#define APRILSAM_AMD_H

#include <stddef.h>
#include <stdint.h>

#ifdef __cplusplus
extern "C" {
#endif


typedef struct zarray {
    size_t el_sz;
    int    size;
    int    alloc;
    char  *data;
} zarray_t;

typedef struct matd {
    unsigned int nrows, ncols;
    double       data[];
} matd_t;

typedef struct april_graph {
    zarray_t   *factors;
// ... 54 lines not shown
    void       *impl;
    const void *stype;
};

typedef struct april_graph_cholesky_param {
    double  tikhanov;
    void   *chol;
    int     factor_num;
    int    *ordering;
    int     nreordering;
    int     show_timing;
    double *delta_x;
    double *B;
    double *y;
    void   *A;
    void   *tr;
    double  l_thresh;
    double  delta_thresh;
    int     nthreshold;
    double  batch_time;
    double  delta_xy;
    double  delta_theta;
} april_graph_cholesky_param_t;


void APRILSAM_VERSION(void);
void april_graph_cholesky_param_init(april_graph_cholesky_param_t *param);
void april_graph_cholesky_param_destory(april_graph_cholesky_param_t *param);
void april_graph_cholesky(april_graph_t *graph, april_graph_cholesky_param_t *param);
void april_graph_cholesky_inc(april_graph_t *graph, april_graph_cholesky_param_t *param);
void april_graph_cholesky_inc_solver(april_graph_t *graph, april_graph_cholesky_param_t *param, int *idxs);
double april_graph_chi2(april_graph_t *graph);

april_graph_t *april_graph_create(void);
void           april_graph_destroy(april_graph_t *graph);
april_graph_node_t   *april_graph_node_xyt_create(const double *state, const double *init, const double *truth);
april_graph_factor_t *april_graph_factor_xyt_create(int a, int b, const double *z, const double *ztruth, const matd_t *W);
april_graph_factor_t *april_graph_factor_xytpos_create(int a, double *z, double *ztruth, matd_t *W);
void april_graph_factor_eval_destroy(april_graph_factor_eval_t *eval);
int  april_graph_dof(april_graph_t *graph);
int            april_graph_save(april_graph_t *graph, const char *path);
april_graph_t *april_graph_create_from_file(const char *path);
void           april_graph_stype_init(void);


void aprilsam_amd_graph_add_node(april_graph_t *graph, april_graph_node_t *node);
void aprilsam_amd_graph_add_factor(april_graph_t *graph, april_graph_factor_t *factor);

int         aprilsam_amd_attr_put_string(void **attr_slot, const char *key, const char *value);
const char *aprilsam_amd_attr_get_string(const void *attr, const char *key);
int         aprilsam_amd_attr_count(const void *attr);
int         aprilsam_amd_attr_item(const void *attr, int i, const char **key, const char **value);

int            aprilsam_amd_graph_save(april_graph_t *graph, const char *path);
int            aprilsam_amd_graph_save_ex(april_graph_t *graph, const char *path, unsigned long long magic_offset);
april_graph_t *aprilsam_amd_graph_load(const char *path);

int aprilsam_amd_selftest(void);

int aprilsam_amd_device_count(void);
int aprilsam_amd_set_device(int device);
int aprilsam_amd_param_set_device(const april_graph_cholesky_param_t *param, int slot);
int aprilsam_amd_param_get_device(const april_graph_cholesky_param_t *param);

typedef struct aprilsam_amd_stats {
    int    n_nodes, n_factors;
    int    n_fronts, n_levels;
    int    max_front_rows;
    int    symbolic_reused;
    int    not_spd;
    int    reserved0;
    long long nnz_L;
    double flops_factor;
    double bytes_fronts;
    double ms_pack, ms_symbolic, ms_h2d, ms_device, ms_d2h, ms_unpack, ms_total;
    double ms_dev_linearize, ms_dev_factor, ms_dev_solve;
    double chi2_before;
    int    error_code;
    int    reserved1;
    int    inc_replanned;
    int    inc_old_old_cross;
    int    inc_fronts_updated;
    int    dn_launch_fronts;
} aprilsam_amd_stats_t;
int aprilsam_amd_get_stats(const april_graph_cholesky_param_t *param, aprilsam_amd_stats_t *out);

int  aprilsam_amd_last_error(char *msg, int cap);
void aprilsam_amd_clear_error(void);

int aprilsam_amd_set_option(const char *name, double value);
int aprilsam_amd_debug_guard_selftest(const april_graph_cholesky_param_t *param);
int aprilsam_amd_get_option(const char *name, double *value);

int aprilsam_amd_batch_resident(april_graph_t *graph, april_graph_cholesky_param_t *param, int iters,
                                double *chi2_out, double *ms_out);

int    aprilsam_amd_resident_begin(april_graph_t *graph, april_graph_cholesky_param_t *param);
int    aprilsam_amd_resident_steps(april_graph_t *graph, april_graph_cholesky_param_t *param, int n, int mode);
int    aprilsam_amd_resident_sync(april_graph_t *graph, april_graph_cholesky_param_t *param);
double aprilsam_amd_resident_chi2(april_graph_t *graph);
int    aprilsam_amd_resident_end(april_graph_t *graph, april_graph_cholesky_param_t *param);
int aprilsam_amd_kernel_profile(const april_graph_cholesky_param_t *param, double *ms, long long *calls,
                                double *flops, double *bytes, const char **names);
int aprilsam_amd_level_profile(const april_graph_cholesky_param_t *param, double *out6, int cap_levels);

int aprilsam_amd_marginals(april_graph_t *graph, april_graph_cholesky_param_t *param, int n, const int *nodes, double *cov);
int aprilsam_amd_marginals_joint(april_graph_t *graph, april_graph_cholesky_param_t *param, int n, const int *a, const int *b, double *cov);
long long aprilsam_amd_debug_selinv_runs(const april_graph_cholesky_param_t *param);

int aprilsam_amd_marginals_joint_any(april_graph_t *graph, april_graph_cholesky_param_t *param, int n, const int *a, const int *b, double *cov);
int aprilsam_amd_gate_xyt(april_graph_t *graph, april_graph_cholesky_param_t *param, int n, const int *a, const int *b, const double *z,
                          const double *W, double *d2, double *S);
long long aprilsam_amd_debug_path_solve_bytes(const april_graph_cholesky_param_t *param);

typedef struct {
    int    max_iters;
    int    check_every;
    double lambda0;
    double lambda_max;
    double eta;
    double ftol;
    double xtol;
} aprilsam_amd_lm_opts_t;
void aprilsam_amd_lm_opts_init(aprilsam_amd_lm_opts_t *opts);

enum { APRILSAM_AMD_LM_CONVERGED_F = 1, APRILSAM_AMD_LM_CONVERGED_X = 2, APRILSAM_AMD_LM_STALLED = 3, APRILSAM_AMD_LM_MAX_ITERS = 4 };
typedef struct {
    int    status, iterations, accepted, rejected_not_spd;
    double F_initial, F_final;
    double chi2_final;
    double lambda_final;
} aprilsam_amd_lm_report_t;

int aprilsam_amd_optimize_lm(april_graph_t *graph, april_graph_cholesky_param_t *param, const aprilsam_amd_lm_opts_t *opts,
                             aprilsam_amd_lm_report_t *report, double *trace);

typedef struct {
    int    stages;
} aprilsam_amd_chordal_opts_t;
void aprilsam_amd_chordal_opts_init(aprilsam_amd_chordal_opts_t *opts);
typedef struct {
    int    status;
    int    n_degenerate;
    int    not_spd_stage;
    double min_norm;
    double F_initial, F_final;
} aprilsam_amd_chordal_report_t;
int aprilsam_amd_initialize_chordal(april_graph_t *graph, april_graph_cholesky_param_t *param, const aprilsam_amd_chordal_opts_t *opts,
                                    aprilsam_amd_chordal_report_t *report, double *rot_out);
int aprilsam_amd_debug_chordal_raw(april_graph_t *graph, april_graph_cholesky_param_t *param, const aprilsam_amd_chordal_opts_t *opts,
                                   aprilsam_amd_chordal_report_t *report, double *raw);

#define APRILSAM_AMD_FACTOR_MAX_TYPE 3
april_graph_factor_t *aprilsam_amd_factor_max_create(april_graph_factor_t **components, const double *logw, int n);
int aprilsam_amd_max_selected(april_graph_t *graph, april_graph_cholesky_param_t *param, int n, const int *factors, int *out);

enum { APRILSAM_AMD_ROBUST_NONE = 0, APRILSAM_AMD_ROBUST_HUBER = 1, APRILSAM_AMD_ROBUST_CAUCHY = 2, APRILSAM_AMD_ROBUST_DCS = 3 };
int aprilsam_amd_factor_set_robust(april_graph_factor_t *factor, int kind, double c);
int aprilsam_amd_factor_get_robust(const april_graph_factor_t *factor, int *kind, double *c);
int aprilsam_amd_robust_weights(april_graph_t *graph, april_graph_cholesky_param_t *param, int n, const int *factors, double *w);

enum { APRILSAM_AMD_GNC_GM = 1, APRILSAM_AMD_GNC_TLS = 2 };
typedef struct {
    int    loss;
    double c;
    double mu_step;
// ... 71 lines not shown
```

Baseline: 4971 GN iterations/s.

## Fuse next-iteration relinearization into the backsolve tail for resident GN steps

Result: no change. 4996 GN iterations/s, median of 6 (+0.5%).

```diff
diff --git a/aprilsam_amd/abi.py b/aprilsam_amd/abi.py
--- a/aprilsam_amd/abi.py
+++ b/aprilsam_amd/abi.py
@@ -70,7 +70,8 @@
                 ("ms_device", C.c_double), ("ms_d2h", C.c_double), ("ms_unpack", C.c_double),
                 ("ms_total", C.c_double), ("ms_dev_linearize", C.c_double), ("ms_dev_factor", C.c_double),
                 ("ms_dev_solve", C.c_double), ("chi2_before", C.c_double), ("error_code", C.c_int), ("reserved1", C.c_int),
-                ("inc_replanned", C.c_int), ("inc_old_old_cross", C.c_int), ("inc_fronts_updated", C.c_int), ("dn_launch_fronts", C.c_int)]
+                ("inc_replanned", C.c_int), ("inc_old_old_cross", C.c_int), ("inc_fronts_updated", C.c_int), ("dn_launch_fronts", C.c_int),
+                ("fused_steps", C.c_int), ("reserved2", C.c_int)]
 
     def asdict(self):
         return {k: getattr(self, k) for k, _ in self._fields_}
diff --git a/aprilsam_amd/csrc/capi.cpp b/aprilsam_amd/csrc/capi.cpp
--- a/aprilsam_amd/csrc/capi.cpp
+++ b/aprilsam_amd/csrc/capi.cpp
@@ -183,6 +183,8 @@
     else if (k == "factor_la") from(P.fac_la);
     else if (k == "factor_lb") from(P.fac_lb);
     else if (k == "factor_swap") from(P.fac_swap);
+    else if (k == "front_fac_ptr") from(P.ff_ptr);
+    else if (k == "front_fac") from(P.ff_idx);
     else if (k == "bd_front_ptr") from(P.bd_front_ptr);
     else if (k == "bd_row") from(P.bd_row);
     else if (k == "bd_col") from(P.bd_col);
diff --git a/aprilsam_amd/csrc/kernels.hip.h b/aprilsam_amd/csrc/kernels.hip.h
--- a/aprilsam_amd/csrc/kernels.hip.h
+++ b/aprilsam_amd/csrc/kernels.hip.h
@@ -24,7 +24,7 @@
     int parent;
     int dinv0;
     int prim1, prim2;
-    int pad[2];
+    int ff_begin, ff_end;
 };
 static_assert(sizeof(FrontDesc) == 64, "FrontDesc must stay one cache line");
 struct DestRec { int brow, bcol, src_begin, src_end; };
@@ -219,7 +219,8 @@
                                                  const double *__restrict__ lp, const double *__restrict__ st,
                                                  const unsigned char *__restrict__ swp, const int *__restrict__ slot_blk,
                                                  const int *__restrict__ slot_rhs, double *__restrict__ Hc, const double *__restrict__ upt,
-                                                 double (*stg)[STAGED ? 64 * LIN_STRIDE : 1], int (*sid)[STAGED ? 128 : 1], double *mirror = nullptr) {
+                                                 double (*stg)[STAGED ? 64 * LIN_STRIDE : 1], int (*sid)[STAGED ? 128 : 1], double *mirror = nullptr,
+                                                 bool pts_in = false, double a0 = 0, double a1 = 0, double a2 = 0, double b0 = 0, double b1 = 0, double b2 = 0) {
     int f = f_begin + gtid;
     bool active = f < f_end;
     if (!STAGED && !active) return;
@@ -233,12 +234,17 @@
 #pragma unroll
     for (int k = 0; k < 3; k++) z[k] = Z[(size_t)3 * f + k];
     const bool binary = b >= 0;
-    const double *src = binary ? lp + (size_t)3 * a : (upt ? upt + (size_t)3 * f : st + (size_t)3 * a);
-#pragma unroll
-    for (int k = 0; k < 3; k++) pa[k] = src[k];
-    if (binary) {
-#pragma unroll
-        for (int k = 0; k < 3; k++) pb[k] = lp[(size_t)3 * b + k];
+    if (pts_in) {
+        pa[0] = a0; pa[1] = a1; pa[2] = a2;
+        if (binary) { pb[0] = b0; pb[1] = b1; pb[2] = b2; }
+    } else {
+        const double *src = binary ? lp + (size_t)3 * a : (upt ? upt + (size_t)3 * f : st + (size_t)3 * a);
+#pragma unroll
+        for (int k = 0; k < 3; k++) pa[k] = src[k];
+        if (binary) {
+#pragma unroll
+            for (int k = 0; k < 3; k++) pb[k] = lp[(size_t)3 * b + k];
+        }
     }
     factor_residual(binary, pa, pb, z, J0, J1, r);
     const int wave = threadIdx.x >> 6, lane = threadIdx.x & 63;
@@ -1828,9 +1834,38 @@
 }
 
 __host__ __device__ inline size_t backsolve_lds(int m, int ns, bool pre) { return (size_t)(m + NB + 8 + NB * (NB + 1) + (pre ? (size_t)ns * ((m + 3) | 1) : 0)) * 8; }
-struct UpdArgs { const int *perm; const double *lp; double *st, *dX, *st_out, *dx_out; int *bad_out; double *lp_next; };
+struct RelinTail {
+    const int4 *ff;
+    const int *fa, *fb; const double *Z, *Wm; const unsigned char *swp; double *Hc;
+    const double *lpz; double *lpz_next;
+    int *bad_clear, *epoch_adv;
+};
+struct UpdArgs { const int *perm; const double *lp; double *st, *dX, *st_out, *dx_out; int *bad_out; double *lp_next; RelinTail rt; };
+__device__ __forceinline__ bool next_point(const double *l, double d0, double d1, double d2, double (&s)[3]) {
+    if (isnan(d0) || isnan(d1) || isnan(d2)) { s[0] = l[0]; s[1] = l[1]; s[2] = l[2]; return false; }
+    s[0] = l[0] + d0; s[1] = l[1] + d1; s[2] = mod2pi_dev(l[2] + d2);
+    return true;
+}
+struct RelinPre { int f, la, lb, a, b; double a0, a1, a2, b0, b1, b2; };
+__device__ __forceinline__ void relin_tail(const DevPlan &P, const FrontDesc &D_, const double *xw, const RelinTail &rt, const RelinPre &pre) {
+    auto one = [&](int f, int la, int lb, const double *la3, const double *lb3) {
+        double pa[3], pb[3] = { 0, 0, 0 };
+        next_point(la3, xw[3 * la], xw[3 * la + 1], xw[3 * la + 2], pa);
+        if (lb >= 0) next_point(lb3, xw[3 * lb], xw[3 * lb + 1], xw[3 * lb + 2], pb);
+        linearise_factor<false>(0, f, f + 1, nullptr, rt.fa, rt.fb, rt.Z, rt.Wm, nullptr, nullptr, rt.swp, P.slot_blk, P.slot_rhs, rt.Hc, nullptr, nullptr, nullptr, nullptr, true, pa[0], pa[1], pa[2], pb[0], pb[1], pb[2]);
+    };
+    if (pre.f >= 0) {
+        const double la3[3] = { pre.a0, pre.a1, pre.a2 }, lb3[3] = { pre.b0, pre.b1, pre.b2 };
+        one(pre.f, pre.la, pre.lb, la3, lb3);
+    }
+    for (int q = D_.ff_begin + TPB + (int)threadIdx.x; q < D_.ff_end; q += TPB) {
+        const int4 rec = rt.ff[q];
+        one(rec.x, rec.y, rec.z, rt.lpz + (size_t)3 * rt.fa[rec.x], rt.lpz + (size_t)3 * (rec.z >= 0 ? rt.fb[rec.x] : 0));
+    }
+}
+template <bool TAIL = false>
 __device__ __forceinline__ void backsolve_finish(const FrontDesc &D_, int t, const double *xw, double *__restrict__ x, int *xflags, int *bad, const UpdArgs &upd, int ev = 0,
-                                                 int xmode = X_FLUSH, const DevPlan *P = nullptr, long long *pf = nullptr) {
+                                                 int xmode = X_FLUSH, const DevPlan *P = nullptr, long long *pf = nullptr, const RelinPre *pre = nullptr) {
     const int tid = threadIdx.x, nsb = D_.nsb, ns = 3 * nsb;
     if (xmode == X_TAGGED) {
         const __amdgpu_buffer_rsrc_t r = xg_rsrc(*P);
@@ -1850,13 +1885,16 @@
         for (int k = tid; k < nsb; k += TPB) {
             const int i = upd.perm[D_.first + k];
             const double d0 = xw[3 * k], d1 = xw[3 * k + 1], d2 = xw[3 * k + 2];
-            if (isnan(d0) || isnan(d1) || isnan(d2)) {
+            double sn[3];
+            const bool moved = next_point(upd.lp + (size_t)3 * i, d0, d1, d2, sn);
+            if constexpr (TAIL) { if (upd.rt.lpz_next) { upd.rt.lpz_next[3 * i + 0] = sn[0]; upd.rt.lpz_next[3 * i + 1] = sn[1]; upd.rt.lpz_next[3 * i + 2] = sn[2]; } }
+            if (!moved) {
                 const double qnan = __longlong_as_double(0x7ff8000000000000ll);
                 upd.dX[3 * i + 0] = qnan; upd.dX[3 * i + 1] = qnan; upd.dX[3 * i + 2] = qnan;
                 if (upd.dx_out) { upd.dx_out[3 * i + 0] = qnan; upd.dx_out[3 * i + 1] = qnan; upd.dx_out[3 * i + 2] = qnan; }
                 continue;
             }
-            const double s0 = upd.lp[3 * i + 0] + d0, s1 = upd.lp[3 * i + 1] + d1, s2 = mod2pi_dev(upd.lp[3 * i + 2] + d2);
+            const double s0 = sn[0], s1 = sn[1], s2 = sn[2];
             if (upd.st) { upd.st[3 * i + 0] = s0; upd.st[3 * i + 1] = s1; upd.st[3 * i + 2] = s2; }
             if (upd.lp_next) { upd.lp_next[3 * i + 0] = s0; upd.lp_next[3 * i + 1] = s1; upd.lp_next[3 * i + 2] = s2; }
             upd.dX[3 * i + 0] = d0; upd.dX[3 * i + 1] = d1; upd.dX[3 * i + 2] = d2;
@@ -1870,6 +1908,7 @@
 #pragma unroll
         for (int k = 0; k < 4; k++) upd.bad_out[k] = __hip_atomic_load(bad + k, __ATOMIC_RELAXED, __HIP_MEMORY_SCOPE_AGENT);
     }
+    if constexpr (TAIL) { if (upd.rt.ff) relin_tail(*P, D_, xw, upd.rt, *pre); }
 }
 constexpr int BS_TALL_ROWS = 768;
 template <bool PRE, bool TALL = false>
@@ -2189,7 +2228,7 @@
 
 constexpr int BSW = 64;
 constexpr int BSW_MAX_NS = NB + 8 + NB * (NB + 1) - 256;
-template <int BSWT = BSW>
+template <int BSWT = BSW, bool TAIL = false>
 __device__ __forceinline__ void backsolve_w_body(const DevPlan &P, const int t, const double *__restrict__ pool, double *__restrict__ x, int *xflags, int *bad,
                                                  const UpdArgs &upd, double *smem) {
     const int ev = xflags ? flag_value(P) : 0;
@@ -2206,6 +2245,10 @@
     const int *rows = P.f_rows + D_.rows_begin;
     long long *pf = (P.prof && P.prof_mode == 2) ? P.prof + (size_t)t * PROF_SLOTS : nullptr;
     if (pf && tid == 0) pf[PROF_XCD_DN] = 1 + xcc_id();
+    RelinPre pre{ -1, 0, -1, 0, 0, 0, 0, 0, 0, 0, 0 };
+    const bool pre_on = TAIL && upd.rt.ff && D_.ff_begin + tid < D_.ff_end;
+    int4 pre_rec = { 0, 0, -1, 0 };
+    if constexpr (TAIL) { if (pre_on) pre_rec = upd.rt.ff[D_.ff_begin + tid]; }
     {
         const int ne = ns * R;
         for (int e0 = tid; e0 < ne; e0 += 8 * TPB) {
@@ -2223,6 +2266,7 @@
             }
         }
     }
+    if constexpr (TAIL) { if (pre_on) { pre.f = pre_rec.x; pre.la = pre_rec.y; pre.lb = pre_rec.z; pre.a = upd.rt.fa[pre.f]; pre.b = upd.rt.fb[pre.f]; } }
     const int xmode = x_handover_mode(P, xflags, ev, true);
     const bool xtag = xmode == X_TAGGED && D_.parent >= 0;
     if (xflags && D_.parent >= 0 && !xtag) {
@@ -2236,6 +2280,12 @@
     else for (int e = tid; e < 3 * nub; e += TPB) xw[ns + e] = ld_agent(x + (size_t)3 * rows[e / 3] + e % 3);
     __syncthreads();
     if (pf && tid == 0) pf[5] = wall_clock64();
+    if constexpr (TAIL) {
+        if (pre_on) {
+            const double *la3 = upd.rt.lpz + (size_t)3 * pre.a, *lb3 = upd.rt.lpz + (size_t)3 * (pre.lb >= 0 ? pre.b : pre.a);
+            pre.a0 = la3[0]; pre.a1 = la3[1]; pre.a2 = la3[2]; pre.b0 = lb3[0]; pre.b1 = lb3[1]; pre.b2 = lb3[2];
+        }
+    }
     for (int k1 = ns; k1 > 0; k1 -= BSWT) {
         const int k0 = max(0, k1 - BSWT), wdt = k1 - k0;
         const bool on = lane < wdt;
@@ -2274,14 +2324,23 @@
         __syncthreads();
     }
     if (pf && tid == 0) pf[7] = wall_clock64();
-    backsolve_finish(D_, t, xw, x, xflags, bad, upd, ev, xmode, &P, pf);
+    backsolve_finish<TAIL>(D_, t, xw, x, xflags, bad, upd, ev, xmode, &P, pf, &pre);
+}
+__global__ void k_step_boundary(int *__restrict__ bad, int *__restrict__ epoch) {
+    bad[0] = 0; bad[1] = 0; bad[2] = 0; bad[3] = 0;
+    atomicAdd(epoch, 1);
 }
 __global__ void __launch_bounds__(TPB) k_backsolve_w(DevPlan P, const int *__restrict__ fronts, const double *__restrict__ pool,
                                                      double *__restrict__ x, int *xflags, int *bad, UpdArgs upd) {
     extern __shared__ __attribute__((aligned(16))) double smem[];
     const int t = fronts[blockIdx.x];
+    if (upd.rt.epoch_adv && blockIdx.x == 0 && threadIdx.x == 0) {
+        int *b = upd.rt.bad_clear;
+        b[0] = 0; b[1] = 0; b[2] = 0; b[3] = 0;
+        atomicAdd(upd.rt.epoch_adv, 1);
+    }
     if (t < 0) return;
-    backsolve_w_body(P, t, pool, x, xflags, bad, upd, smem);
+    backsolve_w_body<BSW, true>(P, t, pool, x, xflags, bad, upd, smem);
 }
 
 __host__ __device__ inline long long upd_packed_offset(int R, int ns, int j) {
diff --git a/aprilsam_amd/csrc/plan.h b/aprilsam_amd/csrc/plan.h
--- a/aprilsam_amd/csrc/plan.h
+++ b/aprilsam_amd/csrc/plan.h
@@ -31,6 +31,7 @@
 
     std::vector<int> fac_front;
     std::vector<int> fac_la, fac_lb;
+    std::vector<int> ff_ptr, ff_idx;
     std::vector<int> bd_front_ptr;
     std::vector<int> bd_row, bd_col;
     std::vector<int> bd_src_ptr;
diff --git a/aprilsam_amd/csrc/solver.h b/aprilsam_amd/csrc/solver.h
--- a/aprilsam_amd/csrc/solver.h
+++ b/aprilsam_amd/csrc/solver.h
@@ -44,6 +44,7 @@
     int blk_backsolve = 1;
     int wave_backsolve = 1;
     int tagged_x = 1;
+    int fused_relin = 1;
     int linearize_staged_min = 32768;
     int mem_cap_mb = 0;
     int pool_guard = 0;
diff --git a/aprilsam_amd/csrc/solver.hip.cpp b/aprilsam_amd/csrc/solver.hip.cpp
--- a/aprilsam_amd/csrc/solver.hip.cpp
+++ b/aprilsam_amd/csrc/solver.hip.cpp
@@ -62,7 +62,7 @@
     { "inc_inline", &Options::inc_inline, 0, true }, { "inc_update", &Options::inc_update, 0, true }, { "inc_tail_solve", &Options::inc_tail_solve, 0, true },
     { "inc_lazy_states", &Options::inc_lazy_states, 0, true }, { "inc_replan_tall", &Options::inc_replan_tall, 0, true },
     { "speculate_factors", &Options::speculate_factors, 0, true }, { "warm_up", &Options::warm_up, 0, true }, { "pin_last", &Options::pin_last, 0, false }, { "persist", &Options::persist, 0, false },
-    { "persist_max_fronts", &Options::persist_max_fronts, 0, false }, { "xcd_place", &Options::xcd_place, 0, false }, { "linearize_staged_min", &Options::linearize_staged_min, 0, false },
+    { "persist_max_fronts", &Options::persist_max_fronts, 0, false }, { "xcd_place", &Options::xcd_place, 0, false }, { "linearize_staged_min", &Options::linearize_staged_min, 0, false }, { "fused_relin", &Options::fused_relin, 0, true, 1 },
     { "wave_backsolve", &Options::wave_backsolve, 0, false }, { "tagged_x", &Options::tagged_x, 0, false, 2 }, { "blk_backsolve", &Options::blk_backsolve, 0, false }, { "tail_poses", &Options::tail_poses, 8, false },
     { "batch_extend", &Options::batch_extend, 0, true }, { "extend_tail_fronts", &Options::extend_tail_fronts, 0, true }, { "mem_cap_mb", &Options::mem_cap_mb, 0, true },
     { "pool_guard", &Options::pool_guard, 0, false }, { "amalg", &Options::amalg, 0, false }, { "amalg_max", &Options::amalg_max, 1, false }, { "pool_poison", &Options::pool_poison, 0, false }, { "skip_flag_waits", &Options::skip_flag_waits, 0, false },
diff --git a/aprilsam_amd/csrc/solver_context.inc.h b/aprilsam_amd/csrc/solver_context.inc.h
--- a/aprilsam_amd/csrc/solver_context.inc.h
+++ b/aprilsam_amd/csrc/solver_context.inc.h
@@ -122,6 +122,9 @@
     DBuf<double> d_dinv, d_bsb_far; DBuf<int> d_bsb_flags;
     DBuf<int> d_solve_tab; std::vector<int> solve_tab;
     DBuf<UpdRec> d_upd; DBuf<double> d_wbuf;
+    hipGraphExec_t gexec_fused[4] = {};
+    const void *fused_key[6] = {};
+    DBuf<int> d_ff;
     hipGraphExec_t gexec = nullptr;
     const void *gexec_key = nullptr;
     long long gexec_serial = 0;
@@ -179,7 +182,8 @@
         h_done.release(); h_kstamp.release(); d_prof.release(); d_upd.release(); d_wbuf.release(); d_flags.release(); d_flevel.release(); d_epoch.release(); d_marks.release(); d_perm.release(); d_solve_tab.release(); d_dinv.release(); d_bsb_far.release(); d_bsb_flags.release(); d_guard.release(); d_guard_cnt.release(); n_guard = 0;
         d_lm_trial.release(); d_lm_hacc.release(); d_lm_terms.release(); d_lm_trace.release(); d_lm.release(); h_lm.release();
         d_ch.release(); h_ch.release(); d_ch_sel.release();
-        retire(gexec); retire(gexec_api); retire(gexec_lm); reap_retired(true);
+        d_ff.release();
+        retire(gexec); retire(gexec_api); retire(gexec_lm); for (auto &g : gexec_fused) retire(g); reap_retired(true);
         if (have_events) for (auto &e : ev) (void)hipEventDestroy(e);
         have_events = false;
         for (auto &e : k_ev) (void)hipEventDestroy(e);
@@ -425,7 +429,7 @@
     const Plan &P = c.plan;
     const bool uprof = getenv("APRILSAM_AMD_PLAN_PROFILE") != nullptr;
     const double u0 = uprof ? now_ms() : 0;
-    c.retire(c.gexec); c.retire(c.gexec_api); c.retire(c.gexec_lm); c.api_key_runs = 0;
+    c.retire(c.gexec); c.retire(c.gexec_api); c.retire(c.gexec_lm); for (auto &g : c.gexec_fused) c.retire(g); c.api_key_runs = 0;
     c.lambda_N = -1;
     c.release_sel();
     std::vector<FrontDesc> &fd = c.inc.fd; fd.assign(P.nF, FrontDesc());
@@ -437,6 +441,7 @@
         d.dest_begin = P.dest_front_ptr[t]; d.dest_end = P.dest_front_ptr[t + 1];
         d.ch_begin = P.ch_ptr[t]; d.ch_end = P.ch_ptr[t + 1];
         d.rows_begin = 0; d.parent = P.f_parent[t];
+        d.ff_begin = P.ff_ptr[t]; d.ff_end = P.ff_ptr[t + 1];
     }
     for (int t = 0; t < P.nF; t++) {
         int best = -1, second = -1;
@@ -493,6 +498,13 @@
     HIPCHECK(hipMemcpyAsync(c.d_pos.p, P.pos.data(), (size_t)P.N * 4, hipMemcpyHostToDevice, s));
     c.d_perm.need((size_t)P.N + INC_NODES_);
     HIPCHECK(hipMemcpyAsync(c.d_perm.p, P.perm.data(), (size_t)P.N * 4, hipMemcpyHostToDevice, s));
+    std::vector<int> ffv;
+    {
+        ffv.assign(4 * P.ff_idx.size() + 4, 0);
+        for (size_t q = 0; q < P.ff_idx.size(); q++) { const int f = P.ff_idx[q]; int *r = &ffv[4 * q]; r[0] = f; r[1] = P.fac_la[f]; r[2] = P.fac_lb[f]; }
+        c.d_ff.need(ffv.size());
+        HIPCHECK(hipMemcpyAsync(c.d_ff.p, ffv.data(), ffv.size() * 4, hipMemcpyHostToDevice, s));
+    }
 
     const double u2 = uprof ? now_ms() : 0;
     std::vector<int> tab;
diff --git a/aprilsam_amd/csrc/solver_launch.inc.h b/aprilsam_amd/csrc/solver_launch.inc.h
--- a/aprilsam_amd/csrc/solver_launch.inc.h
+++ b/aprilsam_amd/csrc/solver_launch.inc.h
@@ -40,6 +40,8 @@
     else hipLaunchKernelGGL((k_backsolve_t<false>), dim3(n), dim3(TPB), lds, s, c.dp, list, c.d_pool.p, c.d_x.p, split, (int *)nullptr, 0, bad, upd);
 }
 
+static bool level_takes_wave(const LevelPlan &L) { return g_opt.wave_backsolve && L.bs_gemv.grid == 0 && L.n_all < g_opt.tp_fronts && L.maxns <= BSW_MAX_NS && L.solve_w_lds <= 80 * 1024; }
+static bool multi_takes_wave(int maxns) { return g_opt.wave_backsolve && maxns <= BSW_MAX_NS; }
 static void launch_backsolve(Context &c, const LevelPlan &L, hipStream_t s, KTimer &kt, const int *tab = nullptr, UpdArgs upd = UpdArgs{}, int list_off = -1, int list_n = 0) {
     if (!tab) tab = c.d_tab.p;
     if (!L.n_all) return;
@@ -54,7 +56,7 @@
         n_all = L.n_rest; all_off = L.rest_off; solve_lds = L.rest_lds;
         if (!n_all) { kt.toc(); return; }
     }
-    const bool wave = g_opt.wave_backsolve && L.bs_gemv.grid == 0 && L.n_all < g_opt.tp_fronts && L.maxns <= BSW_MAX_NS && L.solve_w_lds <= 80 * 1024;
+    const bool wave = level_takes_wave(L);
     const BsForm form = wave ? BS_WAVE : solve_lds >= (size_t)(BS_TALL_ROWS + NB + 8 + NB * (NB + 1)) * 8 ? BS_THREAD_TALL : BS_THREAD;
     launch_backsolve_list(c, s, form, tab + all_off, n_all, wave ? L.solve_w_lds : solve_lds, L.bs_gemv.grid > 0 ? 1 : 0, c.d_bad.p, upd);
     kt.toc();
@@ -74,7 +76,7 @@
 static DevPlan persist_plan(const Context &c) { DevPlan d = c.dp; d.flevel = c.d_flevel.p; d.l0 = c.persist_l0; d.xmode = launch_xmode(c, c.p_dn_maxnu); return d; }
 static void launch_backsolve_multi(Context &c, hipStream_t s, const DevPlan &dp, const int *list, int n, size_t lds, int maxns, int *xflags, const UpdArgs &upd) {
     lds = handover_lds(dp.xmode, lds, n);
-    if (g_opt.wave_backsolve && maxns <= BSW_MAX_NS) hipLaunchKernelGGL(k_backsolve_w, dim3(n), dim3(TPB), lds, s, dp, list, c.d_pool.p, c.d_x.p, xflags, c.d_bad.p, upd);
+    if (multi_takes_wave(maxns)) hipLaunchKernelGGL(k_backsolve_w, dim3(n), dim3(TPB), lds, s, dp, list, c.d_pool.p, c.d_x.p, xflags, c.d_bad.p, upd);
     else hipLaunchKernelGGL((k_backsolve_t<true>), dim3(n), dim3(TPB), lds, s, dp, list, c.d_pool.p, c.d_x.p, 0, xflags, 1, c.d_bad.p, upd);
 }
 
@@ -173,6 +175,8 @@
     bool io_host = false;
     bool relin = false;
     double *st_dest = nullptr;
+    bool no_lin = false;
+    bool tail = false; int parity = 0;
     const std::function<void()> *fill = nullptr;
 };
 static void enqueue_numeric(Context &c, GraphPack &gp, hipStream_t s, const NumericArgs &a = NumericArgs{}) {
@@ -185,9 +189,11 @@
     if (c.dp.prof) HIPCHECK(hipMemsetAsync(c.d_prof.p, 0, (size_t)8 * PROF_SLOTS * P.nF, s));
     if (io_host) hipLaunchKernelGGL(k_load_states, dim3((3 * N + TPB - 1) / TPB), dim3(TPB), 0, s, 3 * N, gp.h_state.p, gp.d_state.p, gp.d_lp.p);
     enqueue_poison(c, s, nullptr, P.nF);
-    kt.tic(K_LINEARIZE);
-    if (a.fill) (*a.fill)(); else enqueue_linearise(c, gp, s, a.unary_at_lp);
-    kt.toc();
+    if (!a.no_lin) {
+        kt.tic(K_LINEARIZE);
+        if (a.fill) (*a.fill)(); else enqueue_linearise(c, gp, s, a.unary_at_lp);
+        kt.toc();
+    }
     if (a.ev) HIPCHECK(hipEventRecord(a.ev[1], s));
     const int l0 = c.persist_l0 >= 0 ? c.persist_l0 : P.nLevels;
     for (int l = 0; l < l0; l++) {
@@ -198,7 +204,11 @@
     kt.level = l0;
     if (l0 < P.nLevels) { kt.tic(K_FRONT_SMALL); launch_front_persist(c, s); kt.toc(); }
     if (a.ev) HIPCHECK(hipEventRecord(a.ev[2], s));
-    UpdArgs upd{ c.d_perm.p, gp.d_lp.p, a.st_dest ? a.st_dest : gp.d_state.p, gp.d_dx.p, io_host ? gp.h_lp.p : nullptr, io_host ? gp.h_dx.p : nullptr, nullptr, a.relin ? gp.d_lp.p : nullptr };
+    UpdArgs upd{ c.d_perm.p, gp.d_lp.p, a.st_dest ? a.st_dest : gp.d_state.p, gp.d_dx.p, io_host ? gp.h_lp.p : nullptr, io_host ? gp.h_dx.p : nullptr, nullptr, a.relin ? gp.d_lp.p : nullptr, RelinTail{} };
+    if (a.tail) {
+        double *z0 = gp.d_lpz.p + (size_t)3 * N * (a.parity & 1), *z1 = gp.d_lpz.p + (size_t)3 * N * (1 - (a.parity & 1));
+        upd.rt = RelinTail{ (const int4 *)c.d_ff.p, gp.d_fa.p, gp.d_fb.p, gp.d_z.p, gp.d_W.p, c.d_swap.p, c.d_H.p, z0, z1, nullptr, nullptr };
+    }
     if (l0 < P.nLevels) {
         UpdArgs u = upd; if (l0 == 0) u.bad_out = io_host ? c.h_bad.p : nullptr;
         kt.tic(K_BACKSOLVE);
@@ -208,10 +218,12 @@
     }
     for (int l = l0 - 1; l >= 0; l--) {
         UpdArgs u = upd; if (l == 0) u.bad_out = io_host ? c.h_bad.p : nullptr;
+        if (l == 0 && a.tail) { u.rt.bad_clear = c.d_bad.p; u.rt.epoch_adv = c.d_epoch.p; }
         kt.level = l;
         if (l == 0 && c.x_leaf_n > 0) launch_backsolve(c, c.levels[0], s, kt, nullptr, u, c.x_leaf_off, c.x_leaf_n);
         else launch_backsolve(c, c.levels[l], s, kt, nullptr, u);
     }
+    if (a.tail && l0 == 0) hipLaunchKernelGGL(k_step_boundary, dim3(1), dim3(1), 0, s, c.d_bad.p, c.d_epoch.p);
     if (a.ev) HIPCHECK(hipEventRecord(a.ev[3], s));
     HIPCHECK(hipGetLastError());
 }
@@ -249,7 +261,17 @@
     return it == g_ctx.end() ? -1 : it->second->n_captures;
 }
 
-struct RunArgs { bool timing = false, unary_at_lp = false, io_host = false, relin = false; };
+enum StepForm { STEP_PLAIN = 0, STEP_FIRST, STEP_MID_EVEN, STEP_MID_ODD, STEP_LAST };
+struct RunArgs { bool timing = false, unary_at_lp = false, io_host = false, relin = false; StepForm form = STEP_PLAIN; };
+static bool fused_relin_ok(const Context &c, const GraphPack &gp) {
+    const Plan &P = c.plan;
+    if (!g_opt.fused_relin || !g_opt.use_graph || !gp.host_idx.empty() || gp.n_max() > 0 || gp.n_robust() > 0 || gp.gc_n > 0) return false;
+    if (P.F >= g_opt.linearize_staged_min || gp.F != P.F || !c.inc.t_first.empty() || !c.d_ff.p || (int)P.ff_ptr.size() != P.nF + 1) return false;
+    const int l0 = c.persist_l0 >= 0 ? c.persist_l0 : P.nLevels;
+    if (l0 < P.nLevels && !multi_takes_wave(c.p_dn_maxns)) return false;
+    for (int l = 0; l < l0; l++) { const LevelPlan &L = c.levels[l]; if (L.n_all == 0 || L.bs_blk.grid > 0 || !level_takes_wave(L)) return false; }
+    return true;
+}
 static void run_numeric(Context &c, GraphPack &gp, const RunArgs &r = RunArgs{}) {
     hipStream_t s = gp.stream;
     set_small_attr();
@@ -265,6 +287,11 @@
         if (memcmp(key, c.api_key, sizeof(key)) != 0) { c.retire(c.gexec_api); memcpy(c.api_key, key, sizeof(key)); c.api_key_runs = 0; }
         if (c.api_key_runs++ == 0) enqueue_numeric(c, gp, s, a);
         else replay_captured(c, c.gexec_api, s, [&] { enqueue_numeric(c, gp, s, a); });
+    } else if (!r.io_host && graph && !r.unary_at_lp && r.form != STEP_PLAIN) {
+        a.no_lin = r.form != STEP_FIRST; a.tail = r.form != STEP_LAST; a.parity = r.form == STEP_MID_ODD ? 1 : 0;
+        const void *key[6] = { gp.d_state.p, gp.d_lp.p, gp.d_lpz.p, c.d_ff.p, (const void *)(size_t)gp.serial, (const void *)(size_t)gp.N };
+        if (memcmp(key, c.fused_key, sizeof(key)) != 0) { for (auto &g : c.gexec_fused) c.retire(g); memcpy(c.fused_key, key, sizeof(key)); }
+        replay_captured(c, c.gexec_fused[r.form - 1], s, [&] { enqueue_numeric(c, gp, s, a); });
     } else if (!r.io_host && graph && !r.unary_at_lp) {
         if (c.gexec_key != (const void *)gp.d_state.p || c.gexec_serial != gp.serial || c.gexec_mx != gp.mx_gen || c.gexec_rb != gp.rb_gen) {
             c.retire(c.gexec);
diff --git a/aprilsam_amd/csrc/solver_pack.inc.h b/aprilsam_amd/csrc/solver_pack.inc.h
--- a/aprilsam_amd/csrc/solver_pack.inc.h
+++ b/aprilsam_amd/csrc/solver_pack.inc.h
@@ -34,6 +34,7 @@
     HBuf<double> h_z, h_W, h_state, h_lp, h_dx;
     DBuf<int> d_fa, d_fb;
     DBuf<double> d_z, d_W, d_state, d_lp, d_dx, d_chi2f, d_scalar;
+    DBuf<double> d_lpz;
     DBuf<double> d_lp_last; bool lp_last_valid = false;
     int F_on_device = 0;
     int dirty_lo = 0, dirty_hi = 0;
@@ -71,7 +72,7 @@
     void release() {
         h_out.release(); mirror_sync = false;
         h_fa.release(); h_fb.release(); h_z.release(); h_W.release(); h_state.release(); h_lp.release(); h_dx.release();
-        d_fa.release(); d_fb.release(); d_z.release(); d_W.release(); d_state.release(); d_lp.release(); d_lp_last.release(); d_dx.release();
+        d_fa.release(); d_fb.release(); d_z.release(); d_W.release(); d_state.release(); d_lp.release(); d_lpz.release(); d_lp_last.release(); d_dx.release();
         d_chi2f.release(); d_scalar.release(); h_scalar.release(); h_hostH.release(); d_hostH.release(); d_host_idx.release(); d_upt.release();
         d_mx_f.release(); d_mx_k.release(); d_sel.release(); d_mx_z.release(); d_mx_W.release(); d_mx_c.release(); mx_stage.release(); mx_clear();
         d_rb_f.release(); d_rb_kind.release(); d_rb_c.release(); d_rb_W0.release(); d_rb_w.release(); rb_stage.release(); rb_clear();
diff --git a/aprilsam_amd/csrc/solver_resident.inc.h b/aprilsam_amd/csrc/solver_resident.inc.h
--- a/aprilsam_amd/csrc/solver_resident.inc.h
+++ b/aprilsam_amd/csrc/solver_resident.inc.h
@@ -18,7 +18,7 @@
     if (!c.have_events) { for (auto &e : c.ev) HIPCHECK(hipEventCreate(&e)); c.have_events = true; }
     for (int k = 0; k < NKERN; k++) { c.k_ms[k] = 0; c.k_calls[k] = 0; }
     c.lev_up_ms.clear(); c.lev_dn_ms.clear();
-    c.st.n_nodes = gp.N; c.st.n_factors = gp.F; c.st.symbolic_reused = reused; c.st.not_spd = 0;
+    c.st.n_nodes = gp.N; c.st.n_factors = gp.F; c.st.symbolic_reused = reused; c.st.not_spd = 0; c.st.fused_steps = 0;
     HIPCHECK(hipStreamSynchronize(gp.stream));
     return 0;
 }
@@ -35,6 +35,11 @@
     set_small_attr();
     gp.mirror_sync = false;
     HIPCHECK(hipMemcpyAsync(gp.d_lp.p, gp.d_state.p, (size_t)24 * N, hipMemcpyDeviceToDevice, s));
+    const bool fuse = mode == 0 && n > 1 && fused_relin_ok(c, gp);
+    if (fuse) {
+        gp.d_lpz.need((size_t)6 * N);
+        HIPCHECK(hipMemcpyAsync(gp.d_lpz.p, gp.d_state.p, (size_t)24 * N, hipMemcpyDeviceToDevice, s));
+    }
     for (int i = 0; i < n; i++) {
         if (i == n - 1) {
             gp.d_lp_last.need((size_t)3 * N);
@@ -43,11 +48,13 @@
         }
         if (mode == 1) {
             NumericArgs a; a.ktime = true; a.relin = true;
+            rewind_epoch(c, s, 1);
             enqueue_numeric(c, gp, s, a);
             HIPCHECK(hipStreamSynchronize(s));
             collect_kernel_times(c);
         } else {
             RunArgs r; r.relin = true;
+            if (fuse) { r.form = i == 0 ? STEP_FIRST : i == n - 1 ? STEP_LAST : (i & 1) ? STEP_MID_ODD : STEP_MID_EVEN; c.st.fused_steps += i > 0; }
             run_numeric(c, gp, r);
         }
     }
@@ -205,10 +212,36 @@
 
 static int debug_stage_impl(april_graph_t *g, april_graph_cholesky_param_t *param, int what, double *out);
 int debug_stage(april_graph_t *g, april_graph_cholesky_param_t *param, int what, double *out) { return guarded_rc(param, g, [&] { return debug_stage_impl(g, param, what, out); }); }
+static void export_slots(Context &c, GraphPack &gp, hipStream_t s, double *out) {
+    const Plan &P = c.plan;
+    std::vector<double> H((size_t)9 * std::max(1, P.n_slots));
+    HIPCHECK(hipMemcpyAsync(H.data(), c.d_H.p, H.size() * 8, hipMemcpyDeviceToHost, s));
+    HIPCHECK(hipStreamSynchronize(s));
+    for (int f = 0; f < gp.F; f++) {
+        double *o = out + (size_t)33 * f;
+        memset(o, 0, 33 * 8);
+        memcpy(o, &H[(size_t)9 * P.slot_blk[3 * f]], 72);
+        memcpy(o + 27, &H[(size_t)9 * P.slot_rhs[2 * f]], 24);
+        if (gp.h_fb.p[f] < 0) continue;
+        const double *b1 = &H[(size_t)9 * P.slot_blk[3 * f + 1]];
+        for (int i = 0; i < 3; i++) for (int j = 0; j < 3; j++) o[9 + i * 3 + j] = P.fac_swap[f] ? b1[j * 3 + i] : b1[i * 3 + j];
+        memcpy(o + 18, &H[(size_t)9 * P.slot_blk[3 * f + 2]], 72);
+        memcpy(o + 30, &H[(size_t)9 * P.slot_rhs[2 * f + 1]], 24);
+    }
+}
 static int debug_stage_impl(april_graph_t *g, april_graph_cholesky_param_t *param, int what, double *out) {
     if (zsize(g->nodes) == 0 || zsize(g->factors) == 0) return -1;
     ensure_device();
     SlotLock lk(param, g);
+    if (what == 2 || what == 3) {
+        auto it = g_ctx.find(param);
+        if (it == g_ctx.end() || !it->second->have_plan) return -1;
+        GraphPack &gp = pack_for(g);
+        if (what == 3) { for (int k = 0; k < 4; k++) out[k] = it->second->h_bad.p ? it->second->h_bad.p[k] : 0; return 0; }
+        if (gp.F != it->second->plan.F || !it->second->d_H.p) return -1;
+        export_slots(*it->second, gp, gp.stream, out);
+        return 0;
+    }
     Context &c = ctx_for(param);
     GraphPack &gp = pack_for(g);
     pack_factors(gp, g);
@@ -227,23 +260,7 @@
     enqueue_robust(gp, s, nullptr);
     hipLaunchKernelGGL((k_linearize_t<false>), dim3((F + TPB - 1) / TPB), dim3(TPB), 0, s, 0, F, (const int *)nullptr, gp.d_fa.p, gp.d_fb.p, gp.d_z.p, gp.d_W.p,
                        gp.d_lp.p, gp.d_state.p, c.d_swap.p, c.dp.slot_blk, c.dp.slot_rhs, c.d_H.p, c.d_bad.p, (const double *)nullptr);
-    if (what == 0) {
-        std::vector<double> H((size_t)9 * std::max(1, P.n_slots));
-        HIPCHECK(hipMemcpyAsync(H.data(), c.d_H.p, H.size() * 8, hipMemcpyDeviceToHost, s));
-        HIPCHECK(hipStreamSynchronize(s));
-        for (int f = 0; f < F; f++) {
-            double *o = out + (size_t)33 * f;
-            memset(o, 0, 33 * 8);
-            memcpy(o, &H[(size_t)9 * P.slot_blk[3 * f]], 72);
-            memcpy(o + 27, &H[(size_t)9 * P.slot_rhs[2 * f]], 24);
-            if (gp.h_fb.p[f] < 0) continue;
-            const double *b1 = &H[(size_t)9 * P.slot_blk[3 * f + 1]];
-            for (int i = 0; i < 3; i++) for (int j = 0; j < 3; j++) o[9 + i * 3 + j] = P.fac_swap[f] ? b1[j * 3 + i] : b1[i * 3 + j];
-            memcpy(o + 18, &H[(size_t)9 * P.slot_blk[3 * f + 2]], 72);
-            memcpy(o + 30, &H[(size_t)9 * P.slot_rhs[2 * f + 1]], 24);
-        }
-        return 0;
-    }
+    if (what == 0) { export_slots(c, gp, s, out); return 0; }
     if (what != 1 || N > 2000) return -2;
     const int nd = (int)P.dest.size();
     DBuf<double> d_out; d_out.need((size_t)9 * std::max(1, nd));
diff --git a/aprilsam_amd/csrc/symbolic.cpp b/aprilsam_amd/csrc/symbolic.cpp
--- a/aprilsam_amd/csrc/symbolic.cpp
+++ b/aprilsam_amd/csrc/symbolic.cpp
@@ -232,6 +232,11 @@
     });
     if (lost.load() >= 0) fail(ERR_INTERNAL, "factor %d not inside its front", lost.load());
     for (int f = 0; f < F; f++) if (P.fac_front[f] >= 0 && P.fac_lb[f] >= 0) P.fac_swap[f] = P.fac_la[f] < P.fac_lb[f];
+    P.ff_ptr.assign(nT + 1, 0);
+    for (int f = 0; f < F; f++) if (P.fac_front[f] >= 0) P.ff_ptr[P.fac_front[f] + 1]++;
+    for (int t = 0; t < nT; t++) P.ff_ptr[t + 1] += P.ff_ptr[t];
+    P.ff_idx.resize(P.ff_ptr[nT]);
+    { std::vector<int> fill(P.ff_ptr.begin(), P.ff_ptr.end() - 1); for (int f = 0; f < F; f++) if (P.fac_front[f] >= 0) P.ff_idx[fill[P.fac_front[f]]++] = f; }
     constexpr int KEY_SRC_BITS = 30, KEY_ROW_BITS = 17, KEY_COL_BITS = 16;
     static_assert(1 + KEY_SRC_BITS + KEY_ROW_BITS + KEY_COL_BITS == 64 && sizeof(unsigned long long) == 8, "packed sort keys");
     if ((size_t)3 * F >= (1u << KEY_SRC_BITS) || (size_t)5 * F >= 0x7fffffffu)
diff --git a/include/aprilsam_amd.h b/include/aprilsam_amd.h
--- a/include/aprilsam_amd.h
+++ b/include/aprilsam_amd.h
@@ -160,6 +160,8 @@
     int    inc_old_old_cross;
     int    inc_fronts_updated;
     int    dn_launch_fronts;
+    int    fused_steps;
+    int    reserved2;
 } aprilsam_amd_stats_t;
 int aprilsam_amd_get_stats(const april_graph_cholesky_param_t *param, aprilsam_amd_stats_t *out);
 
```
